# AntoineBlanot/LC2IS

Measured on AMD Instinct MI355X. Metric: training-step images/sec (512x512, ADE20K-150), higher is better.
Workload: dtype bf16; 1 GPU; BaseModelWithText ViT-B/16 + CLIP-text + decoder + fused head/CE train step, 512x512, 151 classes, text len 16, sgd; batch_per_gpu=32, global_batch=32, parallelism=dp1

## Files before the change

### include/lc2is_hip.h

```cpp
#ifndef LC2IS_HIP_H
#define LC2IS_HIP_H
#include <stddef.h>
#include <stdint.h>

#ifdef __cplusplus
extern "C" {
#endif

#define LC2IS_ACT_NONE 0
#define LC2IS_ACT_QUICK_GELU 1
#define LC2IS_ACT_RELU 2
#define LC2IS_ACT_DQUICK_GELU 3
#define LC2IS_ACT_DRELU 4
#define LC2IS_ACT_QUICK_GELU_GRAD 5
#define LC2IS_ACT_MUL_AUX 6
#define LC2IS_ACT_GELU_ERF 7
#define LC2IS_ACT_DGELU_ERF 8
#define LC2IS_ACT_ADD_AUX 9

#define LC2IS_INTERP_BICUBIC 0
#define LC2IS_INTERP_BILINEAR 1

typedef void* lc2is_stream_t;

typedef struct {
  const void* src;
  void* dst;
  void* dstT;
  int N, K, ld_dst, ld_dstT;
  int tile_start;
  int flags;
} lc2is_shadow_desc;

const char* lc2is_version(void);

int lc2is_set_cu_budget(int ncu);
int lc2is_get_cu_budget(void);

int lc2is_gemm_nt_bf16(const void* A, int lda, const void* W, int ldw, const float* bias,
                       const float* resid, int ldr, const void* aux_in, int ldx, void* out_bf16, int ldo,
                       float* out_f32, int ldf, void* aux_out, int ldy, int M, int N, int K, int act,
                       int tile_cfg, lc2is_stream_t stream);

size_t lc2is_gemm_nt_ln_xchg_bytes(int M, int N);
int lc2is_gemm_nt_ln_bf16(const void* A, int lda, const void* W, int ldw, const float* bias, const float* resid, int ldr,
                          float* out_f32, int ldf, const float* gamma, const float* beta, float eps, void* ln_out, int ldl,
                          float* mean, float* rstd, void* xchg, size_t xchg_bytes, int M, int N, int K, lc2is_stream_t stream);

int lc2is_gemm_nt_bf16_batched(const void* A, int lda, long stride_a, const void* W, int ldw, long stride_w,
                               void* out_bf16, int ldo, long stride_ob, float* out_f32, int ldf, long stride_of,
                               int M, int N, int K, int batch, lc2is_stream_t stream);

size_t lc2is_gemm_tn_workspace_bytes(int M, int N, int K);
int lc2is_gemm_tn_bf16(const void* dY, int ldy, const void* X, int ldx, float* dW, int ldw, float* db, int M,
                       int N, int K, int accumulate, void* workspace, size_t workspace_bytes,
                       lc2is_stream_t stream);

#define LC2IS_TN_GROUP_MAX 128
typedef struct lc2is_tn_problem {
  const void* dY; const void* X; float* dW; float* db;
  int ldy, ldx, ldw, M, N, K, accumulate;
} lc2is_tn_problem;
size_t lc2is_gemm_tn_grouped_workspace_bytes(const lc2is_tn_problem* problems, int n);
int lc2is_gemm_tn_grouped(const lc2is_tn_problem* problems, int n, void* workspace, size_t workspace_bytes,
                          lc2is_stream_t stream);
int lc2is_release_captured_tables(void);
int lc2is_captured_tables_mark(void);
int lc2is_release_captured_tables_range(int first, int last);

size_t lc2is_colsum_workspace_bytes(int M, int N);
int lc2is_colsum_bf16(const void* dY, int ldy, float* db, int M, int N, int accumulate, void* workspace,
                      size_t workspace_bytes, lc2is_stream_t stream);

int lc2is_layernorm_fwd(const void* x, int ldx, int x_is_bf16, const float* gamma, const float* beta, void* y_bf16,
                        int ldy, float* y_f32, int ldyf, float* mean, float* rstd, int M, int C, float eps,
                        lc2is_stream_t stream);

size_t lc2is_layernorm_bwd_workspace_bytes(int M, int C);
int lc2is_layernorm_bwd(const void* dy_bf16, int lddy, const float* dy_f32, int lddyf, const void* x,
                        int ldx, int x_is_bf16, const float* gamma, const float* mean, const float* rstd,
                        const void* dres, int lddres, int dres_is_bf16, float* dx_f32, int lddx, void* dx_bf16,
                        int lddxb, float* dgamma, float* dbeta, int accumulate, int M, int C, void* workspace,
                        size_t workspace_bytes, lc2is_stream_t stream);

#define LC2IS_LN_PARTIALS_MAX 64
typedef struct {
  const float* partials;
  float* dgamma;
  float* dbeta;
  int nparts;
  int C;
  int accumulate;
} lc2is_ln_partials;
int lc2is_layernorm_bwd_partials(int M, int C);
int lc2is_ln_partials_reduce(const lc2is_ln_partials* items, int n, lc2is_stream_t stream);

int lc2is_attention_fwd(const void* Q, int ldq, const void* K, int ldk, const void* V, int ldv, void* O,
                        int ldo, float* lse2, const float* kbias, int B, int H, int Sq, int Sk, int D,
                        float scale, int causal, lc2is_stream_t stream);

int lc2is_attention_bwd(const void* Q, int ldq, const void* K, int ldk, const void* V, int ldv,
                        const void* O, int ldo, const void* dO, int lddo, void* dQ, int lddq, void* dK,
                        int lddk, void* dV, int lddv, const float* lse2, float* delta, const float* kbias,
                        int B, int H, int Sq, int Sk, int D, float scale, int causal, lc2is_stream_t stream);

int lc2is_attention_fwd_dropout(const void* Q, int ldq, const void* K, int ldk, const void* V, int ldv, void* O,
                                int ldo, float* lse2, const float* kbias, int B, int H, int Sq, int Sk, int D,
                                float scale, int causal, float p_drop, unsigned long long seed, lc2is_stream_t stream);
int lc2is_attention_bwd_dropout(const void* Q, int ldq, const void* K, int ldk, const void* V, int ldv,
                                const void* O, int ldo, const void* dO, int lddo, void* dQ, int lddq, void* dK,
                                int lddk, void* dV, int lddv, const float* lse2, float* delta, const float* kbias,
                                int B, int H, int Sq, int Sk, int D, float scale, int causal, float p_drop,
                                unsigned long long seed, lc2is_stream_t stream);

int lc2is_dropout_rows_f32(const float* x, int ldx, const float* resid, int ldr, float* y32, int ldy, void* y16,
                           int ldy16, int M, int C, int rows_per_sample, float p, unsigned long long seed,
                           lc2is_stream_t stream);
int lc2is_dropout_rows_bf16(const void* x, int ldx, void* y, int ldy, int M, int C, float p, unsigned long long seed,
                            lc2is_stream_t stream);
int lc2is_dropout_mask(unsigned char* out, long rows, int cols, float p, unsigned long long seed, lc2is_stream_t stream);


int lc2is_shadow_refresh(const lc2is_shadow_desc* descs, int ndesc, int total_tiles, lc2is_stream_t stream);
int lc2is_cast_f32_bf16(const float* src, int ld_src, void* dst_bf16, int ld_dst, int M, int C,
                        lc2is_stream_t stream);
int lc2is_transpose_bf16(const void* src, int ld_src, void* dst, int ld_dst, int R, int C,
                         lc2is_stream_t stream);
int lc2is_transpose_bf16_batched(const void* src, int ld_src, long stride_src, void* dst, int ld_dst, long stride_dst,
                                 int R, int C, int batch, lc2is_stream_t stream);

int lc2is_patchify(const float* pixels, void* out_bf16, int ld_out, int B, int H, int W, int patch,
                   lc2is_stream_t stream);
int lc2is_vit_embed_fwd(const float* patch, int ld_patch, const float* cls, const float* pos, float* x,
                        int ldx, int B, int P, int C, lc2is_stream_t stream);
int lc2is_vit_embed_bwd(const float* dx, int ldx, float* dpos, float* dcls, void* dpatch_bf16, int ld_dpatch,
                        int B, int P, int C, int accumulate, lc2is_stream_t stream);
int lc2is_text_embed_fwd(const int64_t* ids, const float* tok, const float* pos, float* x, int ldx, int B,
                         int L, int C, int vocab, lc2is_stream_t stream);
int lc2is_text_embed_bwd(const int64_t* ids, const float* dx, int ldx, float* dtok, float* dpos, int B, int L,
                         int C, int vocab, int accumulate, lc2is_stream_t stream);
int lc2is_rows_copy_f32(const float* src, int S_src, int src_off, float* dst_f32, void* dst_bf16, int S_dst,
                        int dst_off, int B, int n, int C, lc2is_stream_t stream);
int lc2is_rows_copy_bf16(const void* src, int S_src, int src_off, float* dst_f32, void* dst_bf16, int S_dst,
                         int dst_off, int B, int n, int C, lc2is_stream_t stream);

int lc2is_sgd_step(float* params, const float* grads, float* momentum_buf, size_t n, float lr, float momentum,
                   float weight_decay, float grad_scale, lc2is_stream_t stream);
int lc2is_adamw_step(float* params, const float* grads, float* exp_avg, float* exp_avg_sq, size_t n, float lr,
                     float beta1, float beta2, float eps, float weight_decay, int step, float grad_scale,
                     lc2is_stream_t stream);

size_t lc2is_head_upsample_ce_workspace_bytes(int B, int h, int w, int C, int S, int mode, int want_grad);
int lc2is_head_upsample_ce(const float* scores_lo, int ld, const int64_t* labels, float* dscores_lo,
                           float* scores_hi, float* loss_sum, int B, int h, int w, int C, int S, int mode,
                           long ignore_index, float grad_scale, void* workspace, size_t workspace_bytes,
                           lc2is_stream_t stream);
int lc2is_head_upsample_ce_opts(const float* scores_lo, int ld, const int64_t* labels, float* dscores_lo,
                                float* scores_hi, float* loss_sum, int B, int h, int w, int C, int S, int mode,
                                long ignore_index, float grad_scale, const float* class_weight, float label_smoothing,
                                void* workspace, size_t workspace_bytes, lc2is_stream_t stream);
int lc2is_upsample_bwd_nchw(const float* dhi, float* dlo, int ld, int B, int h, int w, int C, int S, int mode,
                            lc2is_stream_t stream);
int lc2is_ce_nchw_fwd(const float* logits, const int64_t* labels, float* lse, float* loss_sum, int B, int C,
                      long HW, long ignore_index, lc2is_stream_t stream);
int lc2is_ce_nchw_bwd(const float* logits, const int64_t* labels, const float* lse, const float* grad_scale_dev,
                      float grad_scale, float* dlogits, int B, int C, long HW, long ignore_index,
                      lc2is_stream_t stream);
int lc2is_ce_nchw_fwd_opts(const float* logits, const int64_t* labels, float* lse, float* loss_sum, float* loss_px,
                           int B, int C, long HW, long ignore_index, const float* class_weight, float label_smoothing,
                           lc2is_stream_t stream);
int lc2is_ce_nchw_bwd_opts(const float* logits, const int64_t* labels, const float* lse, const float* grad_scale_dev,
                           float grad_scale, const float* grad_px, float* dlogits, int B, int C, long HW,
                           long ignore_index, const float* class_weight, float label_smoothing,
                           lc2is_stream_t stream);
size_t lc2is_ce_nchw_fwd_workspace_bytes(int B, long HW);
int lc2is_ce_nchw_fwd_ordered(const float* logits, const int64_t* labels, float* lse, float* loss_sum, float* loss_px,
                              int B, int C, long HW, long ignore_index, const float* class_weight, float label_smoothing,
                              void* workspace, size_t workspace_bytes, lc2is_stream_t stream);

int lc2is_bilinear_up_fwd(const float* in, float* out_f32, void* out_bf16, int B, int h, int w, int C, int S,
                          lc2is_stream_t stream);
int lc2is_bilinear_up_bwd(const float* dout, float* din_f32, void* din_bf16, int B, int h, int w, int C, int S,
                          int accumulate, lc2is_stream_t stream);
int lc2is_sr_gather(const void* src_bf16, void* dst_bf16, int B, int h, int w, int C, int scatter,
                    lc2is_stream_t stream);
int lc2is_sr_scatter_add_f32(const void* src_bf16, float* dst_f32, int B, int h, int w, int C, lc2is_stream_t stream);
int lc2is_l2norm_fwd(const float* x, float* y_f32, void* y_bf16, float* inv_norm, int M, int C, float eps,
                     lc2is_stream_t stream);
int lc2is_l2norm_bwd(const float* dy, const float* x, const float* inv_norm, float* dx, int M, int C, float eps,
                     lc2is_stream_t stream);
int lc2is_add_n(const float* a, const float* b, const float* c, const float* d, float* out_f32, void* out_bf16,
                size_t n, lc2is_stream_t stream);

int lc2is_rows_gather(const void* src, int ld_src, int src_bf16, void* dst, int ld_dst, int dst_bf16, const int* map,
                      const float* add, int ld_add, int rows, int cols, lc2is_stream_t stream);
int lc2is_swin_attn_fwd(const void* qkv, int ld, void* out, int ldo, float* lse, const float* bias, int nwin,
                        int win_per_img, int nwx, int Hp, int Wp, int ws, int shift, int nH, int C, float scale,
                        lc2is_stream_t stream);
size_t lc2is_swin_attn_bwd_workspace_bytes(int nwin, int ws, int nH);
int lc2is_swin_attn_bwd(const void* qkv, int ld, const void* o, int ld_o, const void* dout, int lddo, const float* lse,
                        const float* bias, void* dqkv, int lddq, float* dbias, int accumulate_dbias, int nwin,
                        int win_per_img, int nwx, int Hp, int Wp, int ws, int shift, int nH, int C, float scale,
                        void* workspace, size_t workspace_bytes, lc2is_stream_t stream);

int lc2is_swin_bias_table_grad(const float* dbias, const int* offsets, const int* positions, float* dtable, int nH, int SS,
                               int T, int accumulate, lc2is_stream_t stream);

int lc2is_resample_u8(const void* src_u8, int H, int W, int C, void* dst_u8, int out_size, int axis, const int* bounds,
                      const int* kk, int ksize, lc2is_stream_t stream);
int lc2is_gather2d_u8(const void* src_u8, int H, int W, int C, void* dst_u8, int out_h, int out_w, const int* yi,
                      const int* xi, lc2is_stream_t stream);
int lc2is_crop_lut(const void* src_u8, int H, int W, int C, int top, int left, int S, const float* lut_f32,
                   float* dst_f32, const int64_t* lut_i64, int64_t* dst_i64, lc2is_stream_t stream);

int lc2is_rows_ce(const float* x, const int64_t* labels, float* lse, float* loss_sum, float* dx, float grad_scale,
                  int M, int K, int accumulate_dx, lc2is_stream_t stream);
int lc2is_cols_ce(const float* x, const int64_t* labels, float* loss_sum, float* dx, float grad_scale, int B, int H,
                  int W, int K, lc2is_stream_t stream);
int lc2is_npair(const float* x, const float* x_pos, const float* x_neg, float* res, int n, int n_pos, int n_neg, int d,
                lc2is_stream_t stream);
int lc2is_npair_bwd(const float* x, const float* x_pos, const float* x_neg, const float* dres, float* dx, float* dx_pos,
                    float* dx_neg, float* workspace, int n, int n_pos, int n_neg, int d, lc2is_stream_t stream);
int lc2is_miou_counts(const float* scores_hi, const int64_t* labels_lo, int* counts, int B, int K, int H, int W, int S,
                      lc2is_stream_t stream);

#define LC2IS_RESIZE_TILE 16
size_t lc2is_resize_argmax_workspace_bytes(long n_tiles, int K);
int lc2is_resize_argmax(const float* scores, int ld, int N, int h, int w, int K, const int64_t* desc, long n_tiles,
                        long total_px, const void* gt, int gt_bytes, uint8_t* pred, int* counts, void* workspace,
                        size_t workspace_bytes, lc2is_stream_t stream);

typedef struct {
  int32_t calls;
// ... 45 lines not shown
```

### lc2is_amd/csrc/gemm_tn.hip

```cpp
#include "common.h"
#include "lc2is_hip.h"
#include <cstdlib>
#include <mutex>
#include <vector>
#include <type_traits>

namespace {

constexpr int TN_BN = 128, TN_BK = 128, TN_BM = 64;
constexpr int TN_TILE_BYTES = TN_BM * 256;
constexpr int TN_STAGE = 2 * TN_TILE_BYTES;

struct TnPlan {
  int ntn, ntk, splits, chunk;
  int big;
};

inline int tn_forced_cfg() {
  static int cfg = -1;
  if (cfg < 0) {
    const char* e = getenv("LC2IS_GEMM_TN_CFG");
    cfg = e ? atoi(e) : 0;
  }
  return cfg;
}

inline TnPlan tn_plan(int M, int N, int K, int ncu) {
  TnPlan p;
  p.big = 0;
  if (N % 256 == 0 && K % 256 == 0 && tn_forced_cfg() != 1) {
    const int ntn = N / 256, ntk = K / 256, tiles = ntn * ntk;
    int splits = (ncu + tiles / 2) / tiles;
    const int max_splits = (M + 511) / 512;
    if (splits > max_splits) splits = max_splits;
    if (splits < 1) splits = 1;
    if (tiles * splits >= 128 || tn_forced_cfg() == 2) {
      int chunk = (M + splits - 1) / splits;
      chunk = (chunk + TN_BM - 1) / TN_BM * TN_BM;
      p.ntn = ntn; p.ntk = ntk; p.chunk = chunk;
      p.splits = (M + chunk - 1) / chunk;
      p.big = 1;
      return p;
    }
  }
  p.ntn = (N + TN_BN - 1) / TN_BN;
  p.ntk = (K + TN_BK - 1) / TN_BK;
  const int tiles = p.ntn * p.ntk;
  int splits = 1024 / tiles;
  int max_splits = (M + 511) / 512;
  const int long_splits = (M + 2047) / 2048;
  if ((long)tiles * long_splits >= 512) max_splits = long_splits;
  if (splits > max_splits) splits = max_splits;
  if (splits < 1) splits = 1;
  int chunk = (M + splits - 1) / splits;
  chunk = (chunk + TN_BM - 1) / TN_BM * TN_BM;
  p.splits = (M + chunk - 1) / chunk;
  p.chunk = chunk;
  return p;
}

__device__ __forceinline__ int tn_swz(int row, int ch) {
  return row * 256 + ((ch ^ (((row & 3) << 2) | ((row >> 2) & 3))) << 4);
}

__device__ __forceinline__ bf16x8_t tr_frag(const char* tile, int addr_lo, int addr_hi) {
  const s16x4_t lo = __builtin_amdgcn_ds_read_tr16_b64_v4i16(
      (__attribute__((address_space(3))) s16x4_t*)LDS_PTR(tile + addr_lo));
  const s16x4_t hi = __builtin_amdgcn_ds_read_tr16_b64_v4i16(
      (__attribute__((address_space(3))) s16x4_t*)LDS_PTR(tile + addr_hi));
  s16x8_t v = {lo[0], lo[1], lo[2], lo[3], hi[0], hi[1], hi[2], hi[3]};
  return __builtin_bit_cast(bf16x8_t, v);
}

__device__ __forceinline__ void tn_small_body(const bf16_t* __restrict__ dY, int ldy,
                                                       const bf16_t* __restrict__ X, int ldx, float* out,
                                                       int ldo, size_t split_stride, float* bias_out,
                                                       size_t bias_split_stride, int M, int N, int K,
                                                       int ntn, int ntk, int chunk, int accumulate, int blk_x, char* smem) {
  const int tid = threadIdx.x, lane = tid & 63, wid = tid >> 6;
  const int wk = wid >> 1, wn = wid & 1;
  const int tiles = ntn * ntk;
  const int split = blk_x / tiles;
  const int tile = blk_x % tiles;
  const int n0 = (tile / ntk) * TN_BN, k0 = (tile % ntk) * TN_BK;
// ... 77 lines not shown
      if (more) gload(st + 1);
#pragma unroll
      for (int s = 0; s < 2; ++s) {
        bf16x8_t xf[4], yf[4];
#pragma unroll
        for (int t = 0; t < 4; ++t) {
          yf[t] = tr_frag(cur, ya_lo[s][t], ya_hi[s][t]);
          xf[t] = tr_frag(cur + TN_TILE_BYTES, xa_lo[s][t], xa_hi[s][t]);
        }
#pragma unroll
        for (int a = 0; a < 4; ++a)
#pragma unroll
          for (int b = 0; b < 4; ++b)
            acc[a][b] = __builtin_amdgcn_mfma_f32_16x16x32_bf16(xf[a], yf[b], acc[a][b], 0, 0, 0);
        if constexpr (CS) {
#pragma unroll
          for (int b = 0; b < 4; ++b) cs[b] = __builtin_amdgcn_mfma_f32_16x16x32_bf16(ones, yf[b], cs[b], 0, 0, 0);
        }
      }
      if (more) lstore(nxt);
      __syncthreads();
    }
  };
  if (do_cs) mainloop(std::true_type{}); else mainloop(std::false_type{});

  float* o = out + (size_t)split * split_stride;
  if (do_cs && lane < 16) {
#pragma unroll
    for (int b = 0; b < 4; ++b) {
      const int n = n0 + wn * 64 + b * 16 + lane;
      if (n < N) {
        float* dst = bias_out + (size_t)split * bias_split_stride + n;
        *dst = (accumulate ? *dst : 0.f) + cs[b][0];
      }
    }
  }
#pragma unroll
  for (int b = 0; b < 4; ++b) {
    const int n = n0 + wn * 64 + b * 16 + (lane & 15);
    if (n >= N) continue;
#pragma unroll
    for (int a = 0; a < 4; ++a) {
      const int k = k0 + wk * 64 + a * 16 + g * 4;
      if (k >= K) continue;
      float* dst = o + (size_t)n * ldo + k;
      f32x4_t v = acc[a][b];
      if (accumulate) v += *(const f32x4_t*)dst;
      *(f32x4_t*)dst = v;
    }
  }
}

__global__ __launch_bounds__(256) void gemm_tn_kernel(const bf16_t* __restrict__ dY, int ldy,
                                                       const bf16_t* __restrict__ X, int ldx, float* out,
                                                       int ldo, size_t split_stride, float* bias_out,
                                                       size_t bias_split_stride, int M, int N, int K,
                                                       int ntn, int ntk, int chunk, int accumulate) {
  extern __shared__ __attribute__((aligned(16))) char smem[];
  tn_small_body(dY, ldy, X, ldx, out, ldo, split_stride, bias_out, bias_split_stride, M, N, K, ntn, ntk, chunk, accumulate,
                (int)blockIdx.x, smem);
}

constexpr int TD_BN = 256, TD_BK = 256;
constexpr int TD_TILE = TN_BM * 512;
constexpr int TD_STAGE = 2 * TD_TILE;

__device__ __forceinline__ int td_swz(int row) { return ((row & 3) << 2) | ((row >> 2) & 3); }

__device__ __forceinline__ void td_dma(const bf16_t* dY, unsigned y_bytes, const bf16_t* X, unsigned x_bytes, char* stage,
                                       int wid, const int* y_goff, const int* x_goff, int ystep, int xstep) {
#if defined(__HIP_DEVICE_COMPILE__)
  const __amdgpu_buffer_rsrc_t rsY = make_rsrc(dY, y_bytes);
  const __amdgpu_buffer_rsrc_t rsX = make_rsrc(X, x_bytes);
#pragma unroll
  for (int j = 0; j < 4; ++j)
    __builtin_amdgcn_raw_ptr_buffer_load_lds(rsY, LDS_PTR(stage + (wid * 4 + j) * 1024), 16, y_goff[j], ystep, 0, 0);
#pragma unroll
  for (int j = 0; j < 4; ++j)
    __builtin_amdgcn_raw_ptr_buffer_load_lds(rsX, LDS_PTR(stage + TD_TILE + (wid * 4 + j) * 1024), 16, x_goff[j], xstep,
                                             0, 0);
#endif
}

__device__ __forceinline__ void tn_dma_body(const bf16_t* __restrict__ dY, int ldy, const bf16_t* __restrict__ X, int ldx,
                                            float* out, int ldo, size_t split_stride, float* bias_out,
                                            size_t bias_split_stride, int M, int N, int K, int ntn, int ntk, int chunk,
                                            int accumulate, int block, char* smem) {
  const int tid = threadIdx.x, lane = tid & 63;
  const int wid = __builtin_amdgcn_readfirstlane(tid >> 6);
  const int wk = wid >> 2, wn = wid & 3;
  const int tiles = ntn * ntk;
  const int split = block / tiles;
  const int tile = block % tiles;
  const int n0 = (tile / ntk) * TD_BN, k0 = (tile % ntk) * TD_BK;
  const int m_begin = split * chunk;
  int m_end = m_begin + chunk;
  if (m_end > M) m_end = M;
  const int nsteps = (m_end - m_begin + TN_BM - 1) / TN_BM;
  const unsigned y_bytes = (unsigned)m_end * (unsigned)ldy * 2u, x_bytes = (unsigned)m_end * (unsigned)ldx * 2u;

  int y_goff[4], x_goff[4];
#pragma unroll
  for (int j = 0; j < 4; ++j) {
    const int row = 2 * (wid * 4 + j) + (lane >> 5);
    const int ch = (lane & 31) ^ td_swz(row);
    y_goff[j] = ((m_begin + row) * ldy + n0 + ch * 8) * 2;
    x_goff[j] = ((m_begin + row) * ldx + k0 + ch * 8) * 2;
  }

  const int g = lane >> 4, q = (lane >> 2) & 3, pp = lane & 3;
  const int r_lo = 8 * g + q, r_hi = r_lo + 4;
  const int x_lo = TD_TILE + r_lo * 512 + (((wk * 16 + (pp >> 1)) ^ td_swz(r_lo)) << 4) + 8 * (pp & 1);
  const int x_hi = TD_TILE + r_hi * 512 + (((wk * 16 + (pp >> 1)) ^ td_swz(r_hi)) << 4) + 8 * (pp & 1);
  const int y_lo = r_lo * 512 + (((wn * 8 + (pp >> 1)) ^ td_swz(r_lo)) << 4) + 8 * (pp & 1);
  const int y_hi = r_hi * 512 + (((wn * 8 + (pp >> 1)) ^ td_swz(r_hi)) << 4) + 8 * (pp & 1);

  f32x4_t acc[8][4];
#pragma unroll
  for (int a = 0; a < 8; ++a)
#pragma unroll
    for (int b = 0; b < 4; ++b) acc[a][b] = f32x4_t{0.f, 0.f, 0.f, 0.f};
  const bool do_cs = (bias_out != nullptr) && (tile % ntk == 0) && (wk == 0);
  f32x4_t cs[4];
#pragma unroll
  for (int b = 0; b < 4; ++b) cs[b] = f32x4_t{0.f, 0.f, 0.f, 0.f};
  const s16x8_t ones_s = {0x3F80, 0x3F80, 0x3F80, 0x3F80, 0x3F80, 0x3F80, 0x3F80, 0x3F80};
  const bf16x8_t ones = __builtin_bit_cast(bf16x8_t, ones_s);

  if (nsteps > 0) td_dma(dY, y_bytes, X, x_bytes, smem, wid, y_goff, x_goff, 0, 0);
  __syncthreads();

  auto mainloop = [&](auto cs_tag) {
    constexpr bool CS = decltype(cs_tag)::value;
    for (int st = 0; st < nsteps; ++st) {
      const char* cur = smem + (st & 1) * TD_STAGE;
      if (st + 1 < nsteps)
        td_dma(dY, y_bytes, X, x_bytes, smem + ((st + 1) & 1) * TD_STAGE, wid, y_goff, x_goff,
               (st + 1) * TN_BM * ldy * 2, (st + 1) * TN_BM * ldx * 2);
#pragma unroll
      for (int s = 0; s < 2; ++s) {
        bf16x8_t xf[8], yf[4];
#pragma unroll
        for (int t = 0; t < 4; ++t) yf[t] = tr_frag(cur + s * 16384, y_lo ^ (t << 5), y_hi ^ (t << 5));
#pragma unroll
        for (int t = 0; t < 8; ++t) xf[t] = tr_frag(cur + s * 16384, x_lo ^ (t << 5), x_hi ^ (t << 5));
#pragma unroll
        for (int b = 0; b < 4; ++b)
#pragma unroll
          for (int a = 0; a < 8; ++a)
            acc[a][b] = __builtin_amdgcn_mfma_f32_16x16x32_bf16(xf[a], yf[b], acc[a][b], 0, 0, 0);
        if constexpr (CS) {
#pragma unroll
          for (int b = 0; b < 4; ++b) cs[b] = __builtin_amdgcn_mfma_f32_16x16x32_bf16(ones, yf[b], cs[b], 0, 0, 0);
        }
      }
      __syncthreads();
    }
  };
  if (do_cs) mainloop(std::true_type{}); else mainloop(std::false_type{});

  float* o = out + (size_t)split * split_stride;
  if (do_cs && lane < 16) {
#pragma unroll
    for (int b = 0; b < 4; ++b) {
      const int n = n0 + wn * 64 + b * 16 + lane;
      float* dst = bias_out + (size_t)split * bias_split_stride + n;
      *dst = (accumulate ? *dst : 0.f) + cs[b][0];
    }
  }
#pragma unroll
  for (int b = 0; b < 4; ++b) {
    const int n = n0 + wn * 64 + b * 16 + (lane & 15);
#pragma unroll
    for (int a = 0; a < 8; ++a) {
      const int k = k0 + wk * 128 + a * 16 + g * 4;
      float* dst = o + (size_t)n * ldo + k;
      f32x4_t v = acc[a][b];
      if (accumulate) v += *(const f32x4_t*)dst;
      *(f32x4_t*)dst = v;
    }
  }
}

__global__ __launch_bounds__(512, 2) void gemm_tn_dma_kernel(const bf16_t* __restrict__ dY, int ldy,
                                                              const bf16_t* __restrict__ X, int ldx, float* out, int ldo,
                                                              size_t split_stride, float* bias_out,
                                                              size_t bias_split_stride, int M, int N, int K, int ntn,
                                                              int ntk, int chunk, int accumulate) {
  extern __shared__ __attribute__((aligned(16))) char smem[];
  tn_dma_body(dY, ldy, X, ldx, out, ldo, split_stride, bias_out, bias_split_stride, M, N, K, ntn, ntk, chunk, accumulate,
              blockIdx.x, smem);
}

constexpr int TG_MAX = 16;
struct TnGroupProb {
  const bf16_t* dY; const bf16_t* X; float* out; float* bias_out; float* dW; float* db;
  size_t split_stride, bias_split_stride;
  int ldy, ldx, ldo, ldw, M, N, K, ntn, ntk, chunk, splits, accumulate;
  int blk_end;
  int red_end;
  int red_blocks;
};
struct TnGroup {
  int n, remap;
  TnGroupProb p[TG_MAX];
};

constexpr int TG_TBL_MAX = LC2IS_TN_GROUP_MAX;
struct TnGroupTbl {
  int n, pad_[3];
  int blk_end[TG_TBL_MAX];
  int red_end[TG_TBL_MAX];
  TnGroupProb p[TG_TBL_MAX];
};
constexpr size_t TG_TBL_BYTES = (sizeof(TnGroupTbl) + 255) / 256 * 256;

__global__ __launch_bounds__(512, 2) void gemm_tn_grouped_tbl_kernel(const TnGroupTbl* __restrict__ t) {
  extern __shared__ __attribute__((aligned(16))) char smem[];
  int i = 0, begin = 0;
  const int n = t->n;
  const int bid = t->pad_[0] ? xcd_round_remap((int)blockIdx.x, (int)gridDim.x) : (int)blockIdx.x;
#pragma unroll 1
  while (i < n - 1 && bid >= t->blk_end[i]) { begin = t->blk_end[i]; ++i; }
  const TnGroupProb* q = &t->p[i];
  tn_dma_body(q->dY, q->ldy, q->X, q->ldx, q->out, q->ldo, q->split_stride, q->bias_out, q->bias_split_stride, q->M, q->N,
              q->K, q->ntn, q->ntk, q->chunk, q->splits == 1 ? q->accumulate : 0, bid - begin, smem);
}

__global__ __launch_bounds__(256) void gemm_tn_grouped_small_kernel(TnGroup g) {
  extern __shared__ __attribute__((aligned(16))) char smem[];
  int i = 0, begin = 0;
#pragma unroll 1
  while (i < g.n - 1 && (int)blockIdx.x >= g.p[i].blk_end) { begin = g.p[i].blk_end; ++i; }
  const TnGroupProb& q = g.p[i];
  tn_small_body(q.dY, q.ldy, q.X, q.ldx, q.out, q.ldo, q.split_stride, q.bias_out, q.bias_split_stride, q.M, q.N, q.K, q.ntn,
                q.ntk, q.chunk, q.splits == 1 ? q.accumulate : 0, (int)blockIdx.x - begin, smem);
}

__global__ __launch_bounds__(256) void gemm_tn_grouped_small_tbl_kernel(const TnGroupTbl* __restrict__ t) {
  extern __shared__ __attribute__((aligned(16))) char smem[];
  int i = 0, begin = 0;
  const int n = t->n;
#pragma unroll 1
  while (i < n - 1 && (int)blockIdx.x >= t->blk_end[i]) { begin = t->blk_end[i]; ++i; }
  const TnGroupProb* q = &t->p[i];
  tn_small_body(q->dY, q->ldy, q->X, q->ldx, q->out, q->ldo, q->split_stride, q->bias_out, q->bias_split_stride, q->M, q->N,
                q->K, q->ntn, q->ntk, q->chunk, q->splits == 1 ? q->accumulate : 0, (int)blockIdx.x - begin, smem);
}

__global__ __launch_bounds__(512, 2) void gemm_tn_grouped_kernel(TnGroup g) {
  extern __shared__ __attribute__((aligned(16))) char smem[];
  int i = 0, begin = 0;
  const int bid = g.remap ? xcd_round_remap((int)blockIdx.x, (int)gridDim.x) : (int)blockIdx.x;
#pragma unroll 1
  while (i < g.n - 1 && bid >= g.p[i].blk_end) { begin = g.p[i].blk_end; ++i; }
  const TnGroupProb& q = g.p[i];
  tn_dma_body(q.dY, q.ldy, q.X, q.ldx, q.out, q.ldo, q.split_stride, q.bias_out, q.bias_split_stride, q.M, q.N, q.K, q.ntn,
              q.ntk, q.chunk, q.splits == 1 ? q.accumulate : 0, bid - begin, smem);
}

__device__ __forceinline__ void slab_reduce_grouped_body(const TnGroupProb& q, int b);

__global__ __launch_bounds__(256) void slab_reduce_grouped_kernel(TnGroup g) {
  int i = 0, begin = 0;
#pragma unroll 1
  while (i < g.n - 1 && (int)blockIdx.x >= g.p[i].red_end) { begin = g.p[i].red_end; ++i; }
  slab_reduce_grouped_body(g.p[i], (int)blockIdx.x - begin);
}

__global__ __launch_bounds__(256) void slab_reduce_grouped_tbl_kernel(const TnGroupTbl* __restrict__ t) {
  int i = 0, begin = 0;
  const int n = t->n;
#pragma unroll 1
  while (i < n - 1 && (int)blockIdx.x >= t->red_end[i]) { begin = t->red_end[i]; ++i; }
  slab_reduce_grouped_body(t->p[i], (int)blockIdx.x - begin);
}

__device__ __forceinline__ void slab_reduce_grouped_body(const TnGroupProb& q, int b) {
  if (q.splits <= 1) return;
  if (b >= q.red_blocks) {
    const int n = (b - q.red_blocks) * 256 + threadIdx.x;
    if (q.db && n < q.N) {
      float t = 0.f;
      for (int sp = 0; sp < q.splits; ++sp) t += q.bias_out[(size_t)sp * q.bias_split_stride + n];
      q.db[n] = q.accumulate ? q.db[n] + t : t;
    }
    return;
  }
  const int K4 = q.K >> 2;
  const size_t total = (size_t)q.N * K4;
  for (size_t idx = (size_t)b * 256 + threadIdx.x; idx < total; idx += (size_t)q.red_blocks * 256) {
    const int n = (int)(idx / K4), k4 = (int)(idx % K4);
    float4 s4 = *(reinterpret_cast<const float4*>(q.out + (size_t)n * q.K) + k4);
    for (int sp = 1; sp < q.splits; ++sp) {
      const float4 v = *reinterpret_cast<const float4*>(q.out + sp * q.split_stride + (size_t)n * q.K + 4 * k4);
      s4.x += v.x; s4.y += v.y; s4.z += v.z; s4.w += v.w;
    }
    float4* dst = reinterpret_cast<float4*>(q.dW + (size_t)n * q.ldw) + k4;
    if (q.accumulate) {
      const float4 d = *dst;
      s4.x += d.x; s4.y += d.y; s4.z += d.z; s4.w += d.w;
    }
    *dst = s4;
  }
}

__global__ __launch_bounds__(256) void slab_reduce_kernel(const float* __restrict__ ws, int splits,
                                                           size_t split_stride, float* out, int ldo, int N,
                                                           int K, int accumulate, const float* __restrict__ bias_ws,
                                                           float* db, int bias_blocks) {
  const int slab_blocks = gridDim.x - bias_blocks;
  if ((int)blockIdx.x >= slab_blocks) {
    const int n = (blockIdx.x - slab_blocks) * 256 + threadIdx.x;
    if (n < N) {
      float t = 0.f;
      for (int sp = 0; sp < splits; ++sp) t += bias_ws[(size_t)sp * N + n];
      db[n] = accumulate ? db[n] + t : t;
    }
    return;
  }
  const int K4 = K >> 2;
  const size_t total = (size_t)N * K4;
  for (size_t i = (size_t)blockIdx.x * 256 + threadIdx.x; i < total; i += (size_t)slab_blocks * 256) {
    const int n = (int)(i / K4), k4 = (int)(i % K4);
    const float4* src = reinterpret_cast<const float4*>(ws + (size_t)n * K) + k4;
    float4 s = *src;
    for (int sp = 1; sp < splits; ++sp) {
      const float4 v = *reinterpret_cast<const float4*>(ws + sp * split_stride + (size_t)n * K + 4 * k4);
      s.x += v.x; s.y += v.y; s.z += v.z; s.w += v.w;
    }
    float4* dst = reinterpret_cast<float4*>(out + (size_t)n * ldo) + k4;
    if (accumulate) {
      const float4 d = *dst;
      s.x += d.x; s.y += d.y; s.z += d.z; s.w += d.w;
    }
    *dst = s;
  }
}

constexpr int CS_ROWBLOCKS = 128;

__global__ __launch_bounds__(256) void colsum_kernel(const bf16_t* __restrict__ dY, int ldy, float* ws, int M,
                                                      int N) {
  __shared__ float red[4][64][8];
  const int lane = threadIdx.x & 63, wave = threadIdx.x >> 6;
  const int cg = blockIdx.x * 64 + lane;
  float s[8] = {0.f, 0.f, 0.f, 0.f, 0.f, 0.f, 0.f, 0.f};
  if (cg * 8 < N) {
    for (int row = blockIdx.y * 4 + wave; row < M; row += gridDim.y * 4) {
      const uint4 v = *reinterpret_cast<const uint4*>(dY + (size_t)row * ldy + cg * 8);
      s[0] += bf16_to_f32((bf16_t)(v.x & 0xffff)); s[1] += bf16_to_f32((bf16_t)(v.x >> 16));
      s[2] += bf16_to_f32((bf16_t)(v.y & 0xffff)); s[3] += bf16_to_f32((bf16_t)(v.y >> 16));
      s[4] += bf16_to_f32((bf16_t)(v.z & 0xffff)); s[5] += bf16_to_f32((bf16_t)(v.z >> 16));
      s[6] += bf16_to_f32((bf16_t)(v.w & 0xffff)); s[7] += bf16_to_f32((bf16_t)(v.w >> 16));
    }
  }
#pragma unroll
  for (int j = 0; j < 8; ++j) red[wave][lane][j] = s[j];
  __syncthreads();
  if (wave == 0 && cg * 8 < N) {
#pragma unroll
    for (int j = 0; j < 8; ++j)
      ws[(size_t)blockIdx.y * N + cg * 8 + j] =
          (red[0][lane][j] + red[1][lane][j]) + (red[2][lane][j] + red[3][lane][j]);
  }
}

__global__ __launch_bounds__(256) void colsum_reduce_kernel(const float* __restrict__ ws, int nparts, int N,
                                                             float* db, int accumulate) {
  const int c = blockIdx.x * 256 + threadIdx.x;
  if (c >= N) return;
  float s = 0.f;
  for (int p = 0; p < nparts; ++p) s += ws[(size_t)p * N + c];
  db[c] = accumulate ? db[c] + s : s;
}

inline int colsum_parts(int M) {
  int p = (M + 3) / 4;
  return p > CS_ROWBLOCKS ? CS_ROWBLOCKS : p;
}

}

static size_t tn_plan_bytes(const TnPlan& p, int N, int K) {
  return p.splits > 1 ? (size_t)p.splits * N * ((size_t)K + 1) * sizeof(float) : 0;
}
// ... 108 lines not shown
    wbytes += 4.0 * pr[i].N * pr[i].K;
    const int steps = (pr[i].M + TN_BM - 1) / TN_BM;
    if (steps > max_steps) max_steps = steps;
    const int ms = (pr[i].M + 511) / 512;
    if (ms < max_splits) max_splits = ms;
  }
  if (max_splits > 32) max_splits = 32;
  if (max_splits < 1) max_splits = 1;
  const double slab_unit = 2.0 / 4.0e12 / 1.65e-6;
  int best = 1;
  double best_t = 1e300;
  for (int sp = 1; sp <= max_splits; ++sp) {
    const long blocks = tiles * sp;
    const double rounds = (double)((blocks + ncu - 1) / ncu);
    const double t = rounds * ((max_steps + sp - 1) / sp + 13.0) + (sp > 1 ? sp * wbytes * slab_unit : 0.0);
    if (t < best_t) { best_t = t; best = sp; }
  }
  for (int i = 0; i < n; ++i) { pl.splits[i] = best; pl.order[i] = i; }
  const int rem = (int)(tiles % ncu);
  if (n > 1 && tiles > ncu && rem != 0 && max_splits >= 2) {
    bool in_tail[TG_TBL_MAX] = {};
    int ts = 0;
    double tail_bytes = 0;
    while (ts < rem) {
      int pick = -1;
      for (int i = 0; i < n; ++i)
        if (!in_tail[i] && (pick < 0 || ptiles[i] <= ptiles[pick])) pick = i;
      if (pick < 0) break;
      in_tail[pick] = true;
      ts += ptiles[pick];
      tail_bytes += 4.0 * pr[pick].N * pr[pick].K;
    }
    int sp = ts > 0 ? ncu / ts : 0;
    if (sp > max_splits) sp = max_splits;
    if (ts >= rem && sp >= 2) {
      const double rounds = (double)((tiles - ts + ncu - 1) / ncu);
      const double t = rounds * (max_steps + 13.0) + ((max_steps + sp - 1) / sp + 13.0) + sp * tail_bytes * slab_unit;
      if (t < best_t) {
        int k = 0;
        for (int i = 0; i < n; ++i) if (!in_tail[i]) { pl.order[k++] = i; pl.splits[i] = 1; }
        for (int i = 0; i < n; ++i) if (in_tail[i]) { pl.order[k++] = i; pl.splits[i] = sp; }
      }
    }
  }
  pl.ws_floats = 0;
  for (int i = 0; i < n; ++i)
    if (pl.splits[i] > 1) pl.ws_floats += (size_t)pl.splits[i] * pr[i].N * ((size_t)pr[i].K + 1);
}
}

static std::mutex g_captured_mu;
static std::vector<void*> g_captured_tables;

extern "C" int lc2is_release_captured_tables(void) {
  std::lock_guard<std::mutex> lock(g_captured_mu);
  int n = 0;
  for (void*& p : g_captured_tables)
    if (p) { (void)hipHostFree(p); p = nullptr; ++n; }
  return n;
}

extern "C" int lc2is_captured_tables_mark(void) {
  std::lock_guard<std::mutex> lock(g_captured_mu);
  return (int)g_captured_tables.size();
}

extern "C" int lc2is_release_captured_tables_range(int first, int last) {
  std::lock_guard<std::mutex> lock(g_captured_mu);
  if (first < 0) first = 0;
  if (last > (int)g_captured_tables.size()) last = (int)g_captured_tables.size();
  int n = 0;
  for (int i = first; i < last; ++i)
    if (g_captured_tables[i]) { (void)hipHostFree(g_captured_tables[i]); g_captured_tables[i] = nullptr; ++n; }
  return n;
}

extern "C" size_t lc2is_gemm_tn_grouped_workspace_bytes(const lc2is_tn_problem* problems, int n) {
  if (tg_valid(problems, n) != LC2IS_OK) return 0;
  TgPlan pl;
  tg_plan(problems, n, pl, lc2is_ncu());
  return pl.ws_floats * sizeof(float) + (n > TG_MAX ? TG_TBL_BYTES : 0);
}

extern "C" int lc2is_gemm_tn_grouped(const lc2is_tn_problem* problems, int n, void* workspace, size_t workspace_bytes,
                                     lc2is_stream_t stream_) {
  hipStream_t stream = (hipStream_t)stream_;
  int rc = tg_valid(problems, n);
  if (rc) return rc;
  TgPlan pl;
  tg_plan(problems, n, pl, lc2is_ncu());
  const bool tbl = n > TG_MAX;
  const size_t need = pl.ws_floats * sizeof(float) + (tbl ? TG_TBL_BYTES : 0);
  if (need && (!workspace || workspace_bytes < need)) return LC2IS_ERR_WORKSPACE;
  struct TblSlot { TnGroupTbl* host; hipEvent_t done; bool in_flight; };
  static thread_local TblSlot ring[4] = {};
  static thread_local unsigned ring_pos = 0;
  static thread_local TnGroupTbl small_tbl;
  TblSlot* slot = nullptr;
  TnGroupTbl* captured_tbl = nullptr;
  if (tbl) {
    hipStreamCaptureStatus cap = hipStreamCaptureStatusNone;
    if (hipStreamIsCapturing(stream, &cap) != hipSuccess) return LC2IS_ERR_LAUNCH;
    if (cap != hipStreamCaptureStatusNone) {
      hipStreamCaptureMode mode = hipStreamCaptureModeRelaxed;
      if (hipThreadExchangeStreamCaptureMode(&mode) != hipSuccess) return LC2IS_ERR_LAUNCH;
      const hipError_t e = hipHostMalloc((void**)&captured_tbl, sizeof(TnGroupTbl), hipHostMallocDefault);
      if (hipThreadExchangeStreamCaptureMode(&mode) != hipSuccess || e != hipSuccess) return LC2IS_ERR_LAUNCH;
      {
        std::lock_guard<std::mutex> lock(g_captured_mu);
        g_captured_tables.push_back(captured_tbl);
      }
    } else {
      slot = &ring[ring_pos++ & 3];
      if (!slot->host) {
        if (hipHostMalloc((void**)&slot->host, sizeof(TnGroupTbl), hipHostMallocDefault) != hipSuccess ||
            hipEventCreateWithFlags(&slot->done, hipEventDisableTiming) != hipSuccess)
          return LC2IS_ERR_LAUNCH;
      }
      if (slot->in_flight && hipEventSynchronize(slot->done) != hipSuccess) return LC2IS_ERR_LAUNCH;
      slot->in_flight = false;
    }
  }
  TnGroupTbl& t = captured_tbl ? *captured_tbl : (tbl ? *slot->host : small_tbl);
  static const int xcd_order = !(getenv("LC2IS_TN_XCD") && atoi(getenv("LC2IS_TN_XCD")) == 0);
  t.n = n;
  t.pad_[0] = xcd_order;
  float* ws = (float*)((char*)workspace + (tbl ? TG_TBL_BYTES : 0));
  int blk = 0, red = 0;
  for (int k = 0; k < n; ++k) {
    const int i = pl.order[k];
    const lc2is_tn_problem& q = problems[i];
    TnGroupProb& d = t.p[k];
    d.dY = (const bf16_t*)q.dY; d.X = (const bf16_t*)q.X; d.dW = q.dW; d.db = q.db;
    d.ldy = q.ldy; d.ldx = q.ldx; d.ldw = q.ldw; d.M = q.M; d.N = q.N; d.K = q.K; d.accumulate = q.accumulate;
    d.ntn = pl.small ? (q.N + TN_BN - 1) / TN_BN : q.N / 256;
    d.ntk = pl.small ? (q.K + TN_BK - 1) / TN_BK : q.K / 256;
    int chunk = (q.M + pl.splits[i] - 1) / pl.splits[i];
    chunk = (chunk + TN_BM - 1) / TN_BM * TN_BM;
    d.chunk = chunk;
    d.splits = (q.M + chunk - 1) / chunk;
    if (pl.splits[i] > 1) {
      float* base = ws;
      ws += (size_t)pl.splits[i] * q.N * ((size_t)q.K + 1);
      if (d.splits > 1) {
        d.out = base; d.ldo = q.K; d.split_stride = (size_t)q.N * q.K;
        d.bias_out = q.db ? base + (size_t)d.splits * q.N * q.K : nullptr; d.bias_split_stride = (size_t)q.N;
      }
    }
    if (d.splits <= 1) {
      d.out = q.dW; d.ldo = q.ldw; d.split_stride = 0; d.bias_out = q.db; d.bias_split_stride = 0;
    }
    blk += d.ntn * d.ntk * d.splits;
    d.blk_end = blk;
    const size_t total4 = (size_t)q.N * q.K / 4;
    int rb = (int)((total4 + 255) / 256);
    if (rb > 1024) rb = 1024;
    d.red_blocks = d.splits > 1 ? rb : 0;
    red += d.splits > 1 ? rb + (q.db ? (q.N + 255) / 256 : 0) : 0;
    d.red_end = red;
    t.blk_end[k] = blk;
    t.red_end[k] = red;
  }
  static DevOnce attr_set;
  if (attr_set.need()) {
    if (hipFuncSetAttribute((const void*)gemm_tn_grouped_kernel, hipFuncAttributeMaxDynamicSharedMemorySize,
                            2 * TD_STAGE) != hipSuccess ||
        hipFuncSetAttribute((const void*)gemm_tn_grouped_tbl_kernel, hipFuncAttributeMaxDynamicSharedMemorySize,
                            2 * TD_STAGE) != hipSuccess ||
        hipFuncSetAttribute((const void*)gemm_tn_grouped_small_kernel, hipFuncAttributeMaxDynamicSharedMemorySize,
                            2 * TN_STAGE) != hipSuccess ||
        hipFuncSetAttribute((const void*)gemm_tn_grouped_small_tbl_kernel, hipFuncAttributeMaxDynamicSharedMemorySize,
                            2 * TN_STAGE) != hipSuccess)
      return LC2IS_ERR_LAUNCH;
    attr_set.done();
  }
  if (tbl) {
    if (hipMemcpyAsync(workspace, &t, sizeof(TnGroupTbl), hipMemcpyHostToDevice, stream) != hipSuccess) return LC2IS_ERR_LAUNCH;
    if (slot) {
      if (hipEventRecord(slot->done, stream) != hipSuccess) return LC2IS_ERR_LAUNCH;
      slot->in_flight = true;
    }
    const TnGroupTbl* dt = (const TnGroupTbl*)workspace;
    if (pl.small)
      hipLaunchKernelGGL(gemm_tn_grouped_small_tbl_kernel, dim3(blk), dim3(256), 2 * TN_STAGE, stream, dt);
    else
      hipLaunchKernelGGL(gemm_tn_grouped_tbl_kernel, dim3(blk), dim3(512), 2 * TD_STAGE, stream, dt);
    rc = lc2is_check_launch();
    if (rc || red == 0) return rc;
    hipLaunchKernelGGL(slab_reduce_grouped_tbl_kernel, dim3(red), dim3(256), 0, stream, dt);
    return lc2is_check_launch();
  }
  TnGroup g{};
  g.n = n;
  g.remap = xcd_order;
  for (int k = 0; k < n; ++k) g.p[k] = t.p[k];
  if (pl.small)
    hipLaunchKernelGGL(gemm_tn_grouped_small_kernel, dim3(blk), dim3(256), 2 * TN_STAGE, stream, g);
  else
    hipLaunchKernelGGL(gemm_tn_grouped_kernel, dim3(blk), dim3(512), 2 * TD_STAGE, stream, g);
  rc = lc2is_check_launch();
  if (rc || red == 0) return rc;
  hipLaunchKernelGGL(slab_reduce_grouped_kernel, dim3(red), dim3(256), 0, stream, g);
  return lc2is_check_launch();
}

extern "C" size_t lc2is_colsum_workspace_bytes(int M, int N) {
  if (M <= 0 || N <= 0) return 0;
  return (size_t)colsum_parts(M) * N * sizeof(float);
}

extern "C" int lc2is_colsum_bf16(const void* dY, int ldy, float* db, int M, int N, int accumulate,
                                 void* workspace, size_t workspace_bytes, lc2is_stream_t stream_) {
  hipStream_t stream = (hipStream_t)stream_;
  if (!dY || !db) return LC2IS_ERR_NULL;
  if (M <= 0 || N <= 0 || N % 8 || ldy < N || ldy % 8) return LC2IS_ERR_SHAPE;
  if (!workspace || workspace_bytes < lc2is_colsum_workspace_bytes(M, N)) return LC2IS_ERR_WORKSPACE;
  const int parts = colsum_parts(M);
  hipLaunchKernelGGL(colsum_kernel, dim3((N / 8 + 63) / 64, parts), dim3(256), 0, stream, (const bf16_t*)dY,
                     ldy, (float*)workspace, M, N);
  int rc = lc2is_check_launch();
  if (rc) return rc;
  hipLaunchKernelGGL(partials_reduce_kernel, dim3((N + 31) / 32, 1), dim3(1024), 0, stream,
                     (const float*)workspace, parts, (size_t)N, (size_t)0, N, db, (float*)nullptr, accumulate);
  return lc2is_check_launch();
}
```

### lc2is_amd/csrc/misc.hip

```cpp
#include "common.h"
#include "lc2is_hip.h"

namespace {

__global__ __launch_bounds__(256) void shadow_refresh_kernel(const lc2is_shadow_desc* __restrict__ descs,
                                                              int ndesc) {
  __shared__ bf16_t tile[64][66];
  int lo = 0, hi = ndesc - 1;
  const int bid = blockIdx.x;
  while (lo < hi) {
    const int mid = (lo + hi + 1) >> 1;
    if (descs[mid].tile_start <= bid) lo = mid; else hi = mid - 1;
  }
  const lc2is_shadow_desc d = descs[lo];
  const int t = bid - d.tile_start;
  const int tk = (d.K + 63) / 64;
  const int n0 = (t / tk) * 64, k0 = (t % tk) * 64;
  const float* src = (const float*)d.src;
  bf16_t* dst = (bf16_t*)d.dst;
  bf16_t* dstT = (bf16_t*)d.dstT;
  const int tx = threadIdx.x & 15, ty = threadIdx.x >> 4;
#pragma unroll
  for (int r = 0; r < 4; ++r) {
    const int n = n0 + ty + 16 * r, k = k0 + 4 * tx;
    float4 v = make_float4(0.f, 0.f, 0.f, 0.f);
    if (n < d.N && k < d.K) v = *reinterpret_cast<const float4*>(src + (size_t)n * d.K + k);
    const bf16_t b0 = f32_to_bf16(v.x), b1 = f32_to_bf16(v.y), b2 = f32_to_bf16(v.z), b3 = f32_to_bf16(v.w);
    if (d.flags & 1) {
      if (dst && n < d.N && k < d.K) *reinterpret_cast<float4*>((float*)d.dst + (size_t)n * d.ld_dst + k) = v;
    } else if (dst && n < d.N && k < d.K) {
      uint2 pk = make_uint2((unsigned)b0 | ((unsigned)b1 << 16), (unsigned)b2 | ((unsigned)b3 << 16));
      *reinterpret_cast<uint2*>(dst + (size_t)n * d.ld_dst + k) = pk;
    }
    tile[ty + 16 * r][4 * tx + 0] = b0;
    tile[ty + 16 * r][4 * tx + 1] = b1;
    tile[ty + 16 * r][4 * tx + 2] = b2;
    tile[ty + 16 * r][4 * tx + 3] = b3;
  }
  if (!dstT) return;
  __syncthreads();
#pragma unroll
  for (int r = 0; r < 4; ++r) {
    const int k = k0 + ty + 16 * r, n = n0 + 4 * tx;
    if (k < d.K && n < d.N) {
      const int kk = ty + 16 * r;
      uint2 pk = make_uint2((unsigned)tile[4 * tx][kk] | ((unsigned)tile[4 * tx + 1][kk] << 16),
                            (unsigned)tile[4 * tx + 2][kk] | ((unsigned)tile[4 * tx + 3][kk] << 16));
      *reinterpret_cast<uint2*>(dstT + (size_t)k * d.ld_dstT + n) = pk;
    }
  }
}

__global__ __launch_bounds__(256) void cast_f32_bf16_kernel(const float* __restrict__ src, int lds_,
                                                             bf16_t* dst, int ldd, int M, int C) {
  const int C4 = C >> 2;
  const size_t total = (size_t)M * C4;
  for (size_t i = (size_t)blockIdx.x * 256 + threadIdx.x; i < total; i += (size_t)gridDim.x * 256) {
    const int m = (int)(i / C4), c4 = (int)(i % C4);
    const float4 v = *reinterpret_cast<const float4*>(src + (size_t)m * lds_ + 4 * c4);
    *reinterpret_cast<uint2*>(dst + (size_t)m * ldd + 4 * c4) =
        make_uint2(pack_bf16x2(v.x, v.y), pack_bf16x2(v.z, v.w));
  }
}

__global__ __launch_bounds__(256) void transpose_bf16_kernel(const bf16_t* __restrict__ src, int lds_,
                                                              bf16_t* dst, int ldd, int R, int C, long bs_src,
                                                              long bs_dst) {
  __shared__ bf16_t tile[64][66];
  src += (size_t)blockIdx.z * bs_src;
  dst += (size_t)blockIdx.z * bs_dst;
  const int r0 = blockIdx.y * 64, c0 = blockIdx.x * 64;
  const int tx = threadIdx.x & 63, ty = threadIdx.x >> 6;
  for (int r = ty; r < 64; r += 4) {
    const int rr = r0 + r, cc = c0 + tx;
    tile[r][tx] = (rr < R && cc < C) ? src[(size_t)rr * lds_ + cc] : (bf16_t)0;
  }
  __syncthreads();
  for (int c = ty; c < 64; c += 4) {
    const int cc = c0 + c, rr = r0 + tx;
    if (cc < C && rr < R) dst[(size_t)cc * ldd + rr] = tile[tx][c];
  }
}

__global__ __launch_bounds__(256) void patchify_kernel(const float* __restrict__ pix, bf16_t* out, int ldo,
// ... 82 lines not shown
    }
  }
}

__global__ __launch_bounds__(256) void text_embed_fwd_kernel(const int64_t* __restrict__ ids,
                                                              const float* __restrict__ tok,
                                                              const float* __restrict__ pos, float* x, int ldx,
                                                              int BL, int L, int C, int vocab) {
  const int C4 = C >> 2;
  const size_t total = (size_t)BL * C4;
  for (size_t i = (size_t)blockIdx.x * 256 + threadIdx.x; i < total; i += (size_t)gridDim.x * 256) {
    const int c4 = (int)(i % C4), r = (int)(i / C4);
    int64_t id = ids[r];
    if (id < 0) id = 0;
    if (id >= vocab) id = vocab - 1;
    const float4 t = *reinterpret_cast<const float4*>(tok + (size_t)id * C + 4 * c4);
    const float4 pe = *reinterpret_cast<const float4*>(pos + (size_t)(r % L) * C + 4 * c4);
    *reinterpret_cast<float4*>(x + (size_t)r * ldx + 4 * c4) =
        make_float4(t.x + pe.x, t.y + pe.y, t.z + pe.z, t.w + pe.w);
  }
}

__global__ __launch_bounds__(256) void text_embed_dtok_kernel(const int64_t* __restrict__ ids, const float* __restrict__ dx,
                                                               int ldx, float* dtok, int R, int C, int vocab) {
  const int r = blockIdx.x;
  auto clampid = [&](int64_t v) { return v < 0 ? (int64_t)0 : (v >= vocab ? (int64_t)(vocab - 1) : v); };
  const int64_t id = clampid(ids[r]);
  int seen = 0;
  for (int q = threadIdx.x; q < r; q += 256) seen |= (clampid(ids[q]) == id);
  if (__syncthreads_or(seen)) return;
  for (int c = threadIdx.x; c < C; c += 256) {
    float acc = 0.f;
    for (int q = r; q < R; ++q)
      if (clampid(ids[q]) == id) acc += dx[(size_t)q * ldx + c];
    dtok[(size_t)id * C + c] += acc;
  }
}

__global__ __launch_bounds__(256) void text_embed_bwd_kernel(const float* __restrict__ dx, int ldx, float* dpos, int B, int L,
                                                              int C, int accumulate) {
  const int total = L * C;
  for (int i = blockIdx.x * 256 + threadIdx.x; i < total; i += gridDim.x * 256) {
    const int c = i % C, l = i / C;
    float acc = 0.f;
    for (int b = 0; b < B; ++b) acc += dx[((size_t)b * L + l) * ldx + c];
    dpos[(size_t)l * C + c] = accumulate ? dpos[(size_t)l * C + c] + acc : acc;
  }
}

__global__ __launch_bounds__(256) void rows_copy_bf16_kernel(const bf16_t* __restrict__ src, int S_src, int src_off,
                                                              float* dst, bf16_t* dst_b, int S_dst, int dst_off,
                                                              int B, int n, int C) {
  const int C4 = C >> 2;
  const size_t total = (size_t)B * n * C4;
  for (size_t i = (size_t)blockIdx.x * 256 + threadIdx.x; i < total; i += (size_t)gridDim.x * 256) {
    const int c4 = (int)(i % C4);
    const int r = (int)(i / C4);
    const int s = r % n, b = r / n;
    const uint2 pk = *reinterpret_cast<const uint2*>(src + ((size_t)b * S_src + src_off + s) * C + 4 * c4);
    const size_t o = ((size_t)b * S_dst + dst_off + s) * C + 4 * c4;
    if (dst) *reinterpret_cast<float4*>(dst + o) = make_float4(bf16_to_f32((bf16_t)(pk.x & 0xffff)), bf16_to_f32((bf16_t)(pk.x >> 16)),
                                                               bf16_to_f32((bf16_t)(pk.y & 0xffff)), bf16_to_f32((bf16_t)(pk.y >> 16)));
    if (dst_b) *reinterpret_cast<uint2*>(dst_b + o) = pk;
  }
}

__global__ __launch_bounds__(256) void rows_copy_kernel(const float* __restrict__ src, int S_src, int src_off,
                                                         float* dst, bf16_t* dst_b, int S_dst, int dst_off,
                                                         int B, int n, int C) {
  const int C4 = C >> 2;
  const size_t total = (size_t)B * n * C4;
  for (size_t i = (size_t)blockIdx.x * 256 + threadIdx.x; i < total; i += (size_t)gridDim.x * 256) {
    const int c4 = (int)(i % C4);
    const int r = (int)(i / C4);
    const int s = r % n, b = r / n;
    const float4 v = *reinterpret_cast<const float4*>(src + ((size_t)b * S_src + src_off + s) * C + 4 * c4);
    const size_t o = ((size_t)b * S_dst + dst_off + s) * C + 4 * c4;
    if (dst) *reinterpret_cast<float4*>(dst + o) = v;
    if (dst_b) *reinterpret_cast<uint2*>(dst_b + o) = make_uint2(pack_bf16x2(v.x, v.y), pack_bf16x2(v.z, v.w));
  }
}

__global__ __launch_bounds__(256) void sgd_kernel(float* p, const float* __restrict__ g, float* mom, size_t n4,
                                                   float lr, float momentum, float wd, float gscale) {
  for (size_t i = (size_t)blockIdx.x * 256 + threadIdx.x; i < n4; i += (size_t)gridDim.x * 256) {
    float4 pv = reinterpret_cast<float4*>(p)[i];
    const float4 gv = reinterpret_cast<const float4*>(g)[i];
    float d[4] = {gv.x * gscale + wd * pv.x, gv.y * gscale + wd * pv.y, gv.z * gscale + wd * pv.z,
                  gv.w * gscale + wd * pv.w};
    if (mom) {
      float4 mv = reinterpret_cast<float4*>(mom)[i];
      mv.x = momentum * mv.x + d[0]; mv.y = momentum * mv.y + d[1];
      mv.z = momentum * mv.z + d[2]; mv.w = momentum * mv.w + d[3];
      reinterpret_cast<float4*>(mom)[i] = mv;
      d[0] = mv.x; d[1] = mv.y; d[2] = mv.z; d[3] = mv.w;
    }
    pv.x -= lr * d[0]; pv.y -= lr * d[1]; pv.z -= lr * d[2]; pv.w -= lr * d[3];
    reinterpret_cast<float4*>(p)[i] = pv;
  }
}

__global__ __launch_bounds__(256) void adamw_kernel(float* p, const float* __restrict__ g, float* m, float* v,
                                                     size_t n4, float lr, float b1, float b2, float eps,
                                                     float wd, float bc1, float bc2, float gscale) {
  for (size_t i = (size_t)blockIdx.x * 256 + threadIdx.x; i < n4; i += (size_t)gridDim.x * 256) {
    float4 pv = reinterpret_cast<float4*>(p)[i];
    const float4 gv = reinterpret_cast<const float4*>(g)[i];
    float4 mv = reinterpret_cast<float4*>(m)[i], vv = reinterpret_cast<float4*>(v)[i];
    float* pp = &pv.x; const float* gp = &gv.x; float* mp = &mv.x; float* vp = &vv.x;
#pragma unroll
    for (int k = 0; k < 4; ++k) {
      const float gg = gp[k] * gscale;
      pp[k] *= (1.f - lr * wd);
      mp[k] = b1 * mp[k] + (1.f - b1) * gg;
      vp[k] = b2 * vp[k] + (1.f - b2) * gg * gg;
      const float denom = sqrtf(vp[k]) / sqrtf(bc2) + eps;
      pp[k] -= (lr / bc1) * (mp[k] / denom);
    }
    reinterpret_cast<float4*>(p)[i] = pv;
    reinterpret_cast<float4*>(m)[i] = mv;
    reinterpret_cast<float4*>(v)[i] = vv;
  }
}

inline int ew_grid(size_t work_items) {
  size_t g = (work_items + 255) / 256;
  if (g > 4096) g = 4096;
  if (g < 1) g = 1;
  return (int)g;
}

}

extern "C" int lc2is_shadow_refresh(const lc2is_shadow_desc* descs_dev, int ndesc, int total_tiles,
                                    lc2is_stream_t stream_) {
  hipStream_t stream = (hipStream_t)stream_;
  if (!descs_dev) return LC2IS_ERR_NULL;
  if (ndesc <= 0 || total_tiles <= 0) return LC2IS_ERR_SHAPE;
  hipLaunchKernelGGL(shadow_refresh_kernel, dim3(total_tiles), dim3(256), 0, stream, descs_dev, ndesc);
  return lc2is_check_launch();
}

extern "C" int lc2is_cast_f32_bf16(const float* src, int ld_src, void* dst, int ld_dst, int M, int C,
                                   lc2is_stream_t stream_) {
  hipStream_t stream = (hipStream_t)stream_;
  if (!src || !dst) return LC2IS_ERR_NULL;
  if (M <= 0 || C <= 0 || C % 4 || ld_src < C || ld_dst < C || ld_src % 4 || ld_dst % 4) return LC2IS_ERR_SHAPE;
  hipLaunchKernelGGL(cast_f32_bf16_kernel, dim3(ew_grid((size_t)M * C / 4)), dim3(256), 0, stream, src, ld_src,
                     (bf16_t*)dst, ld_dst, M, C);
  return lc2is_check_launch();
}

extern "C" int lc2is_transpose_bf16(const void* src, int ld_src, void* dst, int ld_dst, int R, int C,
                                    lc2is_stream_t stream_) {
  hipStream_t stream = (hipStream_t)stream_;
  if (!src || !dst) return LC2IS_ERR_NULL;
  if (R <= 0 || C <= 0 || ld_src < C || ld_dst < R) return LC2IS_ERR_SHAPE;
  hipLaunchKernelGGL(transpose_bf16_kernel, dim3((C + 63) / 64, (R + 63) / 64), dim3(256), 0, stream,
                     (const bf16_t*)src, ld_src, (bf16_t*)dst, ld_dst, R, C, 0L, 0L);
  return lc2is_check_launch();
}

extern "C" int lc2is_transpose_bf16_batched(const void* src, int ld_src, long stride_src, void* dst, int ld_dst,
                                            long stride_dst, int R, int C, int batch, lc2is_stream_t stream_) {
  hipStream_t stream = (hipStream_t)stream_;
  if (!src || !dst) return LC2IS_ERR_NULL;
  if (R <= 0 || C <= 0 || ld_src < C || ld_dst < R || batch <= 0 || batch > 65535) return LC2IS_ERR_SHAPE;
  hipLaunchKernelGGL(transpose_bf16_kernel, dim3((C + 63) / 64, (R + 63) / 64, batch), dim3(256), 0, stream,
                     (const bf16_t*)src, ld_src, (bf16_t*)dst, ld_dst, R, C, stride_src, stride_dst);
  return lc2is_check_launch();
}

extern "C" int lc2is_patchify(const float* pixels, void* out_bf16, int ld_out, int B, int H, int W,
                              int patch, lc2is_stream_t stream_) {
  hipStream_t stream = (hipStream_t)stream_;
  if (!pixels || !out_bf16) return LC2IS_ERR_NULL;
  if (B <= 0 || H <= 0 || W != H || patch <= 0 || H / patch <= 0) return LC2IS_ERR_SHAPE;
  const int G = H / patch, kdim = 3 * patch * patch;
  if (ld_out < kdim) return LC2IS_ERR_SHAPE;
  if (patch % 8 == 0 && W % 8 == 0 && ld_out % 8 == 0 && ((uintptr_t)pixels & 15) == 0 && ((uintptr_t)out_bf16 & 15) == 0)
    hipLaunchKernelGGL(patchify8_kernel, dim3(ew_grid((size_t)B * 3 * H * W / 8)), dim3(256), 0, stream, pixels, (bf16_t*)out_bf16,
                       ld_out, B, H, W, patch, G);
  else
    hipLaunchKernelGGL(patchify_kernel, dim3(B * G * 3 * patch), dim3(256), 0, stream, pixels, (bf16_t*)out_bf16,
                       ld_out, B, H, W, patch, G);
  int rc = lc2is_check_launch();
  if (rc || ld_out == kdim) return rc;
  hipLaunchKernelGGL(zero_pad_cols_kernel, dim3(ew_grid((size_t)B * G * G * (ld_out - kdim))), dim3(256), 0,
                     stream, (bf16_t*)out_bf16, ld_out, B * G * G, kdim);
  return lc2is_check_launch();
}

extern "C" int lc2is_vit_embed_fwd(const float* patch, int ld_patch, const float* cls, const float* pos,
                                   float* x, int ldx, int B, int P, int C, lc2is_stream_t stream_) {
  hipStream_t stream = (hipStream_t)stream_;
  if (!patch || !cls || !pos || !x) return LC2IS_ERR_NULL;
  if (B <= 0 || P <= 0 || C <= 0 || C % 4 || ld_patch < C || ld_patch % 4 || ldx < C || ldx % 4)
    return LC2IS_ERR_SHAPE;
  hipLaunchKernelGGL(vit_embed_fwd_kernel, dim3(ew_grid((size_t)B * (P + 1) * C / 4)), dim3(256), 0, stream,
                     patch, ld_patch, cls, pos, x, ldx, B, P, C);
  return lc2is_check_launch();
}

extern "C" int lc2is_vit_embed_bwd(const float* dx, int ldx, float* dpos, float* dcls, void* dpatch_bf16,
                                   int ld_dpatch, int B, int P, int C, int accumulate, lc2is_stream_t stream_) {
  hipStream_t stream = (hipStream_t)stream_;
  if (!dx || !dpos || !dcls) return LC2IS_ERR_NULL;
  if (B <= 0 || P <= 0 || C <= 0 || C % 4 || ldx < C || ldx % 4 || (dpatch_bf16 && (ld_dpatch < C || ld_dpatch % 4)))
    return LC2IS_ERR_SHAPE;
  hipLaunchKernelGGL(vit_embed_bwd_kernel, dim3(ew_grid((size_t)(P + 1) * C / 4)), dim3(256), 0, stream, dx, ldx,
                     dpos, dcls, (bf16_t*)dpatch_bf16, ld_dpatch, B, P, C, accumulate);
  return lc2is_check_launch();
}

extern "C" int lc2is_text_embed_fwd(const int64_t* ids, const float* tok, const float* pos, float* x, int ldx,
                                    int B, int L, int C, int vocab, lc2is_stream_t stream_) {
  hipStream_t stream = (hipStream_t)stream_;
  if (!ids || !tok || !pos || !x) return LC2IS_ERR_NULL;
  if (B <= 0 || L <= 0 || C <= 0 || C % 4 || vocab <= 0 || ldx < C || ldx % 4) return LC2IS_ERR_SHAPE;
  hipLaunchKernelGGL(text_embed_fwd_kernel, dim3(ew_grid((size_t)B * L * C / 4)), dim3(256), 0, stream, ids, tok,
                     pos, x, ldx, B * L, L, C, vocab);
  return lc2is_check_launch();
}

extern "C" int lc2is_text_embed_bwd(const int64_t* ids, const float* dx, int ldx, float* dtok, float* dpos,
                                    int B, int L, int C, int vocab, int accumulate, lc2is_stream_t stream_) {
  hipStream_t stream = (hipStream_t)stream_;
  if (!ids || !dx || !dtok || !dpos) return LC2IS_ERR_NULL;
  if (B <= 0 || L <= 0 || C <= 0 || vocab <= 0 || ldx < C) return LC2IS_ERR_SHAPE;
  hipLaunchKernelGGL(text_embed_dtok_kernel, dim3(B * L), dim3(256), 0, stream, ids, dx, ldx, dtok, B * L, C, vocab);
  int rc = lc2is_check_launch();
  if (rc) return rc;
  hipLaunchKernelGGL(text_embed_bwd_kernel, dim3(ew_grid((size_t)L * C)), dim3(256), 0, stream, dx, ldx, dpos, B, L, C,
                     accumulate);
  return lc2is_check_launch();
}

extern "C" int lc2is_rows_copy_f32(const float* src, int S_src, int src_off, float* dst_f32, void* dst_bf16,
                                   int S_dst, int dst_off, int B, int n, int C, lc2is_stream_t stream_) {
  hipStream_t stream = (hipStream_t)stream_;
  if (!src || (!dst_f32 && !dst_bf16)) return LC2IS_ERR_NULL;
  if (B <= 0 || n <= 0 || C <= 0 || C % 4 || src_off < 0 || dst_off < 0 || src_off + n > S_src ||
      dst_off + n > S_dst)
    return LC2IS_ERR_SHAPE;
  hipLaunchKernelGGL(rows_copy_kernel, dim3(ew_grid((size_t)B * n * C / 4)), dim3(256), 0, stream, src, S_src,
                     src_off, dst_f32, (bf16_t*)dst_bf16, S_dst, dst_off, B, n, C);
  return lc2is_check_launch();
}

extern "C" int lc2is_rows_copy_bf16(const void* src, int S_src, int src_off, float* dst_f32, void* dst_bf16,
                                    int S_dst, int dst_off, int B, int n, int C, lc2is_stream_t stream_) {
  hipStream_t stream = (hipStream_t)stream_;
  if (!src || (!dst_f32 && !dst_bf16)) return LC2IS_ERR_NULL;
  if (B <= 0 || n <= 0 || C <= 0 || C % 4 || src_off < 0 || dst_off < 0 || src_off + n > S_src ||
      dst_off + n > S_dst)
    return LC2IS_ERR_SHAPE;
  hipLaunchKernelGGL(rows_copy_bf16_kernel, dim3(ew_grid((size_t)B * n * C / 4)), dim3(256), 0, stream, (const bf16_t*)src,
                     S_src, src_off, dst_f32, (bf16_t*)dst_bf16, S_dst, dst_off, B, n, C);
  return lc2is_check_launch();
}

extern "C" int lc2is_sgd_step(float* params, const float* grads, float* momentum_buf, size_t n, float lr,
                              float momentum, float weight_decay, float grad_scale, lc2is_stream_t stream_) {
  hipStream_t stream = (hipStream_t)stream_;
  if (!params || !grads) return LC2IS_ERR_NULL;
  if (n == 0 || n % 4) return LC2IS_ERR_SHAPE;
  hipLaunchKernelGGL(sgd_kernel, dim3(ew_grid(n / 4)), dim3(256), 0, stream, params, grads, momentum_buf, n / 4,
                     lr, momentum, weight_decay, grad_scale);
  return lc2is_check_launch();
}

extern "C" int lc2is_adamw_step(float* params, const float* grads, float* exp_avg, float* exp_avg_sq, size_t n,
                                float lr, float beta1, float beta2, float eps, float weight_decay, int step,
                                float grad_scale, lc2is_stream_t stream_) {
  hipStream_t stream = (hipStream_t)stream_;
  if (!params || !grads || !exp_avg || !exp_avg_sq) return LC2IS_ERR_NULL;
  if (n == 0 || n % 4 || step < 1) return LC2IS_ERR_SHAPE;
  const float bc1 = 1.f - powf(beta1, (float)step), bc2 = 1.f - powf(beta2, (float)step);
  hipLaunchKernelGGL(adamw_kernel, dim3(ew_grid(n / 4)), dim3(256), 0, stream, params, grads, exp_avg,
                     exp_avg_sq, n / 4, lr, beta1, beta2, eps, weight_decay, bc1, bc2, grad_scale);
  return lc2is_check_launch();
}
```

### lc2is_amd/nn/base.py

```python
from __future__ import annotations

import torch
from torch import nn

from .. import ops


import os as _os

_WGRAD_SIDE = _os.environ.get("LC2IS_WGRAD_STREAM", "0") == "1"
_wgrad_streams: dict = {}


def wgrad_stream(device) -> torch.cuda.Stream:
    s = _wgrad_streams.get(device)
    if s is None:
        s = _wgrad_streams[device] = torch.cuda.Stream(device)
    return s


class _on_wgrad_stream:

    def __init__(self, *tensors):
        self.tensors = [t for t in tensors if t is not None]
# ... 26 lines not shown

    _state = None
    _torch_seed = None
    last = {}

    @classmethod
    def manual_seed(cls, seed: int) -> None:
        cls._state = seed & 0xFFFFFFFFFFFFFFFF
        cls._torch_seed = torch.initial_seed()

    @classmethod
    def get_state(cls) -> int | None:
        return cls._state

    @classmethod
    def set_state(cls, state: int | None) -> None:
        cls._state = None if state is None else int(state) & 0xFFFFFFFFFFFFFFFF
        cls._torch_seed = torch.initial_seed()

    @classmethod
    def next_seed(cls, site: str | None = None, p: float = 0.0) -> int:
        ts = torch.initial_seed()
        if cls._state is None or ts != cls._torch_seed:
            rank = torch.distributed.get_rank() if (torch.distributed.is_available() and torch.distributed.is_initialized()) else 0
            cls._state = (ts * 0x9E3779B97F4A7C15 + rank * 0xD1B54A32D192ED03 + 0x2545F4914F6CDD1D) & 0xFFFFFFFFFFFFFFFF
            cls._torch_seed = ts
        cls._state = (cls._state + 0x9E3779B97F4A7C15) & 0xFFFFFFFFFFFFFFFF
        z = cls._state
        z = ((z ^ (z >> 30)) * 0xBF58476D1CE4E5B9) & 0xFFFFFFFFFFFFFFFF
        z = ((z ^ (z >> 27)) * 0x94D049BB133111EB) & 0xFFFFFFFFFFFFFFFF
        z ^= z >> 31
        if site is not None:
            cls.last[site] = (z, p)
        return z


def assign_rng_names(root) -> None:
    for name, mod in root.named_modules():
        mod.rng_name = (name + ".") if name else ""


class DropSites:

    def __init__(self, p: float, prefix: str = "") -> None:
        self.p, self.prefix, self.seeds = float(p), prefix, {}

    def seed(self, site: str) -> int:
        s = self.seeds.get(site)
        if s is None:
            s = self.seeds[site] = DropoutRng.next_seed(self.prefix + site, self.p)
        return s

    @staticmethod
    def make(module_training: bool, p: float, prefix: str = ""):
        return DropSites(p, prefix) if (module_training and p > 0.0) else None


def drop_branch_add(ds: DropSites | None, site: str, branch32: torch.Tensor, resid32: torch.Tensor) -> torch.Tensor:
    return ops.dropout_rows_f32(branch32, ds.p, ds.seed(site), resid=resid32)[0]


def drop_branch_grad16(ds: DropSites | None, site: str, g32: torch.Tensor, g16: torch.Tensor | None) -> torch.Tensor:
    if ds is None:
        return g16 if g16 is not None else ops.cast_bf16(g32)
    return ops.dropout_rows_f32(g32, ds.p, ds.seeds[site], out_f32=None, out_bf16=True)[1]


def require_cuda(t: torch.Tensor, what: str) -> None:
    if not t.is_cuda:
        raise RuntimeError(
            f"lc2is_amd: {what} is on {t.device}; the MI355X path has no CPU fallback — move the module and its "
            "inputs to a HIP device (the CPU oracle lives in oracle/ and is test-only)")


class HipModule(nn.Module):

    def __init__(self) -> None:
        super().__init__()
        self._sh = None
        self._sh_table = None
        self._sh_versions = None
        self._sh_device = None
        self._sh_ptrs = []
        self._grad_ready_cb = None
        self._part_ready_cb = None

    def _build_shadows(self, device):
        raise NotImplementedError

    def _params_for_version(self):
        return list(self.parameters(recurse=True))

    def _ensure_ready(self):
        ps = self._params_for_version()
        dev = ps[0].device
        require_cuda(ps[0], f"{type(self).__name__} parameters")
        if self._sh is None or self._sh_device != dev or any(p.data_ptr() != q for p, q in zip(ps, self._sh_ptrs)):
            ns, entries = self._build_shadows(dev)
            self._sh = ns
            self._sh_table = ops.ShadowTable(entries, dev) if entries else None
            self._sh_device = dev
            self._sh_ptrs = [p.data_ptr() for p in ps]
            self._sh_versions = None
        vers = [p._version for p in ps]
        if vers != self._sh_versions:
            if self._sh_table is not None:
                self._sh_table.refresh()
            self._post_refresh()
            self._sh_versions = vers
        return self._sh

    def _post_refresh(self):
        pass

    def _grads_ready(self):
        if self._sh_device is not None:
            join_wgrad_stream(self._sh_device)
        if self._grad_ready_cb is not None:
            self._grad_ready_cb(self)

    def _part_grads_ready(self, part: nn.Module):
        if self._part_ready_cb is not None:
            if self._sh_device is not None:
                join_wgrad_stream(self._sh_device)
            self._part_ready_cb(self, part)

    def invalidate_shadows(self):
        self._sh_versions = None

    def _apply(self, fn, *args, **kwargs):
        self._sh = None
        return super()._apply(fn, *args, **kwargs)


def grad_buf(p: torch.Tensor):
    if p.grad is None:
        g = getattr(p, "_lc2is_grad", None)
        if g is None or g.shape != p.shape or g.device != p.device:
            g = torch.empty_like(p)
        p.grad = g
        return g, False
    return p.grad, True


class WgradBatch:

    _active = None

    def __init__(self, enabled: bool = True):
        self.enabled = enabled and _os.environ.get("LC2IS_WGRAD_GROUPED", "1") != "0"
        self.items = []

    def __enter__(self):
        if self.enabled:
            self._prev, WgradBatch._active = WgradBatch._active, self
            self._prev_ln = ops.ln_defer_begin()
        return self

    def __exit__(self, exc_type, *exc):
        if self.enabled:
            WgradBatch._active = self._prev
            if exc_type is None:
                self.flush()
                ops.ln_defer_end(self._prev_ln)
            else:
                ops._ln_defer = self._prev_ln
        return False

    def flush(self):
        ops.ln_defer_flush()
        items, self.items = self.items, []
        gmax = ops.GROUP_MAX
        for i in range(0, len(items), gmax):
            chunk = items[i:i + gmax]
            if len(chunk) == 1:
                dy, x, g, gb, acc = chunk[0]
                ops.gemm_tn(dy, x, g, accumulate=acc, db=gb)
            else:
                ops.gemm_tn_grouped(chunk)


def linear_bwd_params(dy_bf16: torch.Tensor, x_bf16: torch.Tensor, weight: nn.Parameter, bias: nn.Parameter | None):
    want_b = bias is not None and bias.requires_grad
    if weight.requires_grad:
        g, acc = grad_buf(weight)
        gb, accb = grad_buf(bias) if want_b else (None, False)
        batch = WgradBatch._active
        if batch is not None and (gb is None or accb == acc) and ops.gemm_tn_groupable(dy_bf16, x_bf16):
            batch.items.append((dy_bf16, x_bf16, g.reshape(g.shape[0], -1), gb, acc))
            return
        with _on_wgrad_stream(dy_bf16, x_bf16):
            if gb is not None and accb != acc:
                ops.colsum(dy_bf16, gb, accumulate=accb)
                gb = None
            ops.gemm_tn(dy_bf16, x_bf16, g.reshape(g.shape[0], -1), accumulate=acc, db=gb)
    elif want_b:
        g, acc = grad_buf(bias)
        with _on_wgrad_stream(dy_bf16):
            ops.colsum(dy_bf16, g, accumulate=acc)


def vec_grad(p: nn.Parameter | None):
    if p is None or not p.requires_grad:
        return None, False
    return grad_buf(p)


GROUP_SKIP = 255


def granule_group_map(offsets, sizes, group_ids, dead=(), align: int = 64, ngroups: int | None = None) -> torch.Tensor:
    if not (len(offsets) == len(sizes) == len(group_ids)) or not len(offsets):
        raise ValueError("granule_group_map: offsets, sizes and group_ids must be non-empty and of one length")
    top = GROUP_SKIP if ngroups is None else int(ngroups)
    if not 1 <= top <= GROUP_SKIP:
        raise ValueError(f"granule_group_map: ngroups must be 1..{GROUP_SKIP}, got {ngroups}")
    dead = set(dead)
    ids, counts, at = [], [], 0
    for k, (o, n, g) in enumerate(zip(offsets, sizes, group_ids)):
        if o != at or o % align or n < 1:
            raise ValueError(f"granule_group_map: parameter {k} at offset {o} (size {n}) does not continue an aligned layout at {at}")
        if not 0 <= int(g) < top:
            raise ValueError(f"granule_group_map: parameter {k} has group id {g}; ids are 0..{top - 1}")
        ids.append(GROUP_SKIP if k in dead else int(g))
        counts.append((n + align - 1) // align)
        at = o + counts[-1] * align
    return torch.repeat_interleave(torch.tensor(ids, dtype=torch.uint8), torch.tensor(counts, dtype=torch.int64))


class ParamArena:

    ALIGN = 64

    def __init__(self, module: nn.Module):
        params = []
        seen = set()
        for p in module.parameters():
            if id(p) not in seen:
                seen.add(id(p))
                params.append(p)
        if not params:
            raise RuntimeError("ParamArena: module has no parameters")
        dev = params[0].device
        require_cuda(params[0], "ParamArena parameters")
        offs, total = [], 0
        for p in params:
            offs.append(total)
            total += (p.numel() + self.ALIGN - 1) // self.ALIGN * self.ALIGN
        self.flat = torch.zeros(total, dtype=torch.float32, device=dev)
        self.grad = torch.zeros(total, dtype=torch.float32, device=dev)
        self.params, self.offsets = params, offs
        self.ranges = {}
        with torch.no_grad():
            for p, o in zip(params, offs):
                n = p.numel()
                view = self.flat[o:o + n].view(p.shape)
                view.copy_(p.data)
                p.data = view
                p._lc2is_grad = self.grad[o:o + n].view(p.shape)
                p.grad = None
                self.ranges[id(p)] = (o, o + n)
        self.numel = total
        self.dead = ()
        self._group_ids = None
        self._group_maps = {}

    def set_groups(self, group_ids, ngroups: int):
        granule_group_map(self.offsets, [p.numel() for p in self.params], group_ids, ngroups=ngroups)
        self._group_ids, self._ngroups, self._group_maps = [int(g) for g in group_ids], int(ngroups), {}

    def group_map(self) -> torch.Tensor:
        m = self._group_maps.get(self.dead)
# ... 49 lines not shown
```

### lc2is_amd/nn/clip.py

```python
from __future__ import annotations

import math
from dataclasses import dataclass

import torch
from torch import nn

from .. import ops
from .base import HipModule, WgradBatch, grad_buf, linear_bwd_params, require_cuda, vec_grad


@dataclass
class ClipArch:
    hidden: int = 768
    heads: int = 12
    layers: int = 12
    intermediate: int = 3072
    eps: float = 1e-5
    vocab: int = 49408
    max_pos: int = 77
    eos_token_id: int = 49407


VIT_B16 = ClipArch(768, 12, 12, 3072)
# ... 77 lines not shown
            layer.mlp.fc1.bias.zero_()
            layer.mlp.fc2.bias.zero_()
        emb = enc.embeddings
        if hasattr(emb, "class_embedding"):
            emb.class_embedding.normal_(0, a.hidden ** -0.5)
            emb.patch_embedding.weight.normal_(0, 0.02)
            emb.position_embedding.weight.normal_(0, 0.02)
        else:
            emb.token_embedding.weight.normal_(0, 0.02)
            emb.position_embedding.weight.normal_(0, 0.02)


def _stack_shadows(stack: _Stack, a: ClipArch, device):
    C, I = a.hidden, a.intermediate
    bf = dict(dtype=torch.bfloat16, device=device)
    per, entries = [], []
    for layer in stack.layers:
        at, mlp = layer.self_attn, layer.mlp
        s = dict(wqkv=torch.empty(3 * C, C, **bf), wqkvT=torch.empty(C, 3 * C, **bf),
                 bqkv=torch.empty(3 * C, dtype=torch.float32, device=device),
                 wo=torch.empty(C, C, **bf), woT=torch.empty(C, C, **bf),
                 w1=torch.empty(I, C, **bf), w1T=torch.empty(C, I, **bf),
                 w2=torch.empty(C, I, **bf), w2T=torch.empty(I, C, **bf))
        for j, proj in enumerate((at.q_proj, at.k_proj, at.v_proj)):
            entries.append((proj.weight, s["wqkv"][j * C:(j + 1) * C], s["wqkvT"][:, j * C:(j + 1) * C]))
            entries.append((proj.bias, s["bqkv"][j * C:(j + 1) * C], None))
        entries.append((at.out_proj.weight, s["wo"], s["woT"]))
        entries.append((mlp.fc1.weight, s["w1"], s["w1T"]))
        entries.append((mlp.fc2.weight, s["w2"], s["w2T"]))
        per.append(s)
    return per, entries


_RESID_BF16 = __import__('os').environ.get("LC2IS_RESID_STREAM", "f32") == "bf16"


def _stack_fwd(x, stack: _Stack, sh, a: ClipArch, B: int, S: int, kbias, causal: bool, save: bool):
    C, H = a.hidden, a.heads
    D = C // H
    scale = D ** -0.5
    saved = []
    lean = x.dtype == torch.bfloat16
    fuse = (not lean) and ops.gemm_nt_ln_ok(x.shape[0], C, C) and ops.gemm_nt_ln_ok(x.shape[0], C, a.intermediate)
    nxt_ln = None
    layers = list(stack.layers)
    for li, (layer, s) in enumerate(zip(layers, sh)):
        if nxt_ln is not None:
            h, m1, r1 = nxt_ln
        else:
            h, _, m1, r1 = ops.layernorm_fwd(x, layer.layer_norm1.weight, layer.layer_norm1.bias, a.eps, save_stats=save)
        qkv, _, _ = ops.gemm_nt(h, s["wqkv"], s["bqkv"])
        o, lse = ops.attention_fwd(qkv[:, :C], qkv[:, C:2 * C], qkv[:, 2 * C:], B, H, S, S, D, scale, causal=causal,
                                   kbias=kbias, save_lse=save)
        if fuse:
            x_mid, h2, m2, r2 = ops.gemm_nt_ln(o, s["wo"], layer.self_attn.out_proj.bias, x, layer.layer_norm2.weight,
                                               layer.layer_norm2.bias, a.eps, save_stats=save)
        else:
            if lean:
                x_mid, _, _ = ops.gemm_nt(o, s["wo"], layer.self_attn.out_proj.bias, resid=x)
            else:
                _, x_mid, _ = ops.gemm_nt(o, s["wo"], layer.self_attn.out_proj.bias, resid=x, out_bf16=None, out_f32=True)
            h2, _, m2, r2 = ops.layernorm_fwd(x_mid, layer.layer_norm2.weight, layer.layer_norm2.bias, a.eps,
                                              save_stats=save)
        act, _, z = ops.gemm_nt(h2, s["w1"], layer.mlp.fc1.bias, act=ops.ACT_QUICK_GELU, aux_out=True if save else None)
        nxt_ln = None
        if fuse and li + 1 < len(layers):
            nl = layers[li + 1].layer_norm1
            x_out, hn, mn, rn = ops.gemm_nt_ln(act, s["w2"], layer.mlp.fc2.bias, x_mid, nl.weight, nl.bias, a.eps, save_stats=save)
            nxt_ln = (hn, mn, rn)
        elif lean:
            x_out, _, _ = ops.gemm_nt(act, s["w2"], layer.mlp.fc2.bias, resid=x_mid)
        else:
            _, x_out, _ = ops.gemm_nt(act, s["w2"], layer.mlp.fc2.bias, resid=x_mid, out_bf16=None, out_f32=True)
        if save:
            saved.append((x, m1, r1, h, qkv, o, lse, x_mid, m2, r2, h2, z, act))
        x = x_out
    return x, saved


_GRAD_STREAM_BF16 = __import__('os').environ.get("LC2IS_GRAD_STREAM", "bf16") != "f32"


def _stack_bwd(g32, g16, stack: _Stack, sh, saved, a: ClipArch, B: int, S: int, kbias, causal: bool, on_layer_done=None,
               final_f32: bool = True):
    C, H = a.hidden, a.heads
    D = C // H
    scale = D ** -0.5
    if on_layer_done is not None:
        default_pair = min(3, len(stack.layers))
    else:
        default_pair = len(stack.layers)
    pair = int(__import__('os').environ.get('LC2IS_WGRAD_PAIR', str(default_pair)))
    batch, waiting = WgradBatch(), []
    batch.__enter__()
    lean = _GRAD_STREAM_BF16
    if lean:
        g32 = None
    first = stack.layers[0]
    try:
        for layer, s, sv in zip(reversed(stack.layers), reversed(sh), reversed(saved)):
            x, m1, r1, h, qkv, o, lse, x_mid, m2, r2, h2, z, act = sv
            at, mlp = layer.self_attn, layer.mlp
            linear_bwd_params(g16, act, mlp.fc2.weight, mlp.fc2.bias)
            dz, _, _ = ops.gemm_nt(g16, s["w2T"], None, act=ops.ACT_DQUICK_GELU, aux_in=z)
            linear_bwd_params(dz, h2, mlp.fc1.weight, mlp.fc1.bias)
            dh2, _, _ = ops.gemm_nt(dz, s["w1T"], None)
            dg, accg = vec_grad(layer.layer_norm2.weight)
            db, _ = vec_grad(layer.layer_norm2.bias)
            gm32, gm16, _, _ = ops.layernorm_bwd(dh2, x_mid, layer.layer_norm2.weight, m2, r2, dres=g16 if lean else g32,
                                                 dgamma=dg, dbeta=db, accumulate=accg, want_f32=not lean,
                                                 need_param_grads=dg is not None)
            linear_bwd_params(gm16, o, at.out_proj.weight, at.out_proj.bias)
            do, _, _ = ops.gemm_nt(gm16, s["woT"], None)
            dqkv = torch.empty_like(qkv)
            ops.attention_bwd(qkv[:, :C], qkv[:, C:2 * C], qkv[:, 2 * C:], o, do, lse, B, H, S, S, D, scale, causal=causal,
                              kbias=kbias, dq=dqkv[:, :C], dk=dqkv[:, C:2 * C], dv=dqkv[:, 2 * C:])
            for j, proj in enumerate((at.q_proj, at.k_proj, at.v_proj)):
                linear_bwd_params(dqkv[:, j * C:(j + 1) * C], h, proj.weight, proj.bias)
            dh, _, _ = ops.gemm_nt(dqkv, s["wqkvT"], None)
            dg, accg = vec_grad(layer.layer_norm1.weight)
            db, _ = vec_grad(layer.layer_norm1.bias)
            g32, g16, _, _ = ops.layernorm_bwd(dh, x, layer.layer_norm1.weight, m1, r1, dres=gm16 if lean else gm32,
                                               dgamma=dg, dbeta=db, accumulate=accg,
                                               want_f32=(not lean) or (final_f32 and layer is first),
                                               need_param_grads=dg is not None)
            waiting.append(layer)
            if len(waiting) >= pair:
                batch.flush()
                if on_layer_done is not None:
                    for done in waiting:
                        on_layer_done(done)
                waiting = []
    finally:
        batch.__exit__(None, None, None)
    if on_layer_done is not None:
        for done in waiting:
            on_layer_done(done)
    return g32, g16


def _remap_legacy_keys(state_dict, prefix, inner: str):
    legacy = prefix + "enc." + inner + "."
    for k in [k for k in state_dict if k.startswith(legacy)]:
        state_dict[prefix + "enc." + k[len(legacy):]] = state_dict.pop(k)
    state_dict.pop(prefix + "enc.embeddings.position_ids", None)


def _interp_matrix_bicubic(n_in: int, n_out: int) -> torch.Tensor:
    A = -0.75
    c1 = lambda x: ((A + 2) * x - (A + 3)) * x * x + 1
    c2 = lambda x: ((A * x - 5 * A) * x + 8 * A) * x - 4 * A
    U = torch.zeros(n_out, n_in, dtype=torch.float64)
    scale = n_in / n_out
    for o in range(n_out):
        src = scale * (o + 0.5) - 0.5
        i0 = math.floor(src)
        t = src - i0
        for k, wgt in enumerate((c2(t + 1), c1(t), c1(1 - t), c2(2 - t))):
            U[o, min(max(i0 - 1 + k, 0), n_in - 1)] += wgt
    return U


VIT_PRETRAINED_SIZE = 224


class _VisionFn(torch.autograd.Function):
    @staticmethod
    def forward(ctx, pixel_values, anchor, mod, keep_cls, save):
        out, saved = mod._fwd(pixel_values, keep_cls, save)
        ctx.mod, ctx.saved, ctx.keep_cls = mod, saved, keep_cls
        return out

    @staticmethod
    def backward(ctx, gout):
        ctx.mod._bwd(gout.contiguous(), ctx.saved, ctx.keep_cls)
        ctx.saved = None
        return None, None, None, None, None


class ImageEncoderCLIP(HipModule):

    keep_cls = False

    def __init__(self, in_size: int, patch_size: int = 16, arch: ClipArch | None = None) -> None:
        super().__init__()
        self.in_size, self.patch_size = in_size, patch_size
        if arch is None:
            if patch_size == 16:
                arch = VIT_B16
            elif patch_size == 14:
                arch = VIT_L14
            else:
                raise ValueError("ImageEncoderCLIP: only patch_size 16 (ViT-B/16) and 14 (ViT-L/14) have defaults")
        self.arch = arch
        self.enc = _VisionParams(arch, in_size, patch_size)
        _clip_init(self.enc, arch)

    def hidden_size(self) -> int:
        return self.arch.hidden

    def pos_emebedding_interpolate(self, tgt_size: int, ignore_index: int = 1, weight: torch.Tensor | None = None) -> torch.Tensor:
        w = (self.enc.embeddings.position_embedding.weight if weight is None else weight).detach().double().cpu()
        old = VIT_PRETRAINED_SIZE // self.patch_size
        keep, grid = w[:ignore_index], w[ignore_index:].reshape(old, old, -1)
        U = _interp_matrix_bicubic(old, tgt_size)
        new = torch.einsum("yi,ijc,xj->yxc", U, grid, U).reshape(tgt_size * tgt_size, -1)
        return torch.cat([keep, new], dim=0).float()

    def _load_from_state_dict(self, state_dict, prefix, *args, **kwargs):
        _remap_legacy_keys(state_dict, prefix, "vision_model")
        key = prefix + "enc.embeddings.position_embedding.weight"
        old_rows = (VIT_PRETRAINED_SIZE // self.patch_size) ** 2 + 1
        mine = self.enc.embeddings.position_embedding.weight.shape[0]
        if key in state_dict and state_dict[key].shape[0] == old_rows and mine != old_rows:
            state_dict[key] = self.pos_emebedding_interpolate(self.in_size // self.patch_size, weight=state_dict[key])
        super()._load_from_state_dict(state_dict, prefix, *args, **kwargs)

    def _build_shadows(self, device):
        a = self.arch
        per, entries = _stack_shadows(self.enc.encoder, a, device)
        k = 3 * self.patch_size ** 2
        kpad = (k + 63) // 64 * 64
        wp = torch.zeros(a.hidden, kpad, dtype=torch.bfloat16, device=device)
        entries.append((self.enc.embeddings.patch_embedding.weight.view(a.hidden, k), wp[:, :k], None))
        return dict(layers=per, wpatch=wp, kpad=kpad), entries

    def _fwd(self, pixel_values, keep_cls, save):
        require_cuda(pixel_values, "pixel_values")
        a, sh = self.arch, self._ensure_ready()
        B = pixel_values.shape[0]
        G = self.in_size // self.patch_size
        P = G * G
        if pixel_values.shape[-1] != self.in_size or pixel_values.shape[-2] != self.in_size:
            raise ValueError(f"Input image size ({pixel_values.shape[-2]}*{pixel_values.shape[-1]}) doesn't match "
                             f"model ({self.in_size}*{self.in_size}).")
        emb = self.enc.embeddings
        cols = ops.patchify(pixel_values.float().contiguous(), self.patch_size, sh["kpad"])
        _, pe, _ = ops.gemm_nt(cols, sh["wpatch"], None, out_bf16=None, out_f32=True)
        x0 = ops.vit_embed_fwd(pe, emb.class_embedding, emb.position_embedding.weight, B, P)
        xb, xf, m0, r0 = ops.layernorm_fwd(x0, self.enc.pre_layrnorm.weight, self.enc.pre_layrnorm.bias, a.eps,
                                           save_stats=save, out_bf16=True if _RESID_BF16 else None,
                                           out_f32=None if _RESID_BF16 else True)
        x, saved = _stack_fwd(xb if _RESID_BF16 else xf, self.enc.encoder, sh["layers"], a, B, P + 1, None, False, save)
        if keep_cls and x.dtype == torch.float32:
            out = x.view(B, P + 1, a.hidden)
        else:
            n, off = (P + 1, 0) if keep_cls else (P, 1)
            out = torch.empty(B * n, a.hidden, dtype=torch.float32, device=x.device)
            ops.rows_copy(x, P + 1, off, n, 0, B, n, dst_f32=out)
            out = out.view(B, n, a.hidden)
        return out, (dict(cols=cols, x0=x0, m0=m0, r0=r0, layers=saved, B=B, P=P) if save else None)

    def _bwd(self, gout, saved, keep_cls):
        a, sh = self.arch, self._sh
        B, P = saved["B"], saved["P"]
        C = a.hidden
        if keep_cls:
            g32 = gout.reshape(B * (P + 1), C).float()
            g16 = ops.cast_bf16(g32)
        elif _GRAD_STREAM_BF16:
            g32 = None
            g16 = torch.zeros(B * (P + 1), C, dtype=torch.bfloat16, device=gout.device)
            ops.rows_copy(gout.reshape(B * P, C).float().contiguous(), P, 0, P + 1, 1, B, P, dst_bf16=g16)
        else:
            g32 = torch.zeros(B * (P + 1), C, dtype=torch.float32, device=gout.device)
            ops.rows_copy(gout.reshape(B * P, C).float().contiguous(), P, 0, P + 1, 1, B, P, dst_f32=g32)
            g16 = ops.cast_bf16(g32)
        g32, g16 = _stack_bwd(g32, g16, self.enc.encoder, sh["layers"], saved["layers"], a, B, P + 1, None, False,
                              on_layer_done=self._part_grads_ready if self._part_ready_cb is not None else None,
                              final_f32=False)
        dg, accg = vec_grad(self.enc.pre_layrnorm.weight)
        db, _ = vec_grad(self.enc.pre_layrnorm.bias)
        dx0, _, _, _ = ops.layernorm_bwd(g32 if g32 is not None else g16, saved["x0"], self.enc.pre_layrnorm.weight, saved["m0"], saved["r0"],
                                         dgamma=dg, dbeta=db, accumulate=accg, want_bf16=False,
                                         need_param_grads=dg is not None)
        emb = self.enc.embeddings
        gpos, accp = grad_buf(emb.position_embedding.weight)
        gcls, accc = grad_buf(emb.class_embedding)
        if accp != accc:
            raise RuntimeError("lc2is_amd: inconsistent gradient state of the ViT embeddings")
        dpatch = ops.vit_embed_bwd(dx0, gpos, gcls, B, P, accumulate=accp)
        gw, accw = grad_buf(emb.patch_embedding.weight)
        k = 3 * self.patch_size ** 2
        if sh["kpad"] == k:
            ops.gemm_tn(dpatch, saved["cols"], gw.view(C, k), accumulate=accw)
        else:
            tmp = ops.gemm_tn(dpatch, saved["cols"])
            gw.view(C, k).copy_(tmp[:, :k]) if not accw else gw.view(C, k).add_(tmp[:, :k])
        self._grads_ready()

    def forward(self, pixel_values: torch.Tensor) -> torch.Tensor:
        anchor = self.enc.pre_layrnorm.weight
        return _VisionFn.apply(pixel_values, anchor, self, self.keep_cls, torch.is_grad_enabled() and anchor.requires_grad)


class ImageEncoderCLIPFull(ImageEncoderCLIP):

    keep_cls = True


class _TextFn(torch.autograd.Function):
    @staticmethod
    def forward(ctx, input_ids, attention_mask, anchor, mod, save):
        out, saved = mod._fwd(input_ids, attention_mask, save)
        ctx.mod, ctx.saved = mod, saved
        return out

    @staticmethod
    def backward(ctx, gout):
        here = torch.cuda.current_stream(gout.device)
        gout.record_stream(here)
        torch.autograd.Variable._execution_engine.queue_callback(
            lambda: torch.cuda.current_stream(gout.device).wait_stream(here))
        ctx.mod._bwd(gout.contiguous(), ctx.saved)
        ctx.saved = None
        return None, None, None, None, None


class TextEncoderCLIP(HipModule):

    def __init__(self, patch_size: int = 16, arch: ClipArch | None = None) -> None:
        super().__init__()
        self.patch_size = patch_size
        if arch is None:
            arch = TEXT_B if patch_size == 16 else TEXT_L
        self.arch = arch
        self.enc = _TextParams(arch)
        _clip_init(self.enc, arch)

    def hidden_size(self) -> int:
        return self.arch.hidden

    def _load_from_state_dict(self, state_dict, prefix, *args, **kwargs):
        _remap_legacy_keys(state_dict, prefix, "text_model")
        super()._load_from_state_dict(state_dict, prefix, *args, **kwargs)

    def _build_shadows(self, device):
        per, entries = _stack_shadows(self.enc.encoder, self.arch, device)
        return dict(layers=per), entries

    def _fwd(self, input_ids, attention_mask, save):
        require_cuda(input_ids, "input_ids")
        a, sh = self.arch, self._ensure_ready()
        B, L = input_ids.shape
        if L > a.max_pos:
            raise ValueError(f"Sequence length must be less than max_position_embeddings (got `sequence length`: "
                             f"{L} and max_position_embeddings: {a.max_pos}")
        emb = self.enc.embeddings
        ids = input_ids.contiguous()
        x = ops.text_embed_fwd(ids, emb.token_embedding.weight, emb.position_embedding.weight)
        if _RESID_BF16:
            x = ops.cast_bf16(x)
        kbias = None
# ... 44 lines not shown
```

### lc2is_amd/ops.py

```python
from __future__ import annotations

import ctypes as C
import os

import torch

from . import _lib

ACT_NONE, ACT_QUICK_GELU, ACT_RELU, ACT_DQUICK_GELU, ACT_DRELU, ACT_QUICK_GELU_GRAD, ACT_MUL_AUX = 0, 1, 2, 3, 4, 5, 6
ACT_GELU_ERF, ACT_DGELU_ERF, ACT_ADD_AUX = 7, 8, 9

_P, _I, _F, _Z, _L, _U64 = C.c_void_p, C.c_int, C.c_float, C.c_size_t, C.c_long, C.c_ulonglong
_ARGTYPES = {
    "lc2is_gemm_nt_bf16": [_P, _I, _P, _I, _P, _P, _I, _P, _I, _P, _I, _P, _I, _P, _I, _I, _I, _I, _I, _I, _P],
    "lc2is_gemm_nt_ln_xchg_bytes": [_I, _I],
    "lc2is_gemm_nt_ln_bf16": [_P, _I, _P, _I, _P, _P, _I, _P, _I, _P, _P, _F, _P, _I, _P, _P, _P, _Z, _I, _I, _I, _P],
    "lc2is_gemm_nt_bf16_batched": [_P, _I, _L, _P, _I, _L, _P, _I, _L, _P, _I, _L, _I, _I, _I, _I, _P],
    "lc2is_transpose_bf16_batched": [_P, _I, _L, _P, _I, _L, _I, _I, _I, _P],
    "lc2is_gemm_tn_workspace_bytes": [_I, _I, _I],
    "lc2is_gemm_tn_bf16": [_P, _I, _P, _I, _P, _I, _P, _I, _I, _I, _I, _P, _Z, _P],
    "lc2is_colsum_workspace_bytes": [_I, _I],
    "lc2is_colsum_bf16": [_P, _I, _P, _I, _I, _I, _P, _Z, _P],
    "lc2is_layernorm_fwd": [_P, _I, _I, _P, _P, _P, _I, _P, _I, _P, _P, _I, _I, _F, _P],
    "lc2is_layernorm_bwd_partials": [_I, _I],
    "lc2is_ln_partials_reduce": [_P, _I, _P],
    "lc2is_layernorm_bwd_workspace_bytes": [_I, _I],
    "lc2is_layernorm_bwd": [_P, _I, _P, _I, _P, _I, _I, _P, _P, _P, _P, _I, _I, _P, _I, _P, _I, _P, _P, _I, _I, _I,
                            _P, _Z, _P],
    "lc2is_attention_fwd": [_P, _I, _P, _I, _P, _I, _P, _I, _P, _P, _I, _I, _I, _I, _I, _F, _I, _P],
    "lc2is_attention_bwd": [_P, _I, _P, _I, _P, _I, _P, _I, _P, _I, _P, _I, _P, _I, _P, _I, _P, _P, _P,
                            _I, _I, _I, _I, _I, _F, _I, _P],
    "lc2is_attention_fwd_dropout": [_P, _I, _P, _I, _P, _I, _P, _I, _P, _P, _I, _I, _I, _I, _I, _F, _I, _F, _U64, _P],
    "lc2is_attention_bwd_dropout": [_P, _I, _P, _I, _P, _I, _P, _I, _P, _I, _P, _I, _P, _I, _P, _I, _P, _P, _P,
                                    _I, _I, _I, _I, _I, _F, _I, _F, _U64, _P],
    "lc2is_dropout_rows_f32": [_P, _I, _P, _I, _P, _I, _P, _I, _I, _I, _I, _F, _U64, _P],
    "lc2is_dropout_rows_bf16": [_P, _I, _P, _I, _I, _I, _F, _U64, _P],
    "lc2is_dropout_mask": [_P, _L, _I, _F, _U64, _P],
    "lc2is_shadow_refresh": [_P, _I, _I, _P],
    "lc2is_set_cu_budget": [_I],
    "lc2is_get_cu_budget": [],
    "lc2is_cast_f32_bf16": [_P, _I, _P, _I, _I, _I, _P],
    "lc2is_transpose_bf16": [_P, _I, _P, _I, _I, _I, _P],
    "lc2is_patchify": [_P, _P, _I, _I, _I, _I, _I, _P],
    "lc2is_vit_embed_fwd": [_P, _I, _P, _P, _P, _I, _I, _I, _I, _P],
    "lc2is_vit_embed_bwd": [_P, _I, _P, _P, _P, _I, _I, _I, _I, _I, _P],
    "lc2is_text_embed_fwd": [_P, _P, _P, _P, _I, _I, _I, _I, _I, _P],
    "lc2is_text_embed_bwd": [_P, _P, _I, _P, _P, _I, _I, _I, _I, _I, _P],
    "lc2is_rows_copy_bf16": [_P, _I, _I, _P, _P, _I, _I, _I, _I, _I, _P],
    "lc2is_rows_copy_f32": [_P, _I, _I, _P, _P, _I, _I, _I, _I, _I, _P],
    "lc2is_sgd_step": [_P, _P, _P, _Z, _F, _F, _F, _F, _P],
    "lc2is_adamw_step": [_P, _P, _P, _P, _Z, _F, _F, _F, _F, _F, _I, _F, _P],
    "lc2is_grad_sumsq_blocks": [_Z],
    "lc2is_grad_sumsq_workspace_bytes": [_Z],
    "lc2is_grad_sumsq": [_P, _Z, _P, _Z, _P],
    "lc2is_optim_ctrl_update": [_P, _P, _P, _I, _P, _I, _F, _F, _I, _F, _F, _P],
    "lc2is_sgd_step_ctrl": [_P, _P, _P, _Z, _P, _F, _F, _I, _P],
    "lc2is_adamw_step_ctrl": [_P, _P, _P, _P, _Z, _P, _F, _F, _F, _F, _I, _P],
    "lc2is_sgd_step_groups": [_P, _P, _P, _Z, _P, _P, _P, _I, _F, _I, _P],
    "lc2is_adamw_step_groups": [_P, _P, _P, _P, _Z, _P, _P, _P, _I, _F, _F, _F, _I, _P],
    "lc2is_head_upsample_ce_workspace_bytes": [_I, _I, _I, _I, _I, _I, _I],
    "lc2is_head_upsample_ce": [_P, _I, _P, _P, _P, _P, _I, _I, _I, _I, _I, _I, C.c_long, _F, _P, _Z, _P],
    "lc2is_ce_nchw_fwd": [_P, _P, _P, _P, _I, _I, C.c_long, C.c_long, _P],
    "lc2is_ce_nchw_bwd": [_P, _P, _P, _P, _F, _P, _I, _I, C.c_long, C.c_long, _P],
    "lc2is_head_upsample_ce_opts": [_P, _I, _P, _P, _P, _P, _I, _I, _I, _I, _I, _I, C.c_long, _F, _P, _F, _P, _Z, _P],
    "lc2is_ce_nchw_fwd_opts": [_P, _P, _P, _P, _P, _I, _I, C.c_long, C.c_long, _P, _F, _P],
    "lc2is_ce_nchw_fwd_workspace_bytes": [_I, C.c_long],
    "lc2is_ce_nchw_fwd_ordered": [_P, _P, _P, _P, _P, _I, _I, C.c_long, C.c_long, _P, _F, _P, _Z, _P],
    "lc2is_ce_nchw_bwd_opts": [_P, _P, _P, _P, _F, _P, _P, _I, _I, C.c_long, C.c_long, _P, _F, _P],
    "lc2is_upsample_bwd_nchw": [_P, _P, _I, _I, _I, _I, _I, _I, _I, _P],
    "lc2is_bilinear_up_fwd": [_P, _P, _P, _I, _I, _I, _I, _I, _P],
    "lc2is_bilinear_up_bwd": [_P, _P, _P, _I, _I, _I, _I, _I, _I, _P],
    "lc2is_sr_gather": [_P, _P, _I, _I, _I, _I, _I, _P],
    "lc2is_sr_scatter_add_f32": [_P, _P, _I, _I, _I, _I, _P],
    "lc2is_l2norm_fwd": [_P, _P, _P, _P, _I, _I, _F, _P],
    "lc2is_l2norm_bwd": [_P, _P, _P, _P, _I, _I, _F, _P],
    "lc2is_add_n": [_P, _P, _P, _P, _P, _P, _Z, _P],
    "lc2is_rows_ce": [_P, _P, _P, _P, _P, _F, _I, _I, _I, _P],
    "lc2is_cols_ce": [_P, _P, _P, _P, _F, _I, _I, _I, _I, _P],
    "lc2is_npair": [_P, _P, _P, _P, _I, _I, _I, _I, _P],
    "lc2is_miou_counts": [_P, _P, _P, _I, _I, _I, _I, _I, _P],
    "lc2is_resize_argmax_workspace_bytes": [_L, _I],
    "lc2is_resize_argmax": [_P, _I, _I, _I, _I, _I, _P, _L, _L, _P, _I, _P, _P, _P, _Z, _P],
    "lc2is_npair_bwd": [_P, _P, _P, _P, _P, _P, _P, _P, _I, _I, _I, _I, _P],
    "lc2is_gemm_tn_grouped_workspace_bytes": [_P, _I],
    "lc2is_gemm_tn_grouped": [_P, _I, _P, _Z, _P],
    "lc2is_release_captured_tables": [],
    "lc2is_captured_tables_mark": [],
    "lc2is_release_captured_tables_range": [_I, _I],
    "lc2is_rows_gather": [_P, _I, _I, _P, _I, _I, _P, _P, _I, _I, _I, _P],
    "lc2is_resample_u8": [_P, _I, _I, _I, _P, _I, _I, _P, _P, _I, _P],
    "lc2is_gather2d_u8": [_P, _I, _I, _I, _P, _I, _I, _P, _P, _P],
    "lc2is_crop_lut": [_P, _I, _I, _I, _I, _I, _I, _P, _P, _P, _P, _P],
    "lc2is_swin_attn_fwd": [_P, _I, _P, _I, _P, _P, _I, _I, _I, _I, _I, _I, _I, _I, _I, _F, _P],
    "lc2is_swin_bias_table_grad": [_P, _P, _P, _P, _I, _I, _I, _I, _P],
    "lc2is_swin_attn_bwd_workspace_bytes": [_I, _I, _I],
    "lc2is_swin_attn_bwd": [_P, _I, _P, _I, _P, _I, _P, _P, _P, _I, _P, _I, _I, _I, _I, _I, _I, _I, _I, _I, _I, _F,
                            _P, _Z, _P],
}
_bound = {}


def _fn(name: str):
    f = _bound.get(name)
    if f is None:
        f = getattr(_lib.load(), name)
        if name in _ARGTYPES:
            f.argtypes = _ARGTYPES[name]
        if name.endswith("_workspace_bytes"):
            f.restype = C.c_size_t
        _bound[name] = f
    return f


def _stream() -> int:
    return torch.cuda.current_stream().cuda_stream


def _chk(t: torch.Tensor | None, dtype, name: str, ndim: int | None = 2):
    if t is None:
        return
    if not t.is_cuda:
        raise RuntimeError(f"lc2is_amd: {name} must be a CUDA(HIP) tensor; there is no CPU path")
    if t.dtype != dtype:
        raise RuntimeError(f"lc2is_amd: {name} must be {dtype}, got {t.dtype}")
    if ndim is not None and t.dim() != ndim:
        raise RuntimeError(f"lc2is_amd: {name} must be {ndim}-D, got shape {tuple(t.shape)}")
    if t.dim() >= 1 and t.stride(-1) != 1:
        raise RuntimeError(f"lc2is_amd: {name} must have unit stride in its last dimension")


def _ptr(t: torch.Tensor | None) -> int | None:
    return None if t is None else t.data_ptr()


def _ld(t: torch.Tensor | None) -> int:
    return 0 if t is None else (t.stride(0) if t.dim() == 2 else t.shape[-1])


def _out(spec, shape, dtype, dev):
    if spec is True:
        return torch.empty(shape, dtype=dtype, device=dev)
    if spec is None or spec is False:
        return None
    return spec



_ws_cache: dict = {}


def workspace(nbytes: int, device, tag: str = "default") -> torch.Tensor:
    key = (str(device), _stream(), tag)
    buf = _ws_cache.get(key)
    if buf is None or buf.numel() < nbytes:
        buf = torch.empty(max(int(nbytes), 1 << 20), dtype=torch.uint8, device=device)
        _ws_cache[key] = buf
    return buf


def gemm_nt(a: torch.Tensor, w: torch.Tensor, bias: torch.Tensor | None = None, *, act: int = ACT_NONE,
            resid: torch.Tensor | None = None, aux_in: torch.Tensor | None = None,
            out_bf16: torch.Tensor | bool | None = True, out_f32: torch.Tensor | bool | None = None,
            aux_out: torch.Tensor | bool | None = None, tile_cfg: int = 0):
    _chk(a, torch.bfloat16, "a"); _chk(w, torch.bfloat16, "w")
    if resid is not None and resid.dtype == torch.bfloat16:
        if act != ACT_NONE or aux_in is not None:
            raise RuntimeError("lc2is_amd.gemm_nt: a bf16 residual needs act == ACT_NONE and no aux_in")
        act, aux_in, resid = ACT_ADD_AUX, resid, None
    _chk(bias, torch.float32, "bias", 1); _chk(resid, torch.float32, "resid"); _chk(aux_in, torch.bfloat16, "aux_in")
    M, K = a.shape
    N, K2 = w.shape
    if K2 != K:
        raise RuntimeError(f"lc2is_amd.gemm_nt: K mismatch {K} vs {K2}")
    if bias is not None and bias.numel() != N:
        raise RuntimeError("lc2is_amd.gemm_nt: bias length != N")
    dev = a.device
    ob = _out(out_bf16, (M, N), torch.bfloat16, dev)
    of = _out(out_f32, (M, N), torch.float32, dev)
    ao = _out(aux_out, (M, N), torch.bfloat16, dev)
    _chk(ob, torch.bfloat16, "out_bf16"); _chk(of, torch.float32, "out_f32"); _chk(ao, torch.bfloat16, "aux_out")
    rc = _fn("lc2is_gemm_nt_bf16")(_ptr(a), _ld(a), _ptr(w), _ld(w), _ptr(bias), _ptr(resid), _ld(resid),
                                   _ptr(aux_in), _ld(aux_in), _ptr(ob), _ld(ob), _ptr(of), _ld(of), _ptr(ao),
                                   _ld(ao), M, N, K, act, tile_cfg, _stream())
    _lib.check(rc, f"gemm_nt M={M} N={N} K={K}")
    return ob, of, ao


_xchg_cache = {}
_LN_FUSE = os.environ.get("LC2IS_LN_FUSE", "1") != "0"
_LN_FUSE_MIN_ROWS = int(os.environ.get("LC2IS_LN_FUSE_MIN_ROWS", "0"))

# ... 17 lines not shown
        raise RuntimeError("lc2is_amd.gemm_nt_ln: shape mismatch")
    dev = a.device
    xf = _out(out_f32 if out_f32 is not None else True, (M, N), torch.float32, dev)
    h = _out(ln_out if ln_out is not None else True, (M, N), torch.bfloat16, dev)
    mean = torch.empty((M,), dtype=torch.float32, device=dev) if save_stats else None
    rstd = torch.empty((M,), dtype=torch.float32, device=dev) if save_stats else None
    nb = _fn("lc2is_gemm_nt_ln_xchg_bytes")(M, N)
    xc = None
    if nb:
        key = (str(dev), _stream())
        xc = _xchg_cache.get(key)
        if xc is None or xc.numel() < nb:
            xc = torch.zeros(max(int(nb), 1 << 21), dtype=torch.uint8, device=dev)
            _xchg_cache[key] = xc
    rc = _fn("lc2is_gemm_nt_ln_bf16")(_ptr(a), _ld(a), _ptr(w), _ld(w), _ptr(bias), _ptr(resid), _ld(resid), _ptr(xf), _ld(xf),
                                      _ptr(gamma), _ptr(beta), float(eps), _ptr(h), _ld(h), _ptr(mean), _ptr(rstd), _ptr(xc),
                                      xc.numel() if xc is not None else 0, M, N, K, _stream())
    _lib.check(rc, f"gemm_nt_ln M={M} N={N} K={K}")
    return xf, h, mean, rstd


def gemm_nt_batched(a: torch.Tensor, w: torch.Tensor, *, out_bf16: torch.Tensor | bool | None = None,
                    out_f32: torch.Tensor | bool | None = True):
    _chk(a, torch.bfloat16, "a", 3); _chk(w, torch.bfloat16, "w", 3)
    Bn, M, K = a.shape
    if w.shape[0] != Bn or w.shape[2] != K:
        raise RuntimeError(f"lc2is_amd.gemm_nt_batched: shape mismatch {tuple(a.shape)} vs {tuple(w.shape)}")
    N = w.shape[1]
    ob = _out(out_bf16, (Bn, M, N), torch.bfloat16, a.device)
    of = _out(out_f32, (Bn, M, N), torch.float32, a.device)
    _chk(ob, torch.bfloat16, "out_bf16", 3); _chk(of, torch.float32, "out_f32", 3)
    st = lambda t: (0, 0) if t is None else (t.stride(1), t.stride(0))
    rc = _fn("lc2is_gemm_nt_bf16_batched")(_ptr(a), a.stride(1), a.stride(0), _ptr(w), w.stride(1), w.stride(0),
                                           _ptr(ob), *st(ob), _ptr(of), *st(of), M, N, K, Bn, _stream())
    _lib.check(rc, f"gemm_nt_batched B={Bn} M={M} N={N} K={K}")
    return ob, of


def transpose_bf16_batched(x: torch.Tensor) -> torch.Tensor:
    _chk(x, torch.bfloat16, "x", 3)
    Bn, R, Cc = x.shape
    out = torch.empty((Bn, Cc, R), dtype=torch.bfloat16, device=x.device)
    rc = _fn("lc2is_transpose_bf16_batched")(_ptr(x), x.stride(1), x.stride(0), _ptr(out), R, Cc * R, R, Cc, Bn, _stream())
    _lib.check(rc, f"transpose_bf16_batched B={Bn} R={R} C={Cc}")
    return out


def gemm_tn(dy: torch.Tensor, x: torch.Tensor, dw: torch.Tensor | None = None, accumulate: bool = False,
            db: torch.Tensor | None = None):
    _chk(dy, torch.bfloat16, "dy"); _chk(x, torch.bfloat16, "x")
    M, N = dy.shape
    M2, K = x.shape
    if M2 != M:
        raise RuntimeError("lc2is_amd.gemm_tn: M mismatch")
    if dw is None:
        dw = torch.empty((N, K), dtype=torch.float32, device=dy.device)
        accumulate = False
    _chk(dw, torch.float32, "dw"); _chk(db, torch.float32, "db", 1)
    if db is not None and db.numel() != N:
        raise RuntimeError("lc2is_amd.gemm_tn: db length != N")
    nbytes = _fn("lc2is_gemm_tn_workspace_bytes")(M, N, K)
    ws = workspace(nbytes, dy.device, "gemm_tn")
    rc = _fn("lc2is_gemm_tn_bf16")(_ptr(dy), _ld(dy), _ptr(x), _ld(x), _ptr(dw), _ld(dw), _ptr(db), M, N, K,
                                   int(accumulate), _ptr(ws), ws.numel(), _stream())
    _lib.check(rc, f"gemm_tn M={M} N={N} K={K}")
    return dw


class TnProblem(C.Structure):
    _fields_ = [("dY", C.c_void_p), ("X", C.c_void_p), ("dW", C.c_void_p), ("db", C.c_void_p), ("ldy", C.c_int),
                ("ldx", C.c_int), ("ldw", C.c_int), ("M", C.c_int), ("N", C.c_int), ("K", C.c_int), ("accumulate", C.c_int)]


GROUP_MAX = 128


_GROUP_MIN_ROWS = int(os.environ.get("LC2IS_GROUP_MIN_ROWS", "4096"))


def gemm_tn_groupable(dy: torch.Tensor, x: torch.Tensor) -> bool:
    return dy.shape[1] % 8 == 0 and x.shape[1] % 8 == 0 and dy.shape[0] >= _GROUP_MIN_ROWS


def gemm_tn_grouped(problems):
    if not 1 <= len(problems) <= GROUP_MAX:
        raise RuntimeError(f"lc2is_amd.gemm_tn_grouped: 1..{GROUP_MAX} problems per launch")
    arr = (TnProblem * len(problems))()
    for i, (dy, x, dw, db, acc) in enumerate(problems):
        _chk(dy, torch.bfloat16, "dy"); _chk(x, torch.bfloat16, "x"); _chk(dw, torch.float32, "dw"); _chk(db, torch.float32, "db", 1)
        M, N = dy.shape
        if x.shape[0] != M or tuple(dw.shape) != (N, x.shape[1]) or (db is not None and db.numel() != N):
            raise RuntimeError("lc2is_amd.gemm_tn_grouped: shape mismatch")
        arr[i] = TnProblem(_ptr(dy), _ptr(x), _ptr(dw), _ptr(db), _ld(dy), _ld(x), _ld(dw), M, N, x.shape[1], int(acc))
    nbytes = _fn("lc2is_gemm_tn_grouped_workspace_bytes")(arr, len(problems))
    ws = workspace(nbytes, problems[0][0].device, "gemm_tn_grouped")
    rc = _fn("lc2is_gemm_tn_grouped")(arr, len(problems), _ptr(ws), ws.numel(), _stream())
    _lib.check(rc, f"gemm_tn_grouped n={len(problems)}")


def release_captured_tables() -> int:
    f = _fn("lc2is_release_captured_tables")
    f.restype = C.c_int
    return int(f())


def captured_tables_mark() -> int:
    return int(_fn("lc2is_captured_tables_mark")())


def release_captured_tables_range(first: int, last: int) -> int:
    return int(_fn("lc2is_release_captured_tables_range")(int(first), int(last)))


def colsum(dy: torch.Tensor, db: torch.Tensor | None = None, accumulate: bool = False):
    _chk(dy, torch.bfloat16, "dy")
    M, N = dy.shape
    if db is None:
        db = torch.empty((N,), dtype=torch.float32, device=dy.device)
        accumulate = False
    _chk(db, torch.float32, "db", 1)
    nbytes = _fn("lc2is_colsum_workspace_bytes")(M, N)
    ws = workspace(nbytes, dy.device, "colsum")
    rc = _fn("lc2is_colsum_bf16")(_ptr(dy), _ld(dy), _ptr(db), M, N, int(accumulate), _ptr(ws), ws.numel(),
                                  _stream())
    _lib.check(rc, f"colsum M={M} N={N}")
    return db


def layernorm_fwd(x: torch.Tensor, gamma: torch.Tensor, beta: torch.Tensor | None, eps: float = 1e-5, *,
                  save_stats: bool = True, out_bf16: torch.Tensor | bool | None = True,
                  out_f32: torch.Tensor | bool | None = None):
    xb = x.dtype == torch.bfloat16
    _chk(x, torch.bfloat16 if xb else torch.float32, "x"); _chk(gamma, torch.float32, "gamma", 1); _chk(beta, torch.float32, "beta", 1)
    M, Cc = x.shape
    dev = x.device
    yb = _out(out_bf16, (M, Cc), torch.bfloat16, dev)
    yf = _out(out_f32, (M, Cc), torch.float32, dev)
    mean = torch.empty((M,), dtype=torch.float32, device=dev) if save_stats else None
    rstd = torch.empty((M,), dtype=torch.float32, device=dev) if save_stats else None
    rc = _fn("lc2is_layernorm_fwd")(_ptr(x), _ld(x), int(xb), _ptr(gamma), _ptr(beta), _ptr(yb), _ld(yb), _ptr(yf),
                                    _ld(yf), _ptr(mean), _ptr(rstd), M, Cc, float(eps), _stream())
    _lib.check(rc, f"layernorm_fwd M={M} C={Cc}")
    return yb, yf, mean, rstd


def layernorm_bwd(dy: torch.Tensor, x: torch.Tensor, gamma: torch.Tensor, mean: torch.Tensor,
                  rstd: torch.Tensor, *, dres: torch.Tensor | None = None, dgamma: torch.Tensor | None = None,
                  dbeta: torch.Tensor | None = None, accumulate: bool = False, want_f32: bool = True,
                  want_bf16: bool = True, need_param_grads: bool = True):
    M, Cc = x.shape
    dev = x.device
    dyb = dy if dy.dtype == torch.bfloat16 else None
    dyf = dy if dy.dtype == torch.float32 else None
    if dyb is None and dyf is None:
        raise RuntimeError("lc2is_amd.layernorm_bwd: dy must be bf16 or fp32")
    xb = x.dtype == torch.bfloat16
    rb = dres is not None and dres.dtype == torch.bfloat16
    _chk(dyb, torch.bfloat16, "dy"); _chk(dyf, torch.float32, "dy"); _chk(x, torch.bfloat16 if xb else torch.float32, "x")
    _chk(dres, torch.bfloat16 if rb else torch.float32, "dres")
    dxf = torch.empty((M, Cc), dtype=torch.float32, device=dev) if want_f32 else None
    dxb = torch.empty((M, Cc), dtype=torch.bfloat16, device=dev) if want_bf16 else None
    if need_param_grads:
        if dgamma is None:
            dgamma = torch.empty((Cc,), dtype=torch.float32, device=dev)
            accumulate = False
            if dbeta is None:
                dbeta = torch.empty((Cc,), dtype=torch.float32, device=dev)
    nbytes = _fn("lc2is_layernorm_bwd_workspace_bytes")(M, Cc)
    defer = _ln_defer if (need_param_grads and (dgamma is not None or dbeta is not None)) else None
    if defer is not None:
        ws = torch.empty(max(int(nbytes), 16), dtype=torch.uint8, device=dev)
        defer.append((ws, _fn("lc2is_layernorm_bwd_partials")(M, Cc), Cc, dgamma, dbeta, bool(accumulate)))
        pg, pb = None, None
    else:
        ws = workspace(nbytes, dev, "ln_bwd")
        pg, pb = dgamma, dbeta
    rc = _fn("lc2is_layernorm_bwd")(_ptr(dyb), _ld(dyb), _ptr(dyf), _ld(dyf), _ptr(x), _ld(x), int(xb), _ptr(gamma),
                                    _ptr(mean), _ptr(rstd), _ptr(dres), _ld(dres), int(rb), _ptr(dxf), _ld(dxf),
                                    _ptr(dxb), _ld(dxb), _ptr(pg), _ptr(pb), int(accumulate), M, Cc,
                                    _ptr(ws), ws.numel(), _stream())
# ... 47 lines not shown


def attention_fwd(q: torch.Tensor, k: torch.Tensor, v: torch.Tensor, B: int, H: int, Sq: int, Sk: int, D: int,
                  scale: float, *, causal: bool = False, kbias: torch.Tensor | None = None,
                  save_lse: bool = True, out: torch.Tensor | None = None, dropout_p: float = 0.0, seed: int = 0):
    _chk(q, torch.bfloat16, "q"); _chk(k, torch.bfloat16, "k"); _chk(v, torch.bfloat16, "v")
    _chk(kbias, torch.float32, "kbias")
    if q.shape != (B * Sq, H * D) or k.shape != (B * Sk, H * D) or v.shape != (B * Sk, H * D):
        raise RuntimeError("lc2is_amd.attention_fwd: q/k/v shapes do not match B,H,S,D")
    if kbias is not None and (kbias.shape != (B, Sk) or not kbias.is_contiguous()):
        raise RuntimeError("lc2is_amd.attention_fwd: kbias must be contiguous [B,Sk]")
    o = out if out is not None else torch.empty((B * Sq, H * D), dtype=torch.bfloat16, device=q.device)
    _chk(o, torch.bfloat16, "out")
    lse = torch.empty((B, H, Sq), dtype=torch.float32, device=q.device) if save_lse else None
    if dropout_p > 0.0:
        rc = _fn("lc2is_attention_fwd_dropout")(_ptr(q), _ld(q), _ptr(k), _ld(k), _ptr(v), _ld(v), _ptr(o), _ld(o),
                                                _ptr(lse), _ptr(kbias), B, H, Sq, Sk, D, float(scale), int(causal),
                                                float(dropout_p), int(seed), _stream())
    else:
        rc = _fn("lc2is_attention_fwd")(_ptr(q), _ld(q), _ptr(k), _ld(k), _ptr(v), _ld(v), _ptr(o), _ld(o),
                                        _ptr(lse), _ptr(kbias), B, H, Sq, Sk, D, float(scale), int(causal),
                                        _stream())
    _lib.check(rc, f"attention_fwd B={B} H={H} Sq={Sq} Sk={Sk} D={D}")
    return o, lse


def attention_bwd(q, k, v, o, do, lse2, B: int, H: int, Sq: int, Sk: int, D: int, scale: float, *,
                  causal: bool = False, kbias: torch.Tensor | None = None, dq=None, dk=None, dv=None,
                  dropout_p: float = 0.0, seed: int = 0):
    for t, n in ((q, "q"), (k, "k"), (v, "v"), (o, "o"), (do, "do")):
        _chk(t, torch.bfloat16, n)
    _chk(lse2, torch.float32, "lse2", 3); _chk(kbias, torch.float32, "kbias")
    dev = q.device
    dq = dq if dq is not None else torch.empty((B * Sq, H * D), dtype=torch.bfloat16, device=dev)
    dk = dk if dk is not None else torch.empty((B * Sk, H * D), dtype=torch.bfloat16, device=dev)
    dv = dv if dv is not None else torch.empty((B * Sk, H * D), dtype=torch.bfloat16, device=dev)
    for t, n in ((dq, "dq"), (dk, "dk"), (dv, "dv")):
        _chk(t, torch.bfloat16, n)
    delta = torch.empty((B, H, Sq), dtype=torch.float32, device=dev)
    args = (_ptr(q), _ld(q), _ptr(k), _ld(k), _ptr(v), _ld(v), _ptr(o), _ld(o), _ptr(do), _ld(do), _ptr(dq), _ld(dq),
            _ptr(dk), _ld(dk), _ptr(dv), _ld(dv), _ptr(lse2), _ptr(delta), _ptr(kbias), B, H, Sq, Sk, D, float(scale),
            int(causal))
    if dropout_p > 0.0:
        rc = _fn("lc2is_attention_bwd_dropout")(*args, float(dropout_p), int(seed), _stream())
    else:
        rc = _fn("lc2is_attention_bwd")(*args, _stream())
    _lib.check(rc, f"attention_bwd B={B} H={H} Sq={Sq} Sk={Sk} D={D}")
    return dq, dk, dv


def dropout_rows_f32(x: torch.Tensor, p: float, seed: int, *, resid: torch.Tensor | None = None,
                     out_f32: torch.Tensor | bool | None = True, out_bf16: torch.Tensor | bool | None = None,
                     rows_per_sample: int = 0):
    _chk(x, torch.float32, "x"); _chk(resid, torch.float32, "resid")
    M, Cc = x.shape
    yf = _out(out_f32, (M, Cc), torch.float32, x.device)
    yb = _out(out_bf16, (M, Cc), torch.bfloat16, x.device)
    _chk(yf, torch.float32, "out_f32"); _chk(yb, torch.bfloat16, "out_bf16")
    rc = _fn("lc2is_dropout_rows_f32")(_ptr(x), _ld(x), _ptr(resid), _ld(resid), _ptr(yf), _ld(yf), _ptr(yb), _ld(yb), M, Cc,
                                       int(rows_per_sample), float(p), int(seed), _stream())
    _lib.check(rc, f"dropout_rows_f32 M={M} C={Cc}")
    return yf, yb


def dropout_rows_bf16(x: torch.Tensor, p: float, seed: int, out: torch.Tensor | None = None):
    _chk(x, torch.bfloat16, "x")
    y = x if out is None else out
    _chk(y, torch.bfloat16, "out")
    M, Cc = x.shape
    rc = _fn("lc2is_dropout_rows_bf16")(_ptr(x), _ld(x), _ptr(y), _ld(y), M, Cc, float(p), int(seed), _stream())
    _lib.check(rc, f"dropout_rows_bf16 M={M} C={Cc}")
    return y


def dropout_mask(rows: int, cols: int, p: float, seed: int, device) -> torch.Tensor:
    out = torch.empty((rows, cols), dtype=torch.uint8, device=device)
    _lib.check(_fn("lc2is_dropout_mask")(_ptr(out), rows, cols, float(p), int(seed), _stream()), "dropout_mask")
    return out


INTERP_BICUBIC, INTERP_BILINEAR = 0, 1


class ShadowDesc(C.Structure):
    _fields_ = [("src", C.c_void_p), ("dst", C.c_void_p), ("dstT", C.c_void_p), ("N", C.c_int), ("K", C.c_int),
                ("ld_dst", C.c_int), ("ld_dstT", C.c_int), ("tile_start", C.c_int), ("flags", C.c_int)]


class ShadowTable:

    def __init__(self, entries, device):
        descs = (ShadowDesc * len(entries))()
        start = 0
        self._keep = []
        for i, (src, dst, dstT) in enumerate(entries):
            if src.dim() == 1:
                src = src.unsqueeze(0)
                dst = dst.unsqueeze(0) if dst is not None and dst.dim() == 1 else dst
            f32copy = dst is not None and dst.dtype == torch.float32
            _chk(src, torch.float32, "shadow src")
            _chk(dst, torch.float32 if f32copy else torch.bfloat16, "shadow dst")
            _chk(dstT, torch.bfloat16, "shadow dstT")
            if f32copy and dstT is not None:
                raise RuntimeError("lc2is_amd: fp32 shadow copies have no transposed twin")
            if not src.is_contiguous():
                raise RuntimeError("lc2is_amd: shadow source must be contiguous")
            N, K = src.shape
            if K % 4 or (dstT is not None and N % 4):
                raise RuntimeError(f"lc2is_amd: shadow shape [{N},{K}] not supported")
            if dst is not None and tuple(dst.shape) != (N, K):
                raise RuntimeError("lc2is_amd: shadow dst shape mismatch")
            if dstT is not None and tuple(dstT.shape) != (K, N):
                raise RuntimeError("lc2is_amd: shadow dstT shape mismatch")
            descs[i] = ShadowDesc(src.data_ptr(), _ptr(dst), _ptr(dstT), N, K, _ld(dst), _ld(dstT), start, int(f32copy))
            start += ((N + 63) // 64) * ((K + 63) // 64)
            self._keep.append((src, dst, dstT))
        self.n = len(entries)
        self.total_tiles = start
        raw = bytes(descs)
        self.dev = torch.frombuffer(bytearray(raw), dtype=torch.uint8).to(device)

    def refresh(self):
        rc = _fn("lc2is_shadow_refresh")(self.dev.data_ptr(), self.n, self.total_tiles, _stream())
        _lib.check(rc, "shadow_refresh")


def cast_bf16(src: torch.Tensor, out: torch.Tensor | None = None):
    _chk(src, torch.float32, "src")
    M, Cc = src.shape
    out = out if out is not None else torch.empty((M, Cc), dtype=torch.bfloat16, device=src.device)
    _chk(out, torch.bfloat16, "out")
    _lib.check(_fn("lc2is_cast_f32_bf16")(_ptr(src), _ld(src), _ptr(out), _ld(out), M, Cc, _stream()), "cast")
    return out


def transpose_bf16(src: torch.Tensor, out: torch.Tensor | None = None):
    _chk(src, torch.bfloat16, "src")
    R, Cc = src.shape
    out = out if out is not None else torch.empty((Cc, R), dtype=torch.bfloat16, device=src.device)
    _chk(out, torch.bfloat16, "out")
    _lib.check(_fn("lc2is_transpose_bf16")(_ptr(src), _ld(src), _ptr(out), _ld(out), R, Cc, _stream()),
               "transpose")
    return out


def patchify(pixels: torch.Tensor, patch: int, kpad: int | None = None):
    _chk(pixels, torch.float32, "pixel_values", 4)
    if not pixels.is_contiguous() or pixels.shape[1] != 3:
        raise RuntimeError("lc2is_amd.patchify: pixel_values must be contiguous [B,3,H,W]")
    B, _, H, W = pixels.shape
    G = H // patch
    k = 3 * patch * patch
    kpad = kpad or ((k + 63) // 64) * 64
    out = torch.empty((B * G * G, kpad), dtype=torch.bfloat16, device=pixels.device)
    _lib.check(_fn("lc2is_patchify")(_ptr(pixels), _ptr(out), kpad, B, H, W, patch, _stream()), "patchify")
    return out


def vit_embed_fwd(patch_f32, cls, pos, B: int, P: int):
    _chk(patch_f32, torch.float32, "patch"); _chk(cls, torch.float32, "cls", 1); _chk(pos, torch.float32, "pos")
    Cc = patch_f32.shape[1]
    x = torch.empty((B * (P + 1), Cc), dtype=torch.float32, device=patch_f32.device)
    _lib.check(_fn("lc2is_vit_embed_fwd")(_ptr(patch_f32), _ld(patch_f32), _ptr(cls), _ptr(pos), _ptr(x), Cc, B,
                                          P, Cc, _stream()), "vit_embed_fwd")
    return x


def vit_embed_bwd(dx, dpos, dcls, B: int, P: int, accumulate: bool = False):
    _chk(dx, torch.float32, "dx"); _chk(dpos, torch.float32, "dpos"); _chk(dcls, torch.float32, "dcls", 1)
    Cc = dx.shape[1]
    dpatch = torch.empty((B * P, Cc), dtype=torch.bfloat16, device=dx.device)
    _lib.check(_fn("lc2is_vit_embed_bwd")(_ptr(dx), _ld(dx), _ptr(dpos), _ptr(dcls), _ptr(dpatch), Cc, B, P, Cc,
                                          int(accumulate), _stream()), "vit_embed_bwd")
    return dpatch


def text_embed_fwd(ids, tok, pos):
    _chk(ids, torch.int64, "input_ids"); _chk(tok, torch.float32, "tok"); _chk(pos, torch.float32, "pos")
    if not ids.is_contiguous():
        raise RuntimeError("lc2is_amd.text_embed_fwd: input_ids must be contiguous")
    B, L = ids.shape
    V, Cc = tok.shape
    x = torch.empty((B * L, Cc), dtype=torch.float32, device=tok.device)
    _lib.check(_fn("lc2is_text_embed_fwd")(_ptr(ids), _ptr(tok), _ptr(pos), _ptr(x), Cc, B, L, Cc, V, _stream()),
               "text_embed_fwd")
    return x


def text_embed_bwd(ids, dx, dtok, dpos, accumulate: bool = False):
    _chk(ids, torch.int64, "input_ids"); _chk(dx, torch.float32, "dx")
    B, L = ids.shape
    V, Cc = dtok.shape
    _lib.check(_fn("lc2is_text_embed_bwd")(_ptr(ids), _ptr(dx), _ld(dx), _ptr(dtok), _ptr(dpos), B, L, Cc, V,
                                           int(accumulate), _stream()), "text_embed_bwd")


def rows_copy(src, S_src: int, src_off: int, S_dst: int, dst_off: int, B: int, n: int, *, dst_f32=None,
              dst_bf16=None):
    sb = src.dtype == torch.bfloat16
    _chk(src, torch.bfloat16 if sb else torch.float32, "src")
    Cc = src.shape[1]
    if not src.is_contiguous() or src.shape[0] != B * S_src:
        raise RuntimeError("lc2is_amd.rows_copy: src must be contiguous [B*S_src, C]")
    for t in (dst_f32, dst_bf16):
        if t is not None and (not t.is_contiguous() or tuple(t.shape) != (B * S_dst, Cc)):
            raise RuntimeError("lc2is_amd.rows_copy: dst must be contiguous [B*S_dst, C]")
    _lib.check(_fn("lc2is_rows_copy_bf16" if sb else "lc2is_rows_copy_f32")(_ptr(src), S_src, src_off, _ptr(dst_f32), _ptr(dst_bf16),
                                                                            S_dst, dst_off, B, n, Cc, _stream()), "rows_copy")


def sgd_step(params, grads, momentum_buf, lr, momentum=0.0, weight_decay=0.0, grad_scale=1.0):
    _chk(params, torch.float32, "params", 1); _chk(grads, torch.float32, "grads", 1)
    _lib.check(_fn("lc2is_sgd_step")(_ptr(params), _ptr(grads), _ptr(momentum_buf), params.numel(), lr, momentum,
                                     weight_decay, grad_scale, _stream()), "sgd_step")


def adamw_step(params, grads, m, v, lr, beta1, beta2, eps, weight_decay, step, grad_scale=1.0):
    _chk(params, torch.float32, "params", 1); _chk(grads, torch.float32, "grads", 1)
    _lib.check(_fn("lc2is_adamw_step")(_ptr(params), _ptr(grads), _ptr(m), _ptr(v), params.numel(), lr, beta1,
                                       beta2, eps, weight_decay, int(step), grad_scale, _stream()), "adamw_step")


OPTIM_CTRL_WORDS = 12
(CTRL_CALLS, CTRL_APPLIED, CTRL_SKIPPED, CTRL_FINITE, CTRL_GRAD_NORM, CTRL_CLIP_COEF, CTRL_LR, CTRL_BC1, CTRL_BC2, CTRL_GRAD_MUL,
 CTRL_APPLY) = range(11)


def _chk_ctrl(ctrl):
    _chk(ctrl, torch.int32, "ctrl", 1)
    if ctrl.numel() != OPTIM_CTRL_WORDS:
        raise RuntimeError(f"lc2is_amd: ctrl must be an int32 [{OPTIM_CTRL_WORDS}] control block (lc2is_optim_ctrl)")


def _chk_same_numel(name, params, *others):
    for t in others:
        if t is not None:
            _chk(t, torch.float32, name + " buffer", 1)
            if t.numel() != params.numel():
                raise RuntimeError(f"lc2is_amd.{name}: every buffer must have params' {params.numel()} elements, got {t.numel()}")


def grad_sumsq(grads):
    _chk(grads, torch.float32, "grads", 1)
    n = grads.numel()
    nb = _fn("lc2is_grad_sumsq_blocks")(n)
    if nb <= 0:
        raise RuntimeError(f"lc2is_amd.grad_sumsq: numel must be a positive multiple of 4, got {n}")
    need = _fn("lc2is_grad_sumsq_workspace_bytes")(n)
    ws = workspace(need, grads.device, "grad_sumsq")
    _lib.check(_fn("lc2is_grad_sumsq")(_ptr(grads), n, _ptr(ws), ws.numel(), _stream()), "grad_sumsq")
    return ws[:4 * nb].view(torch.float32), ws[4 * nb:8 * nb].view(torch.int32)


def optim_ctrl_update(ctrl, partials, flags, lr_table, *, grad_scale=1.0, max_norm=float("inf"), skip_nonfinite=False,
                      beta1=0.0, beta2=0.0):
    _chk_ctrl(ctrl); _chk(partials, torch.float32, "partials", 1); _chk(flags, torch.int32, "flags", 1)
    _chk(lr_table, torch.float32, "lr_table", 1)
    if flags.numel() != partials.numel() or not partials.is_contiguous() or not flags.is_contiguous():
        raise RuntimeError("lc2is_amd.optim_ctrl_update: partials and flags must be contiguous and of one length")
    if lr_table.numel() < 1 or not lr_table.is_contiguous():
        raise RuntimeError("lc2is_amd.optim_ctrl_update: lr_table must be a non-empty contiguous fp32 tensor")
    _lib.check(_fn("lc2is_optim_ctrl_update")(_ptr(ctrl), _ptr(partials), _ptr(flags), partials.numel(), _ptr(lr_table),
                                              lr_table.numel(), grad_scale, max_norm, int(bool(skip_nonfinite)), beta1, beta2,
                                              _stream()), "optim_ctrl_update")


def sgd_step_ctrl(params, grads, momentum_buf, ctrl, momentum=0.0, weight_decay=0.0, reverse=False):
    _chk(params, torch.float32, "params", 1); _chk_same_numel("sgd_step_ctrl", params, grads, momentum_buf); _chk_ctrl(ctrl)
    _lib.check(_fn("lc2is_sgd_step_ctrl")(_ptr(params), _ptr(grads), _ptr(momentum_buf), params.numel(), _ptr(ctrl), momentum,
                                          weight_decay, int(bool(reverse)), _stream()), "sgd_step_ctrl")


def adamw_step_ctrl(params, grads, m, v, ctrl, beta1, beta2, eps, weight_decay, reverse=False):
    _chk(params, torch.float32, "params", 1); _chk_same_numel("adamw_step_ctrl", params, grads, m, v); _chk_ctrl(ctrl)
    _lib.check(_fn("lc2is_adamw_step_ctrl")(_ptr(params), _ptr(grads), _ptr(m), _ptr(v), params.numel(), _ptr(ctrl), beta1,
                                            beta2, eps, weight_decay, int(bool(reverse)), _stream()), "adamw_step_ctrl")


GROUP_GRANULE, MAX_PARAM_GROUPS, GROUP_SKIP = 64, 255, 255


def _chk_groups(name, params, granule_group, groups):
    _chk(granule_group, torch.uint8, "granule_group", 1); _chk(groups, torch.float32, "groups", 2)
    if granule_group is None or groups is None:
        raise RuntimeError(f"lc2is_amd.{name}: granule_group and groups are required")
    n = params.numel()
    if n == 0 or n % GROUP_GRANULE:
        raise RuntimeError(f"lc2is_amd.{name}: numel must be a positive multiple of {GROUP_GRANULE}, got {n}")
    if not params.is_contiguous() or not granule_group.is_contiguous() or granule_group.numel() != n // GROUP_GRANULE:
        raise RuntimeError(f"lc2is_amd.{name}: granule_group must be a contiguous uint8 [{n // GROUP_GRANULE}] map (one id per "
                           f"{GROUP_GRANULE} elements), got {tuple(granule_group.shape)}")
    if not groups.is_contiguous() or groups.shape[1] != 2 or not 1 <= groups.shape[0] <= MAX_PARAM_GROUPS:
        raise RuntimeError(f"lc2is_amd.{name}: groups must be a contiguous fp32 [ngroups, 2] table of (lr_scale, weight_decay), "
                           f"1 <= ngroups <= {MAX_PARAM_GROUPS}, got {tuple(groups.shape)}")


def sgd_step_groups(params, grads, momentum_buf, ctrl, granule_group, groups, momentum=0.0, reverse=False):
    _chk(params, torch.float32, "params", 1); _chk_same_numel("sgd_step_groups", params, grads, momentum_buf); _chk_ctrl(ctrl)
    _chk_groups("sgd_step_groups", params, granule_group, groups)
    _lib.check(_fn("lc2is_sgd_step_groups")(_ptr(params), _ptr(grads), _ptr(momentum_buf), params.numel(), _ptr(ctrl),
                                            _ptr(granule_group), _ptr(groups), groups.shape[0], momentum, int(bool(reverse)),
                                            _stream()), "sgd_step_groups")

# ... 442 lines not shown
```

### lc2is_amd/step.py

```python
from __future__ import annotations

import math
import os
import re

import torch
from torch import nn

from . import ops
from .nn.base import HipModule, ParamArena


_DEFAULT_LR = 1e-5


def lr_table_from_torch(make_scheduler, base_lr: float, steps: int) -> torch.Tensor:
    if steps < 1:
        raise ValueError("lr_table_from_torch: steps must be >= 1")
    opt = torch.optim.SGD([torch.nn.Parameter(torch.zeros(1))], lr=base_lr)
    sched = make_scheduler(opt)
    rates = []
    for i in range(steps):
        rates.append(opt.param_groups[0]["lr"])
        if i + 1 < steps:
            opt.step()
            sched.step()
    return torch.tensor(rates, dtype=torch.float64).to(torch.float32)


def _lr_table(lr_schedule, schedule_steps, lr) -> torch.Tensor:
    if lr_schedule is None:
        if schedule_steps is not None:
            raise ValueError("TrainStep: schedule_steps needs a callable lr_schedule")
        return torch.tensor([lr], dtype=torch.float64).to(torch.float32)
    if callable(lr_schedule):
        if schedule_steps is None or int(schedule_steps) < 1:
            raise ValueError("TrainStep: a callable lr_schedule needs schedule_steps=N >= 1 (the table is tabulated on the host)")
        table = torch.tensor([float(lr_schedule(i)) for i in range(int(schedule_steps))], dtype=torch.float64)
    else:
        if schedule_steps is not None:
            raise ValueError("TrainStep: schedule_steps goes with a callable lr_schedule, not with a table")
        table = torch.as_tensor(lr_schedule).detach().to("cpu", torch.float64)
        if table.dim() != 1:
            raise ValueError("TrainStep: lr_schedule must be a 1-D sequence or tensor of rates")
    if table.numel() == 0:
        raise ValueError("TrainStep: lr_schedule is empty")
    if not bool(torch.isfinite(table).all()) or bool((table < 0).any()):
        raise ValueError("TrainStep: lr_schedule must hold finite, non-negative rates")
    table = table.to(torch.float32)
    if lr != _DEFAULT_LR and torch.tensor(lr, dtype=torch.float64).to(torch.float32) != table[0]:
        raise ValueError(f"TrainStep: lr={lr} conflicts with lr_schedule, which starts at {float(table[0])}; give the rates "
                         "through lr_schedule alone")
    return table


_GROUP_KEYS = {"params", "lr_scale", "weight_decay"}
_MAX_GROUPS = ops.MAX_PARAM_GROUPS


def _resolve_param_groups(model: nn.Module, param_groups, weight_decay: float):
    named, seen = [], set()
    for name, prm in model.named_parameters():
        if id(prm) not in seen:
            seen.add(id(prm))
            named.append((name, prm))
    by_name, name_of = dict(named), {id(prm): name for name, prm in named}
    if isinstance(param_groups, dict) or not hasattr(param_groups, "__iter__"):
        raise ValueError("TrainStep: param_groups must be a sequence of dicts")
    param_groups = list(param_groups)
    if not param_groups:
        raise ValueError("TrainStep: param_groups is empty (use None for no groups)")
    if len(param_groups) > _MAX_GROUPS:
        raise ValueError(f"TrainStep: {len(param_groups)} param_groups; more than {_MAX_GROUPS} groups are not supported")
    groups, group_of = [], {}
    for gi, g in enumerate(param_groups):
        if not isinstance(g, dict) or "params" not in g:
            raise ValueError(f"TrainStep: param_groups[{gi}] must be a dict with a 'params' entry")
        unknown = set(g) - _GROUP_KEYS
        if unknown:
            raise ValueError(f"TrainStep: param_groups[{gi}] has unknown keys {sorted(unknown)} (known: {sorted(_GROUP_KEYS)})")
        lr_scale, wd = float(g.get("lr_scale", 1.0)), float(g.get("weight_decay", weight_decay))
        for key, val in (("lr_scale", lr_scale), ("weight_decay", wd)):
            if not math.isfinite(val) or val < 0.0:
                raise ValueError(f"TrainStep: param_groups[{gi}] {key} must be finite and >= 0, got {val}")
        members = g["params"]
        members = [members] if isinstance(members, (str, torch.Tensor)) else list(members)
        if not members:
            raise ValueError(f"TrainStep: param_groups[{gi}] has empty params")
        names = []
        for m in members:
            if isinstance(m, str):
                if m not in by_name:
                    raise ValueError(f"TrainStep: param_groups[{gi}]: '{m}' is not a parameter of the model")
                prm = by_name[m]
            elif isinstance(m, torch.Tensor) and id(m) in name_of:
                prm = m
            else:
                what = f"a tensor of shape {tuple(m.shape)}" if isinstance(m, torch.Tensor) else repr(m)
                raise ValueError(f"TrainStep: param_groups[{gi}]: {what} is not a parameter of the model")
            if id(prm) in group_of:
                raise ValueError(f"TrainStep: parameter '{name_of[id(prm)]}' is in two groups (param_groups[{group_of[id(prm)]}] "
                                 f"and param_groups[{gi}])" if group_of[id(prm)] != gi else
                                 f"TrainStep: parameter '{name_of[id(prm)]}' is listed twice in param_groups[{gi}]")
            group_of[id(prm)] = gi
            names.append(name_of[id(prm)])
        groups.append(dict(names=tuple(names), numel=sum(by_name[n].numel() for n in names), lr_scale=lr_scale, weight_decay=wd))
    rest = [name for name, prm in named if id(prm) not in group_of]
    if rest:
        if len(groups) + 1 > _MAX_GROUPS:
            raise ValueError(f"TrainStep: {len(groups)} param_groups plus the implicit group of the {len(rest)} parameters named in "
                             f"none; more than {_MAX_GROUPS} groups are not supported")
        for n in rest:
            group_of[id(by_name[n])] = len(groups)
        groups.append(dict(names=tuple(rest), numel=sum(by_name[n].numel() for n in rest), lr_scale=1.0,
                           weight_decay=float(weight_decay)))
    return groups, group_of


_TOWER_LAYER = re.compile(r"^(.*)\.encoder\.layers\.(\d+)\.")


def make_param_groups(model: nn.Module, *, weight_decay: float, no_decay=True, lr_scales=None, layer_decay=None) -> list:
    extra = tuple(no_decay) if isinstance(no_decay, (tuple, list)) else ()
    lr_scales = dict(lr_scales or {})
    named, seen = [], set()
    for name, prm in model.named_parameters():
        if id(prm) not in seen:
            seen.add(id(prm))
            named.append((name, prm))
    depth = {}
    for name, _ in named:
        m = _TOWER_LAYER.match(name)
        if m:
            depth[m.group(1)] = max(depth.get(m.group(1), 0), int(m.group(2)) + 1)
    merged = {}
    for name, prm in named:
        wd = float(weight_decay)
        if no_decay and (prm.dim() == 1 or name.endswith(("position_embedding.weight", "token_embedding.weight"))
                         or any(sub in name for sub in extra)):
            wd = 0.0
        scale, best = 1.0, -1
        for prefix, f in lr_scales.items():
            if name.startswith(prefix) and len(prefix) > best:
                scale, best = float(f), len(prefix)
        if layer_decay is not None:
            m = _TOWER_LAYER.match(name)
            if m:
                scale *= float(layer_decay) ** (depth[m.group(1)] - int(m.group(2)))
            else:
                for tower, L in depth.items():
                    if name.startswith((tower + ".embeddings.", tower + ".pre_layrnorm.")):
                        scale *= float(layer_decay) ** (L + 1)
        merged.setdefault((scale, wd), []).append(name)
    return [dict(params=names, lr_scale=scale, weight_decay=wd) for (scale, wd), names in merged.items()]


class TrainStep:

    def __init__(self, model: nn.Module, *, optimizer: str = "sgd", lr: float = _DEFAULT_LR, momentum: float = 0.0,
                 weight_decay: float = 0.0, betas=(0.9, 0.999), eps: float = 1e-8, reducer=None,
                 ignore_index: int | None = None, criterion: nn.Module | None = None, lr_schedule=None,
                 schedule_steps: int | None = None, max_grad_norm: float | None = None, skip_nonfinite: bool = False,
                 device_state: bool = False, param_groups=None) -> None:
        device_path = bool(device_state or skip_nonfinite or lr_schedule is not None or max_grad_norm is not None
                           or param_groups is not None)
        groups = None
        if param_groups is not None:
            groups, group_of = _resolve_param_groups(model, param_groups, weight_decay)
        if max_grad_norm is not None and not float(max_grad_norm) > 0.0:
            raise ValueError(f"TrainStep: max_grad_norm must be > 0 (or None / inf for no clipping), got {max_grad_norm}")
        table = _lr_table(lr_schedule, schedule_steps, lr) if (device_path or schedule_steps is not None) else None
        self._loss_opts = False
        if criterion is not None:
            from .nn.loss import AuxiliaryLoss, CrossEntropyLoss
            if not isinstance(criterion, (CrossEntropyLoss, nn.CrossEntropyLoss)) or isinstance(criterion, AuxiliaryLoss):
                raise TypeError("TrainStep: criterion must be a CrossEntropyLoss (lc2is_amd.nn or torch.nn)")
            if ignore_index is not None and ignore_index != -100:
                raise ValueError("TrainStep: give ignore_index through the criterion, not as a TrainStep argument too")
            if criterion.reduction == "none":
                raise ValueError("TrainStep: a training step needs a scalar loss; criterion reduction='none' cannot train")
            ignore_index = criterion.ignore_index
            self._loss_opts = (criterion.weight is not None or criterion.label_smoothing != 0.0
                               or criterion.reduction != "mean")
        self.criterion = criterion
        self.model = model
        self.arena = ParamArena(model)
        self.kind = optimizer.lower()
        if self.kind not in ("sgd", "adamw"):
            raise ValueError("TrainStep: optimizer must be 'sgd' or 'adamw'")
        self.lr, self.momentum, self.weight_decay, self.betas, self.eps = lr, momentum, weight_decay, betas, eps
        dev = self.arena.flat.device
        self.mom = torch.zeros_like(self.arena.flat) if (self.kind == "sgd" and momentum != 0.0) else None
        if self.kind == "adamw":
            self.m, self.v = torch.zeros_like(self.arena.flat), torch.zeros_like(self.arena.flat)
        self.t = 0
        self.reducer = reducer
        self.ignore_index = -100 if ignore_index is None else ignore_index
        self._hip_modules = [m for m in model.modules() if isinstance(m, HipModule)]
        if reducer is not None:
            reducer.attach(model, self.arena)
        self._dev = dev
        self._ctrl = None
        if device_path:
            self._ctrl = torch.zeros(ops.OPTIM_CTRL_WORDS, dtype=torch.int32, device=dev)
            self._ctrl_f = self._ctrl.view(torch.float32)
            self.lr_table = table.to(dev)
            self.max_grad_norm = float("inf") if max_grad_norm is None else float(max_grad_norm)
            self.skip_nonfinite = bool(skip_nonfinite)
            self.reverse_walk = False
        self._groups = groups
        if groups is not None:
            self.arena.set_groups([group_of[id(p)] for p in self.arena.params], len(groups))
            self._group_table = torch.tensor([[g["lr_scale"], g["weight_decay"]] for g in groups], dtype=torch.float32).to(dev)

    def _ctrl_view(self, word: int, as_float: bool) -> torch.Tensor:
        if self._ctrl is None:
            raise RuntimeError("TrainStep: this accessor needs the device-held path (lr_schedule / max_grad_norm / "
                               "skip_nonfinite / device_state=True)")
        return (self._ctrl_f if as_float else self._ctrl)[word]

    @property
    def last_grad_norm(self) -> torch.Tensor:
        return self._ctrl_view(ops.CTRL_GRAD_NORM, True)

    @property
    def last_clip_coef(self) -> torch.Tensor:
        return self._ctrl_view(ops.CTRL_CLIP_COEF, True)

    @property
    def last_lr(self) -> torch.Tensor:
        return self._ctrl_view(ops.CTRL_LR, True)

    @property
    def skipped_steps(self) -> torch.Tensor:
        return self._ctrl_view(ops.CTRL_SKIPPED, False)

    @property
    def applied_steps(self) -> torch.Tensor:
        return self._ctrl_view(ops.CTRL_APPLIED, False)

    @property
    def param_groups(self):
        return None if self._groups is None else tuple(dict(g) for g in self._groups)

    def step(self, inputs: dict, labels: torch.Tensor) -> torch.Tensor:
        arena = self.arena
        arena.zero_grad(set_to_none=True)
        if self.reducer is not None:
            self.reducer.begin_step()
        if self._loss_opts:
            c = self.criterion
            loss = self.model.forward_loss(inputs, labels, self.ignore_index, weight=c.weight,
                                           label_smoothing=float(c.label_smoothing), reduction=c.reduction)
        else:
            loss = self.model.forward_loss(inputs, labels, self.ignore_index)
        loss.backward()
        live = arena.finalize_grads()
        gscale = 1.0
        if self.reducer is not None:
            self.reducer.finish_step()
            gscale = 1.0 / self.reducer.world_size
        self.t += 1
        segs = [(0, arena.numel)] if (self.weight_decay == 0.0 or live == [(0, arena.numel)]) else live
        if self._ctrl is not None:
            ctrl = self._ctrl
            b1, b2 = self.betas if self.kind == "adamw" else (0.0, 0.0)
            partials, flags = ops.grad_sumsq(arena.grad)
            ops.optim_ctrl_update(ctrl, partials, flags, self.lr_table, grad_scale=gscale, max_norm=self.max_grad_norm,
                                  skip_nonfinite=self.skip_nonfinite, beta1=b1, beta2=b2)
            if self._groups is not None:
                gmap = arena.group_map()
                if self.kind == "sgd":
                    ops.sgd_step_groups(arena.flat, arena.grad, self.mom, ctrl, gmap, self._group_table, self.momentum,
                                        reverse=self.reverse_walk)
                else:
                    ops.adamw_step_groups(arena.flat, arena.grad, self.m, self.v, ctrl, gmap, self._group_table, self.betas[0],
                                          self.betas[1], self.eps, reverse=self.reverse_walk)
                segs = []
            for lo, hi in segs:
                sl = slice(lo, hi)
                if self.kind == "sgd":
                    ops.sgd_step_ctrl(arena.flat[sl], arena.grad[sl], None if self.mom is None else self.mom[sl], ctrl,
                                      self.momentum, self.weight_decay, reverse=self.reverse_walk)
                else:
                    ops.adamw_step_ctrl(arena.flat[sl], arena.grad[sl], self.m[sl], self.v[sl], ctrl, self.betas[0],
                                        self.betas[1], self.eps, self.weight_decay, reverse=self.reverse_walk)
            segs = []
        for lo, hi in segs:
            sl = slice(lo, hi)
            if self.kind == "sgd":
                ops.sgd_step(arena.flat[sl], arena.grad[sl], None if self.mom is None else self.mom[sl], self.lr,
                             self.momentum, self.weight_decay, gscale)
            else:
                ops.adamw_step(arena.flat[sl], arena.grad[sl], self.m[sl], self.v[sl], self.lr, self.betas[0],
                               self.betas[1], self.eps, self.weight_decay, self.t, gscale)
        for m in self._hip_modules:
            m.invalidate_shadows()
        return loss.detach()

    def capture(self, inputs: dict, labels: torch.Tensor, warmup: int = 2):
        if self.reducer is not None:
            raise RuntimeError("TrainStep.capture: graph capture is only wired for single-GPU steps")
        if self.kind == "adamw" and self._ctrl is None:
            raise RuntimeError("TrainStep.capture: AdamW bias correction is step-dependent; capture supports SGD")
        if hasattr(self.model, "overlap_text") and os.environ.get("LC2IS_GRAPH_OVERLAP", "1") == "0":
            self.model.overlap_text = False
        from .nn.base import DropoutRng
        DropoutRng.last.clear()
        static_in = {k: v.clone() for k, v in inputs.items()}
        static_lb = labels.clone()
        side = torch.cuda.Stream()
        side.wait_stream(torch.cuda.current_stream())
        with torch.cuda.stream(side):
            for _ in range(warmup):
                self.step(static_in, static_lb)
        torch.cuda.current_stream().wait_stream(side)
        torch.cuda.synchronize()
        if DropoutRng.last:
            raise RuntimeError("TrainStep.capture: the model has active dropout / drop-path sites "
                               f"({len(DropoutRng.last)}); their per-step seeds cannot be captured — train eagerly or set the rates to 0")
        prev = getattr(self, "_captured", None)
        if prev is not None:
            prev.release()
        graph = torch.cuda.CUDAGraph()
        t_before = self.t
        mark0 = ops.captured_tables_mark()
        with torch.cuda.graph(graph, stream=side):
            static_loss = self.step(static_in, static_lb)
        mark1 = ops.captured_tables_mark()
        self.t = t_before

        def replay(new_inputs: dict, new_labels: torch.Tensor) -> torch.Tensor:
            for k, v in new_inputs.items():
                if v is not static_in[k]:
                    static_in[k].copy_(v, non_blocking=True)
            if new_labels is not static_lb:
                static_lb.copy_(new_labels, non_blocking=True)
            graph.replay()
            self.t += 1
            return static_loss

        state = {"live": True}

        def release() -> None:
            if not state["live"]:
                return
            state["live"] = False
            torch.cuda.synchronize()
            graph.reset()
            ops.release_captured_tables_range(mark0, mark1)
            if getattr(self, "_captured", None) is replay:
                self._captured = None

        replay.static_inputs, replay.static_labels, replay.graph, replay.release = static_in, static_lb, graph, release
        self._captured = replay
        return replay
```

Measured before the change: 1079 images/s.

## Fuse optimizer update and bf16 shadow refresh into grouped weight-gradient GEMM epilogue

Adds an update-capable grouped TN GEMM: after computing each weight-gradient tile (or in the split-K reduction), the kernel applies the SGD/AdamW step in registers and writes bf16 shadow copies (including a transposed copy via LDS). The later flat optimizer pass then skips these weights through a per-granule skip mask, and the separate shadow refresh is avoided for weights already refreshed in-kernel. The aim is to cut re-reading of gradients, parameters and optimizer state plus the shadow-refresh launches. The cost is a heavier GEMM epilogue with extra registers and LDS traffic, and a skip-map lookup in the optimizer kernels.

```diff
diff --git a/include/lc2is_hip.h b/include/lc2is_hip.h
--- a/include/lc2is_hip.h
+++ b/include/lc2is_hip.h
@@ -64,6 +64,21 @@
 size_t lc2is_gemm_tn_grouped_workspace_bytes(const lc2is_tn_problem* problems, int n);
 int lc2is_gemm_tn_grouped(const lc2is_tn_problem* problems, int n, void* workspace, size_t workspace_bytes,
                           lc2is_stream_t stream);
+#define LC2IS_UPDATE_SGD 1
+#define LC2IS_UPDATE_ADAMW 2
+typedef struct lc2is_tn_update {
+  float* p; float* state0; float* state1;
+  void* dst; void* dstT;
+  int ld_dst, ld_dstT;
+} lc2is_tn_update;
+typedef struct lc2is_update_consts {
+  int kind;
+  int step;
+  float lr, momentum, weight_decay, grad_scale, beta1, beta2, eps;
+} lc2is_update_consts;
+int lc2is_gemm_tn_grouped_update(const lc2is_tn_problem* problems, int n, const lc2is_tn_update* updates,
+                                 const lc2is_update_consts* consts, int* applied, void* workspace, size_t workspace_bytes,
+                                 lc2is_stream_t stream);
 int lc2is_release_captured_tables(void);
 int lc2is_captured_tables_mark(void);
 int lc2is_release_captured_tables_range(int first, int last);
@@ -149,6 +164,11 @@
 int lc2is_adamw_step(float* params, const float* grads, float* exp_avg, float* exp_avg_sq, size_t n, float lr,
                      float beta1, float beta2, float eps, float weight_decay, int step, float grad_scale,
                      lc2is_stream_t stream);
+int lc2is_sgd_step_masked(float* params, const float* grads, float* momentum_buf, size_t n, float lr, float momentum,
+                          float weight_decay, float grad_scale, const unsigned char* skip, lc2is_stream_t stream);
+int lc2is_adamw_step_masked(float* params, const float* grads, float* exp_avg, float* exp_avg_sq, size_t n, float lr,
+                            float beta1, float beta2, float eps, float weight_decay, int step, float grad_scale,
+                            const unsigned char* skip, lc2is_stream_t stream);
 
 size_t lc2is_head_upsample_ce_workspace_bytes(int B, int h, int w, int C, int S, int mode, int want_grad);
 int lc2is_head_upsample_ce(const float* scores_lo, int ld, const int64_t* labels, float* dscores_lo,
diff --git a/lc2is_amd/csrc/gemm_tn.hip b/lc2is_amd/csrc/gemm_tn.hip
--- a/lc2is_amd/csrc/gemm_tn.hip
+++ b/lc2is_amd/csrc/gemm_tn.hip
@@ -1,5 +1,7 @@
 #include "common.h"
 #include "lc2is_hip.h"
+#include "optim_update.h"
+#include <cmath>
 #include <cstdlib>
 #include <mutex>
 #include <vector>
@@ -243,10 +245,94 @@
 #endif
 }
 
+__device__ __forceinline__ uint2 tn_update4(const lc2is_tn_update& up, const UpdConsts& uc, const AdamwScalars& sc, size_t off,
+                                            const float4 gv) {
+  float4 pv = *reinterpret_cast<const float4*>(up.p + off);
+  if (uc.kind == LC2IS_UPD_ADAMW)
+    pv = adamw_update4(sc, pv, gv, up.state0 + off, up.state1 + off);
+  else
+    pv = sgd_update4(pv, gv, up.state0 ? up.state0 + off : nullptr, uc.lr, uc.momentum, uc.wd, uc.gscale);
+  *reinterpret_cast<float4*>(up.p + off) = pv;
+  return make_uint2(pack_bf16x2(pv.x, pv.y), pack_bf16x2(pv.z, pv.w));
+}
+
+template <int MODE>
+__device__ __forceinline__ void tn_update_tile_mode(const f32x4_t (&acc)[8][4], const lc2is_tn_update& up, const UpdConsts& uc,
+                                                    int ldw, int n0, int k0, int wn, int wk, int g, int lane, char* smem) {
+  constexpr int BATCH = MODE == 2 ? 4 : 8;
+  const AdamwScalars sc = adamw_scalars(uc.lr, uc.b1, uc.b2, uc.eps, uc.wd, uc.bc1, uc.bc2, uc.gscale);
+  bf16_t* D = (bf16_t*)up.dst;
+  bf16_t* DT = (bf16_t*)up.dstT;
+#pragma unroll
+  for (int b = 0; b < 4; ++b) {
+    const int nl = wn * 64 + b * 16 + (lane & 15);
+    const size_t row = (size_t)(n0 + nl) * ldw + k0 + wk * 128 + g * 4;
+#pragma unroll
+    for (int a0 = 0; a0 < 8; a0 += BATCH) {
+      float4 pv[BATCH], s0[BATCH], s1[BATCH];
+#pragma unroll
+      for (int j = 0; j < BATCH; ++j) {
+        const size_t off = row + (a0 + j) * 16;
+        pv[j] = *reinterpret_cast<const float4*>(up.p + off);
+        if constexpr (MODE >= 1) s0[j] = *reinterpret_cast<const float4*>(up.state0 + off);
+        if constexpr (MODE == 2) s1[j] = *reinterpret_cast<const float4*>(up.state1 + off);
+      }
+#pragma unroll
+      for (int j = 0; j < BATCH; ++j) {
+        const int a = a0 + j;
+        const int kl = wk * 128 + a * 16 + g * 4;
+        const size_t off = row + a * 16;
+        const f32x4_t v = acc[a][b];
+        const float4 gv = make_float4(v[0], v[1], v[2], v[3]);
+        if constexpr (MODE == 2) {
+          adamw_update4_regs(sc, pv[j], gv, s0[j], s1[j]);
+          *reinterpret_cast<float4*>(up.state0 + off) = s0[j];
+          *reinterpret_cast<float4*>(up.state1 + off) = s1[j];
+        } else if constexpr (MODE == 1) {
+          sgd_update4_regs<true>(pv[j], gv, s0[j], uc.lr, uc.momentum, uc.wd, uc.gscale);
+          *reinterpret_cast<float4*>(up.state0 + off) = s0[j];
+        } else {
+          sgd_update4_regs<false>(pv[j], gv, s0[j], uc.lr, uc.momentum, uc.wd, uc.gscale);
+        }
+        *reinterpret_cast<float4*>(up.p + off) = pv[j];
+        const uint2 pk = make_uint2(pack_bf16x2(pv[j].x, pv[j].y), pack_bf16x2(pv[j].z, pv[j].w));
+        if (D) *reinterpret_cast<uint2*>(D + (size_t)(n0 + nl) * up.ld_dst + k0 + kl) = pk;
+        if (DT) {
+          char* t = smem + kl * 512 + ((nl * 2) ^ (((kl >> 2) & 3) << 5));
+          *reinterpret_cast<bf16_t*>(t) = (bf16_t)(pk.x & 0xffffu);
+          *reinterpret_cast<bf16_t*>(t + 512) = (bf16_t)(pk.x >> 16);
+          *reinterpret_cast<bf16_t*>(t + 1024) = (bf16_t)(pk.y & 0xffffu);
+          *reinterpret_cast<bf16_t*>(t + 1536) = (bf16_t)(pk.y >> 16);
+        }
+      }
+    }
+  }
+  if (!DT) return;
+  __syncthreads();
+#pragma unroll 4
+  for (int it = 0; it < 16; ++it) {
+    const int c = it * 512 + (int)threadIdx.x;
+    const int row = c >> 5, c16 = c & 31;
+    const uint4 v = *reinterpret_cast<const uint4*>(smem + row * 512 + ((c16 ^ (((row >> 2) & 3) << 1)) << 4));
+    *reinterpret_cast<uint4*>(DT + (size_t)(k0 + row) * up.ld_dstT + n0 + c16 * 8) = v;
+  }
+}
+
+__device__ __forceinline__ void tn_update_tile(const f32x4_t (&acc)[8][4], const lc2is_tn_update& up, const UpdConsts& uc,
+                                               int ldw, int n0, int k0, int wn, int wk, int g, int lane, char* smem) {
+  if (uc.kind == LC2IS_UPD_ADAMW)
+    tn_update_tile_mode<2>(acc, up, uc, ldw, n0, k0, wn, wk, g, lane, smem);
+  else if (up.state0)
+    tn_update_tile_mode<1>(acc, up, uc, ldw, n0, k0, wn, wk, g, lane, smem);
+  else
+    tn_update_tile_mode<0>(acc, up, uc, ldw, n0, k0, wn, wk, g, lane, smem);
+}
+
 __device__ __forceinline__ void tn_dma_body(const bf16_t* __restrict__ dY, int ldy, const bf16_t* __restrict__ X, int ldx,
                                             float* out, int ldo, size_t split_stride, float* bias_out,
                                             size_t bias_split_stride, int M, int N, int K, int ntn, int ntk, int chunk,
-                                            int accumulate, int block, char* smem) {
+                                            int accumulate, int block, char* smem,
+                                            const lc2is_tn_update up = lc2is_tn_update{}, const UpdConsts uc = UpdConsts{}) {
   const int tid = threadIdx.x, lane = tid & 63;
   const int wid = __builtin_amdgcn_readfirstlane(tid >> 6);
   const int wk = wid >> 2, wn = wid & 3;
@@ -341,6 +427,7 @@
       *(f32x4_t*)dst = v;
     }
   }
+  if (up.p != nullptr) tn_update_tile(acc, up, uc, ldo, n0, k0, wn, wk, g, lane, smem);
 }
 
 __global__ __launch_bounds__(512, 2) void gemm_tn_dma_kernel(const bf16_t* __restrict__ dY, int ldy,
@@ -361,9 +448,12 @@
   int blk_end;
   int red_end;
   int red_blocks;
+  int upd_where;
+  lc2is_tn_update up;
 };
 struct TnGroup {
   int n, remap;
+  UpdConsts uc;
   TnGroupProb p[TG_MAX];
 };
 
@@ -372,6 +462,7 @@
   int n, pad_[3];
   int blk_end[TG_TBL_MAX];
   int red_end[TG_TBL_MAX];
+  UpdConsts uc;
   TnGroupProb p[TG_TBL_MAX];
 };
 constexpr size_t TG_TBL_BYTES = (sizeof(TnGroupTbl) + 255) / 256 * 256;
@@ -385,7 +476,8 @@
   while (i < n - 1 && bid >= t->blk_end[i]) { begin = t->blk_end[i]; ++i; }
   const TnGroupProb* q = &t->p[i];
   tn_dma_body(q->dY, q->ldy, q->X, q->ldx, q->out, q->ldo, q->split_stride, q->bias_out, q->bias_split_stride, q->M, q->N,
-              q->K, q->ntn, q->ntk, q->chunk, q->splits == 1 ? q->accumulate : 0, bid - begin, smem);
+              q->K, q->ntn, q->ntk, q->chunk, q->splits == 1 ? q->accumulate : 0, bid - begin, smem,
+              q->upd_where == 1 ? q->up : lc2is_tn_update{}, t->uc);
 }
 
 __global__ __launch_bounds__(256) void gemm_tn_grouped_small_kernel(TnGroup g) {
@@ -417,16 +509,16 @@
   while (i < g.n - 1 && bid >= g.p[i].blk_end) { begin = g.p[i].blk_end; ++i; }
   const TnGroupProb& q = g.p[i];
   tn_dma_body(q.dY, q.ldy, q.X, q.ldx, q.out, q.ldo, q.split_stride, q.bias_out, q.bias_split_stride, q.M, q.N, q.K, q.ntn,
-              q.ntk, q.chunk, q.splits == 1 ? q.accumulate : 0, bid - begin, smem);
-}
-
-__device__ __forceinline__ void slab_reduce_grouped_body(const TnGroupProb& q, int b);
+              q.ntk, q.chunk, q.splits == 1 ? q.accumulate : 0, bid - begin, smem, q.upd_where == 1 ? q.up : lc2is_tn_update{}, g.uc);
+}
+
+__device__ __forceinline__ void slab_reduce_grouped_body(const TnGroupProb& q, const UpdConsts& uc, int b);
 
 __global__ __launch_bounds__(256) void slab_reduce_grouped_kernel(TnGroup g) {
   int i = 0, begin = 0;
 #pragma unroll 1
   while (i < g.n - 1 && (int)blockIdx.x >= g.p[i].red_end) { begin = g.p[i].red_end; ++i; }
-  slab_reduce_grouped_body(g.p[i], (int)blockIdx.x - begin);
+  slab_reduce_grouped_body(g.p[i], g.uc, (int)blockIdx.x - begin);
 }
 
 __global__ __launch_bounds__(256) void slab_reduce_grouped_tbl_kernel(const TnGroupTbl* __restrict__ t) {
@@ -434,10 +526,10 @@
   const int n = t->n;
 #pragma unroll 1
   while (i < n - 1 && (int)blockIdx.x >= t->red_end[i]) { begin = t->red_end[i]; ++i; }
-  slab_reduce_grouped_body(t->p[i], (int)blockIdx.x - begin);
-}
-
-__device__ __forceinline__ void slab_reduce_grouped_body(const TnGroupProb& q, int b) {
+  slab_reduce_grouped_body(t->p[i], t->uc, (int)blockIdx.x - begin);
+}
+
+__device__ __forceinline__ void slab_reduce_grouped_body(const TnGroupProb& q, const UpdConsts& uc, int b) {
   if (q.splits <= 1) return;
   if (b >= q.red_blocks) {
     const int n = (b - q.red_blocks) * 256 + threadIdx.x;
@@ -450,6 +542,8 @@
   }
   const int K4 = q.K >> 2;
   const size_t total = (size_t)q.N * K4;
+  const bool upd = q.upd_where == 2;
+  const AdamwScalars sc = adamw_scalars(uc.lr, uc.b1, uc.b2, uc.eps, uc.wd, uc.bc1, uc.bc2, uc.gscale);
   for (size_t idx = (size_t)b * 256 + threadIdx.x; idx < total; idx += (size_t)q.red_blocks * 256) {
     const int n = (int)(idx / K4), k4 = (int)(idx % K4);
     float4 s4 = *(reinterpret_cast<const float4*>(q.out + (size_t)n * q.K) + k4);
@@ -463,6 +557,17 @@
       s4.x += d.x; s4.y += d.y; s4.z += d.z; s4.w += d.w;
     }
     *dst = s4;
+    if (upd) {
+      const uint2 pk = tn_update4(q.up, uc, sc, (size_t)n * q.ldw + 4 * k4, s4);
+      if (q.up.dst) *reinterpret_cast<uint2*>((bf16_t*)q.up.dst + (size_t)n * q.up.ld_dst + 4 * k4) = pk;
+      if (q.up.dstT) {
+        bf16_t* t = (bf16_t*)q.up.dstT + (size_t)(4 * k4) * q.up.ld_dstT + n;
+        t[0] = (bf16_t)(pk.x & 0xffffu);
+        t[(size_t)q.up.ld_dstT] = (bf16_t)(pk.x >> 16);
+        t[2 * (size_t)q.up.ld_dstT] = (bf16_t)(pk.y & 0xffffu);
+        t[3 * (size_t)q.up.ld_dstT] = (bf16_t)(pk.y >> 16);
+      }
+    }
   }
 }
 
@@ -737,11 +842,46 @@
   return pl.ws_floats * sizeof(float) + (n > TG_MAX ? TG_TBL_BYTES : 0);
 }
 
+static int tn_grouped_impl(const lc2is_tn_problem* problems, int n, const lc2is_tn_update* updates,
+                           const lc2is_update_consts* consts, int* applied, void* workspace, size_t workspace_bytes,
+                           hipStream_t stream);
+
 extern "C" int lc2is_gemm_tn_grouped(const lc2is_tn_problem* problems, int n, void* workspace, size_t workspace_bytes,
                                      lc2is_stream_t stream_) {
-  hipStream_t stream = (hipStream_t)stream_;
+  return tn_grouped_impl(problems, n, nullptr, nullptr, nullptr, workspace, workspace_bytes, (hipStream_t)stream_);
+}
+
+extern "C" int lc2is_gemm_tn_grouped_update(const lc2is_tn_problem* problems, int n, const lc2is_tn_update* updates,
+                                            const lc2is_update_consts* consts, int* applied, void* workspace,
+                                            size_t workspace_bytes, lc2is_stream_t stream_) {
+  if (updates && !consts) return LC2IS_ERR_NULL;
+  return tn_grouped_impl(problems, n, updates, consts, applied, workspace, workspace_bytes, (hipStream_t)stream_);
+}
+
+static int tg_update_valid(const lc2is_tn_problem* pr, int n, const lc2is_tn_update* up, const lc2is_update_consts* c) {
+  if (c->kind != LC2IS_UPDATE_SGD && c->kind != LC2IS_UPDATE_ADAMW) return LC2IS_ERR_UNSUPPORTED;
+  if (c->kind == LC2IS_UPDATE_ADAMW && c->step < 1) return LC2IS_ERR_SHAPE;
+  for (int i = 0; i < n; ++i) {
+    const lc2is_tn_update& u = up[i];
+    if (!u.p) continue;
+    if (c->kind == LC2IS_UPDATE_ADAMW && (!u.state0 || !u.state1)) return LC2IS_ERR_NULL;
+    if (((uintptr_t)u.p | (uintptr_t)u.state0 | (uintptr_t)u.state1 | (uintptr_t)pr[i].dW | (uintptr_t)u.dstT) & 15u)
+      return LC2IS_ERR_SHAPE;
+    if ((uintptr_t)u.dst & 7u) return LC2IS_ERR_SHAPE;
+    if (u.dst && (u.ld_dst < pr[i].K || u.ld_dst % 4)) return LC2IS_ERR_SHAPE;
+    if (u.dstT && (u.ld_dstT < pr[i].N || u.ld_dstT % 8)) return LC2IS_ERR_SHAPE;
+  }
+  return LC2IS_OK;
+}
+
+static int tn_grouped_impl(const lc2is_tn_problem* problems, int n, const lc2is_tn_update* updates,
+                           const lc2is_update_consts* consts, int* applied, void* workspace, size_t workspace_bytes,
+                           hipStream_t stream) {
   int rc = tg_valid(problems, n);
   if (rc) return rc;
+  if (updates && (rc = tg_update_valid(problems, n, updates, consts)) != LC2IS_OK) return rc;
+  if (applied)
+    for (int i = 0; i < n; ++i) applied[i] = 0;
   TgPlan pl;
   tg_plan(problems, n, pl, lc2is_ncu());
   const bool tbl = n > TG_MAX;
@@ -780,6 +920,16 @@
   static const int xcd_order = !(getenv("LC2IS_TN_XCD") && atoi(getenv("LC2IS_TN_XCD")) == 0);
   t.n = n;
   t.pad_[0] = xcd_order;
+  t.uc = UpdConsts{};
+  if (updates) {
+    t.uc.kind = consts->kind == LC2IS_UPDATE_ADAMW ? LC2IS_UPD_ADAMW : LC2IS_UPD_SGD;
+    t.uc.lr = consts->lr; t.uc.momentum = consts->momentum; t.uc.wd = consts->weight_decay; t.uc.gscale = consts->grad_scale;
+    t.uc.b1 = consts->beta1; t.uc.b2 = consts->beta2; t.uc.eps = consts->eps;
+    if (consts->kind == LC2IS_UPDATE_ADAMW) {
+      t.uc.bc1 = 1.f - powf(consts->beta1, (float)consts->step);
+      t.uc.bc2 = 1.f - powf(consts->beta2, (float)consts->step);
+    }
+  }
   float* ws = (float*)((char*)workspace + (tbl ? TG_TBL_BYTES : 0));
   int blk = 0, red = 0;
   for (int k = 0; k < n; ++k) {
@@ -811,6 +961,13 @@
     int rb = (int)((total4 + 255) / 256);
     if (rb > 1024) rb = 1024;
     d.red_blocks = d.splits > 1 ? rb : 0;
+    d.up = lc2is_tn_update{};
+    d.upd_where = 0;
+    if (updates && updates[i].p && !pl.small && !q.accumulate) {
+      d.up = updates[i];
+      d.upd_where = d.splits > 1 ? 2 : 1;
+      if (applied) applied[i] = 1;
+    }
     red += d.splits > 1 ? rb + (q.db ? (q.N + 255) / 256 : 0) : 0;
     d.red_end = red;
     t.blk_end[k] = blk;
@@ -848,6 +1005,7 @@
   TnGroup g{};
   g.n = n;
   g.remap = xcd_order;
+  g.uc = t.uc;
   for (int k = 0; k < n; ++k) g.p[k] = t.p[k];
   if (pl.small)
     hipLaunchKernelGGL(gemm_tn_grouped_small_kernel, dim3(blk), dim3(256), 2 * TN_STAGE, stream, g);
diff --git a/lc2is_amd/csrc/misc.hip b/lc2is_amd/csrc/misc.hip
--- a/lc2is_amd/csrc/misc.hip
+++ b/lc2is_amd/csrc/misc.hip
@@ -1,5 +1,6 @@
 #include "common.h"
 #include "lc2is_hip.h"
+#include "optim_update.h"
 
 namespace {
 
@@ -248,44 +249,27 @@
 }
 
 __global__ __launch_bounds__(256) void sgd_kernel(float* p, const float* __restrict__ g, float* mom, size_t n4,
-                                                   float lr, float momentum, float wd, float gscale) {
+                                                   float lr, float momentum, float wd, float gscale,
+                                                   const uint8_t* __restrict__ skip) {
   for (size_t i = (size_t)blockIdx.x * 256 + threadIdx.x; i < n4; i += (size_t)gridDim.x * 256) {
-    float4 pv = reinterpret_cast<float4*>(p)[i];
+    if (skip && skip[i >> 4]) continue;
+    const float4 pv = reinterpret_cast<float4*>(p)[i];
     const float4 gv = reinterpret_cast<const float4*>(g)[i];
-    float d[4] = {gv.x * gscale + wd * pv.x, gv.y * gscale + wd * pv.y, gv.z * gscale + wd * pv.z,
-                  gv.w * gscale + wd * pv.w};
-    if (mom) {
-      float4 mv = reinterpret_cast<float4*>(mom)[i];
-      mv.x = momentum * mv.x + d[0]; mv.y = momentum * mv.y + d[1];
-      mv.z = momentum * mv.z + d[2]; mv.w = momentum * mv.w + d[3];
-      reinterpret_cast<float4*>(mom)[i] = mv;
-      d[0] = mv.x; d[1] = mv.y; d[2] = mv.z; d[3] = mv.w;
-    }
-    pv.x -= lr * d[0]; pv.y -= lr * d[1]; pv.z -= lr * d[2]; pv.w -= lr * d[3];
-    reinterpret_cast<float4*>(p)[i] = pv;
+    reinterpret_cast<float4*>(p)[i] =
+        sgd_update4(pv, gv, mom ? mom + 4 * i : nullptr, lr, momentum, wd, gscale);
   }
 }
 
 __global__ __launch_bounds__(256) void adamw_kernel(float* p, const float* __restrict__ g, float* m, float* v,
                                                      size_t n4, float lr, float b1, float b2, float eps,
-                                                     float wd, float bc1, float bc2, float gscale) {
+                                                     float wd, float bc1, float bc2, float gscale,
+                                                     const uint8_t* __restrict__ skip) {
+  const AdamwScalars sc = adamw_scalars(lr, b1, b2, eps, wd, bc1, bc2, gscale);
   for (size_t i = (size_t)blockIdx.x * 256 + threadIdx.x; i < n4; i += (size_t)gridDim.x * 256) {
-    float4 pv = reinterpret_cast<float4*>(p)[i];
+    if (skip && skip[i >> 4]) continue;
+    const float4 pv = reinterpret_cast<float4*>(p)[i];
     const float4 gv = reinterpret_cast<const float4*>(g)[i];
-    float4 mv = reinterpret_cast<float4*>(m)[i], vv = reinterpret_cast<float4*>(v)[i];
-    float* pp = &pv.x; const float* gp = &gv.x; float* mp = &mv.x; float* vp = &vv.x;
-#pragma unroll
-    for (int k = 0; k < 4; ++k) {
-      const float gg = gp[k] * gscale;
-      pp[k] *= (1.f - lr * wd);
-      mp[k] = b1 * mp[k] + (1.f - b1) * gg;
-      vp[k] = b2 * vp[k] + (1.f - b2) * gg * gg;
-      const float denom = sqrtf(vp[k]) / sqrtf(bc2) + eps;
-      pp[k] -= (lr / bc1) * (mp[k] / denom);
-    }
-    reinterpret_cast<float4*>(p)[i] = pv;
-    reinterpret_cast<float4*>(m)[i] = mv;
-    reinterpret_cast<float4*>(v)[i] = vv;
+    reinterpret_cast<float4*>(p)[i] = adamw_update4(sc, pv, gv, m + 4 * i, v + 4 * i);
   }
 }
 
@@ -426,24 +410,49 @@
   return lc2is_check_launch();
 }
 
+static int sgd_step_impl(float* params, const float* grads, float* momentum_buf, size_t n, float lr, float momentum,
+                         float weight_decay, float grad_scale, const uint8_t* skip, hipStream_t stream) {
+  if (!params || !grads) return LC2IS_ERR_NULL;
+  if (n == 0 || n % 4 || (skip && n % 64)) return LC2IS_ERR_SHAPE;
+  hipLaunchKernelGGL(sgd_kernel, dim3(ew_grid(n / 4)), dim3(256), 0, stream, params, grads, momentum_buf, n / 4,
+                     lr, momentum, weight_decay, grad_scale, skip);
+  return lc2is_check_launch();
+}
+
+static int adamw_step_impl(float* params, const float* grads, float* exp_avg, float* exp_avg_sq, size_t n, float lr,
+                           float beta1, float beta2, float eps, float weight_decay, int step, float grad_scale,
+                           const uint8_t* skip, hipStream_t stream) {
+  if (!params || !grads || !exp_avg || !exp_avg_sq) return LC2IS_ERR_NULL;
+  if (n == 0 || n % 4 || step < 1 || (skip && n % 64)) return LC2IS_ERR_SHAPE;
+  const float bc1 = 1.f - powf(beta1, (float)step), bc2 = 1.f - powf(beta2, (float)step);
+  hipLaunchKernelGGL(adamw_kernel, dim3(ew_grid(n / 4)), dim3(256), 0, stream, params, grads, exp_avg,
+                     exp_avg_sq, n / 4, lr, beta1, beta2, eps, weight_decay, bc1, bc2, grad_scale, skip);
+  return lc2is_check_launch();
+}
+
 extern "C" int lc2is_sgd_step(float* params, const float* grads, float* momentum_buf, size_t n, float lr,
                               float momentum, float weight_decay, float grad_scale, lc2is_stream_t stream_) {
-  hipStream_t stream = (hipStream_t)stream_;
-  if (!params || !grads) return LC2IS_ERR_NULL;
-  if (n == 0 || n % 4) return LC2IS_ERR_SHAPE;
-  hipLaunchKernelGGL(sgd_kernel, dim3(ew_grid(n / 4)), dim3(256), 0, stream, params, grads, momentum_buf, n / 4,
-                     lr, momentum, weight_decay, grad_scale);
-  return lc2is_check_launch();
+  return sgd_step_impl(params, grads, momentum_buf, n, lr, momentum, weight_decay, grad_scale, nullptr, (hipStream_t)stream_);
 }
 
 extern "C" int lc2is_adamw_step(float* params, const float* grads, float* exp_avg, float* exp_avg_sq, size_t n,
                                 float lr, float beta1, float beta2, float eps, float weight_decay, int step,
                                 float grad_scale, lc2is_stream_t stream_) {
-  hipStream_t stream = (hipStream_t)stream_;
-  if (!params || !grads || !exp_avg || !exp_avg_sq) return LC2IS_ERR_NULL;
-  if (n == 0 || n % 4 || step < 1) return LC2IS_ERR_SHAPE;
-  const float bc1 = 1.f - powf(beta1, (float)step), bc2 = 1.f - powf(beta2, (float)step);
-  hipLaunchKernelGGL(adamw_kernel, dim3(ew_grid(n / 4)), dim3(256), 0, stream, params, grads, exp_avg,
-                     exp_avg_sq, n / 4, lr, beta1, beta2, eps, weight_decay, bc1, bc2, grad_scale);
-  return lc2is_check_launch();
-}
+  return adamw_step_impl(params, grads, exp_avg, exp_avg_sq, n, lr, beta1, beta2, eps, weight_decay, step, grad_scale, nullptr,
+                         (hipStream_t)stream_);
+}
+
+extern "C" int lc2is_sgd_step_masked(float* params, const float* grads, float* momentum_buf, size_t n, float lr,
+                                     float momentum, float weight_decay, float grad_scale, const uint8_t* skip,
+                                     lc2is_stream_t stream_) {
+  if (!skip) return LC2IS_ERR_NULL;
+  return sgd_step_impl(params, grads, momentum_buf, n, lr, momentum, weight_decay, grad_scale, skip, (hipStream_t)stream_);
+}
+
+extern "C" int lc2is_adamw_step_masked(float* params, const float* grads, float* exp_avg, float* exp_avg_sq, size_t n,
+                                       float lr, float beta1, float beta2, float eps, float weight_decay, int step,
+                                       float grad_scale, const uint8_t* skip, lc2is_stream_t stream_) {
+  if (!skip) return LC2IS_ERR_NULL;
+  return adamw_step_impl(params, grads, exp_avg, exp_avg_sq, n, lr, beta1, beta2, eps, weight_decay, step, grad_scale, skip,
+                         (hipStream_t)stream_);
+}
diff --git a/lc2is_amd/csrc/optim_update.h b/lc2is_amd/csrc/optim_update.h
--- /dev/null
+++ b/lc2is_amd/csrc/optim_update.h
@@ -0,0 +1,81 @@
+#pragma once
+#include <hip/hip_runtime.h>
+
+enum { LC2IS_UPD_NONE = 0, LC2IS_UPD_SGD = 1, LC2IS_UPD_ADAMW = 2 };
+
+struct UpdConsts {
+  int kind;
+  float lr, momentum, wd, gscale;
+  float b1, b2, eps, bc1, bc2;
+};
+
+__device__ __forceinline__ float sgd_dir(float p, float g, float wd, float gscale) {
+  return __fmaf_rn(wd, p, __fmul_rn(g, gscale));
+}
+__device__ __forceinline__ float sgd_mom(float momentum, float mv, float d) { return __fmaf_rn(momentum, mv, d); }
+__device__ __forceinline__ float sgd_apply(float p, float lr, float d) { return __fmaf_rn(-lr, d, p); }
+
+struct AdamwScalars {
+  float decay, omb1, omb2, b1, b2, lr_bc1, sqrt_bc2, eps, gscale;
+};
+__device__ __forceinline__ AdamwScalars adamw_scalars(float lr, float b1, float b2, float eps, float wd, float bc1, float bc2,
+                                                      float gscale) {
+  AdamwScalars s;
+  s.decay = __fmaf_rn(-lr, wd, 1.f);
+  s.omb1 = __fsub_rn(1.f, b1);
+  s.omb2 = __fsub_rn(1.f, b2);
+  s.b1 = b1; s.b2 = b2;
+  s.lr_bc1 = lr / bc1;
+  s.sqrt_bc2 = sqrtf(bc2);
+  s.eps = eps; s.gscale = gscale;
+  return s;
+}
+__device__ __forceinline__ void adamw_update1(const AdamwScalars& s, float& p, float g, float& m, float& v) {
+  const float gg = __fmul_rn(g, s.gscale);
+  m = __fmaf_rn(s.omb1, gg, __fmul_rn(s.b1, m));
+  v = __fmaf_rn(gg, __fmul_rn(s.omb2, gg), __fmul_rn(s.b2, v));
+  const float denom = __fadd_rn(sqrtf(v) / s.sqrt_bc2, s.eps);
+  p = __fmaf_rn(s.decay, p, -__fmul_rn(s.lr_bc1, (m / denom)));
+}
+
+template <bool HAS_MOM>
+__device__ __forceinline__ void sgd_update4_regs(float4& pv, const float4 gv, float4& mv, float lr, float momentum, float wd,
+                                                 float gscale) {
+  float d[4] = {sgd_dir(pv.x, gv.x, wd, gscale), sgd_dir(pv.y, gv.y, wd, gscale), sgd_dir(pv.z, gv.z, wd, gscale),
+                sgd_dir(pv.w, gv.w, wd, gscale)};
+  if constexpr (HAS_MOM) {
+    mv.x = sgd_mom(momentum, mv.x, d[0]); mv.y = sgd_mom(momentum, mv.y, d[1]);
+    mv.z = sgd_mom(momentum, mv.z, d[2]); mv.w = sgd_mom(momentum, mv.w, d[3]);
+    d[0] = mv.x; d[1] = mv.y; d[2] = mv.z; d[3] = mv.w;
+  }
+  pv.x = sgd_apply(pv.x, lr, d[0]); pv.y = sgd_apply(pv.y, lr, d[1]);
+  pv.z = sgd_apply(pv.z, lr, d[2]); pv.w = sgd_apply(pv.w, lr, d[3]);
+}
+
+__device__ __forceinline__ void adamw_update4_regs(const AdamwScalars& s, float4& pv, const float4 gv, float4& mv, float4& vv) {
+  adamw_update1(s, pv.x, gv.x, mv.x, vv.x);
+  adamw_update1(s, pv.y, gv.y, mv.y, vv.y);
+  adamw_update1(s, pv.z, gv.z, mv.z, vv.z);
+  adamw_update1(s, pv.w, gv.w, mv.w, vv.w);
+}
+
+__device__ __forceinline__ float4 sgd_update4(float4 pv, const float4 gv, float* mom, float lr, float momentum, float wd,
+                                              float gscale) {
+  float4 mv = make_float4(0.f, 0.f, 0.f, 0.f);
+  if (mom) {
+    mv = *reinterpret_cast<float4*>(mom);
+    sgd_update4_regs<true>(pv, gv, mv, lr, momentum, wd, gscale);
+    *reinterpret_cast<float4*>(mom) = mv;
+  } else {
+    sgd_update4_regs<false>(pv, gv, mv, lr, momentum, wd, gscale);
+  }
+  return pv;
+}
+
+__device__ __forceinline__ float4 adamw_update4(const AdamwScalars& s, float4 pv, const float4 gv, float* m, float* v) {
+  float4 mv = *reinterpret_cast<float4*>(m), vv = *reinterpret_cast<float4*>(v);
+  adamw_update4_regs(s, pv, gv, mv, vv);
+  *reinterpret_cast<float4*>(m) = mv;
+  *reinterpret_cast<float4*>(v) = vv;
+  return pv;
+}
diff --git a/lc2is_amd/nn/base.py b/lc2is_amd/nn/base.py
--- a/lc2is_amd/nn/base.py
+++ b/lc2is_amd/nn/base.py
@@ -132,6 +132,10 @@
         self._sh_versions = None
         self._sh_device = None
         self._sh_ptrs = []
+        self._sh_entries = []
+        self._sh_pending = None
+        self._sh_residuals = {}
+        self._fwd_saves = 0
         self._grad_ready_cb = None
         self._part_ready_cb = None
 
@@ -149,12 +153,17 @@
             ns, entries = self._build_shadows(dev)
             self._sh = ns
             self._sh_table = ops.ShadowTable(entries, dev) if entries else None
+            self._sh_entries, self._sh_residuals, self._sh_pending = list(entries), {}, None
             self._sh_device = dev
             self._sh_ptrs = [p.data_ptr() for p in ps]
             self._sh_versions = None
         vers = [p._version for p in ps]
         if vers != self._sh_versions:
-            if self._sh_table is not None:
+            pending, self._sh_pending = self._sh_pending, None
+            if pending is not None and pending[0] == vers:
+                if pending[1] is not None:
+                    pending[1].refresh()
+            elif self._sh_table is not None:
                 self._sh_table.refresh()
             self._post_refresh()
             self._sh_versions = vers
@@ -177,6 +186,23 @@
 
     def invalidate_shadows(self):
         self._sh_versions = None
+        self._sh_pending = None
+
+    def shadows_refreshed_in_kernel(self, param_ptrs) -> bool:
+        if self._sh is None or self._sh_table is None:
+            return False
+        done = frozenset(i for i, (src, _, _) in enumerate(self._sh_entries) if src.data_ptr() in param_ptrs)
+        if not done:
+            return False
+        if done not in self._sh_residuals:
+            if torch.cuda.is_current_stream_capturing():
+                raise RuntimeError("HipModule: the set of weights updated in-kernel while capturing differs from every warm-up "
+                                   "step's; the residual shadow table cannot be uploaded inside a captured step")
+            rest = [e for i, e in enumerate(self._sh_entries) if i not in done]
+            self._sh_residuals[done] = ops.ShadowTable(rest, self._sh_device) if rest else None
+        self._sh_versions = None
+        self._sh_pending = ([p._version for p in self._params_for_version()], self._sh_residuals[done])
+        return True
 
     def _apply(self, fn, *args, **kwargs):
         self._sh = None
@@ -221,23 +247,80 @@
         ops.ln_defer_flush()
         items, self.items = self.items, []
         gmax = ops.GROUP_MAX
+        fu = FusedUpdate._active
         for i in range(0, len(items), gmax):
             chunk = items[i:i + gmax]
+            probs = [it[:5] for it in chunk]
             if len(chunk) == 1:
-                dy, x, g, gb, acc = chunk[0]
+                dy, x, g, gb, acc = probs[0]
                 ops.gemm_tn(dy, x, g, accumulate=acc, db=gb)
+            elif fu is None:
+                ops.gemm_tn_grouped(probs)
             else:
-                ops.gemm_tn_grouped(chunk)
-
-
-def linear_bwd_params(dy_bf16: torch.Tensor, x_bf16: torch.Tensor, weight: nn.Parameter, bias: nn.Parameter | None):
+                weights = [it[5] for it in chunk]
+                updates = fu.updates_for(weights, [it[6] for it in chunk])
+                with ops.tn_update(updates, fu.consts):
+                    flags = ops.gemm_tn_grouped(probs)
+                fu.record([w for w, f in zip(weights, flags) if f])
+
+
+class FusedUpdate:
+
+    _active = None
+
+    def __init__(self, arena, consts, state0=None, state1=None):
+        self.arena, self.consts, self.state0, self.state1 = arena, consts, state0, state1
+        self.applied = []
+        self._offered = set()
+        self._twice = set()
+
+    def offer(self, weight, acc: bool, shadow) -> bool:
+        wid = id(weight)
+        if wid in self._offered:
+            self._twice.add(wid)
+        self._offered.add(wid)
+        return (not acc) and shadow is not None and weight.dim() == 2 and wid in self.arena.ranges and wid not in self._twice
+
+    def updates_for(self, weights, shadows):
+        out = []
+        for w, sh in zip(weights, shadows):
+            if w is None or id(w) in self._twice:
+                out.append(None)
+                continue
+            lo, hi = self.arena.ranges[id(w)]
+            st = [None if s is None else s[lo:hi].view(w.shape) for s in (self.state0, self.state1)]
+            out.append((w.data, st[0], st[1], sh[0], sh[1]))
+        return out
+
+    def record(self, weights):
+        self.applied.extend(weights)
+
+    def applied_ranges(self):
+        return sorted(self.arena.ranges[id(w)] for w in self.applied)
+
+
+def skip_granules(ranges, numel: int, align: int = 64) -> torch.Tensor:
+    if numel % align:
+        raise ValueError("skip_granules: the arena must be whole granules")
+    m = torch.zeros(numel // align, dtype=torch.uint8)
+    for lo, hi in ranges:
+        if not 0 <= lo < hi <= numel or lo % align or hi % align:
+            raise ValueError(f"skip_granules: range ({lo}, {hi}) is not whole granules of a {numel}-element arena")
+        m[lo // align:hi // align] = 1
+    return m
+
+
+def linear_bwd_params(dy_bf16: torch.Tensor, x_bf16: torch.Tensor, weight: nn.Parameter, bias: nn.Parameter | None,
+                      shadow=None):
     want_b = bias is not None and bias.requires_grad
     if weight.requires_grad:
         g, acc = grad_buf(weight)
         gb, accb = grad_buf(bias) if want_b else (None, False)
         batch = WgradBatch._active
+        fu = FusedUpdate._active
+        take = fu is not None and fu.offer(weight, acc, shadow)
         if batch is not None and (gb is None or accb == acc) and ops.gemm_tn_groupable(dy_bf16, x_bf16):
-            batch.items.append((dy_bf16, x_bf16, g.reshape(g.shape[0], -1), gb, acc))
+            batch.items.append((dy_bf16, x_bf16, g.reshape(g.shape[0], -1), gb, acc, weight if take else None, shadow))
             return
         with _on_wgrad_stream(dy_bf16, x_bf16):
             if gb is not None and accb != acc:
diff --git a/lc2is_amd/nn/clip.py b/lc2is_amd/nn/clip.py
--- a/lc2is_amd/nn/clip.py
+++ b/lc2is_amd/nn/clip.py
@@ -183,7 +183,7 @@
 
 
 def _stack_bwd(g32, g16, stack: _Stack, sh, saved, a: ClipArch, B: int, S: int, kbias, causal: bool, on_layer_done=None,
-               final_f32: bool = True):
+               final_f32: bool = True, fuse: bool = False):
     C, H = a.hidden, a.heads
     D = C // H
     scale = D ** -0.5
@@ -202,22 +202,23 @@
         for layer, s, sv in zip(reversed(stack.layers), reversed(sh), reversed(saved)):
             x, m1, r1, h, qkv, o, lse, x_mid, m2, r2, h2, z, act = sv
             at, mlp = layer.self_attn, layer.mlp
-            linear_bwd_params(g16, act, mlp.fc2.weight, mlp.fc2.bias)
+            linear_bwd_params(g16, act, mlp.fc2.weight, mlp.fc2.bias, shadow=(s["w2"], s["w2T"]) if fuse else None)
             dz, _, _ = ops.gemm_nt(g16, s["w2T"], None, act=ops.ACT_DQUICK_GELU, aux_in=z)
-            linear_bwd_params(dz, h2, mlp.fc1.weight, mlp.fc1.bias)
+            linear_bwd_params(dz, h2, mlp.fc1.weight, mlp.fc1.bias, shadow=(s["w1"], s["w1T"]) if fuse else None)
             dh2, _, _ = ops.gemm_nt(dz, s["w1T"], None)
             dg, accg = vec_grad(layer.layer_norm2.weight)
             db, _ = vec_grad(layer.layer_norm2.bias)
             gm32, gm16, _, _ = ops.layernorm_bwd(dh2, x_mid, layer.layer_norm2.weight, m2, r2, dres=g16 if lean else g32,
                                                  dgamma=dg, dbeta=db, accumulate=accg, want_f32=not lean,
                                                  need_param_grads=dg is not None)
-            linear_bwd_params(gm16, o, at.out_proj.weight, at.out_proj.bias)
+            linear_bwd_params(gm16, o, at.out_proj.weight, at.out_proj.bias, shadow=(s["wo"], s["woT"]) if fuse else None)
             do, _, _ = ops.gemm_nt(gm16, s["woT"], None)
             dqkv = torch.empty_like(qkv)
             ops.attention_bwd(qkv[:, :C], qkv[:, C:2 * C], qkv[:, 2 * C:], o, do, lse, B, H, S, S, D, scale, causal=causal,
                               kbias=kbias, dq=dqkv[:, :C], dk=dqkv[:, C:2 * C], dv=dqkv[:, 2 * C:])
             for j, proj in enumerate((at.q_proj, at.k_proj, at.v_proj)):
-                linear_bwd_params(dqkv[:, j * C:(j + 1) * C], h, proj.weight, proj.bias)
+                linear_bwd_params(dqkv[:, j * C:(j + 1) * C], h, proj.weight, proj.bias,
+                                  shadow=(s["wqkv"][j * C:(j + 1) * C], s["wqkvT"][:, j * C:(j + 1) * C]) if fuse else None)
             dh, _, _ = ops.gemm_nt(dqkv, s["wqkvT"], None)
             dg, accg = vec_grad(layer.layer_norm1.weight)
             db, _ = vec_grad(layer.layer_norm1.bias)
@@ -329,6 +330,8 @@
     def _fwd(self, pixel_values, keep_cls, save):
         require_cuda(pixel_values, "pixel_values")
         a, sh = self.arch, self._ensure_ready()
+        if save:
+            self._fwd_saves += 1
         B = pixel_values.shape[0]
         G = self.in_size // self.patch_size
         P = G * G
@@ -369,7 +372,7 @@
             g16 = ops.cast_bf16(g32)
         g32, g16 = _stack_bwd(g32, g16, self.enc.encoder, sh["layers"], saved["layers"], a, B, P + 1, None, False,
                               on_layer_done=self._part_grads_ready if self._part_ready_cb is not None else None,
-                              final_f32=False)
+                              final_f32=False, fuse=self._fwd_saves == 1)
         dg, accg = vec_grad(self.enc.pre_layrnorm.weight)
         db, _ = vec_grad(self.enc.pre_layrnorm.bias)
         dx0, _, _, _ = ops.layernorm_bwd(g32 if g32 is not None else g16, saved["x0"], self.enc.pre_layrnorm.weight, saved["m0"], saved["r0"],
diff --git a/lc2is_amd/ops.py b/lc2is_amd/ops.py
--- a/lc2is_amd/ops.py
+++ b/lc2is_amd/ops.py
@@ -50,6 +50,8 @@
     "lc2is_rows_copy_f32": [_P, _I, _I, _P, _P, _I, _I, _I, _I, _I, _P],
     "lc2is_sgd_step": [_P, _P, _P, _Z, _F, _F, _F, _F, _P],
     "lc2is_adamw_step": [_P, _P, _P, _P, _Z, _F, _F, _F, _F, _F, _I, _F, _P],
+    "lc2is_sgd_step_masked": [_P, _P, _P, _Z, _F, _F, _F, _F, _P, _P],
+    "lc2is_adamw_step_masked": [_P, _P, _P, _P, _Z, _F, _F, _F, _F, _F, _I, _F, _P, _P],
     "lc2is_grad_sumsq_blocks": [_Z],
     "lc2is_grad_sumsq_workspace_bytes": [_Z],
     "lc2is_grad_sumsq": [_P, _Z, _P, _Z, _P],
@@ -84,6 +86,7 @@
     "lc2is_npair_bwd": [_P, _P, _P, _P, _P, _P, _P, _P, _I, _I, _I, _I, _P],
     "lc2is_gemm_tn_grouped_workspace_bytes": [_P, _I],
     "lc2is_gemm_tn_grouped": [_P, _I, _P, _Z, _P],
+    "lc2is_gemm_tn_grouped_update": [_P, _I, _P, _P, _P, _P, _Z, _P],
     "lc2is_release_captured_tables": [],
     "lc2is_captured_tables_mark": [],
     "lc2is_release_captured_tables_range": [_I, _I],
@@ -106,7 +109,7 @@
         f = getattr(_lib.load(), name)
         if name in _ARGTYPES:
             f.argtypes = _ARGTYPES[name]
-        if name.endswith("_workspace_bytes"):
+        if name.endswith("_bytes"):
             f.restype = C.c_size_t
         _bound[name] = f
     return f
@@ -290,9 +293,77 @@
     return dy.shape[1] % 8 == 0 and x.shape[1] % 8 == 0 and dy.shape[0] >= _GROUP_MIN_ROWS
 
 
-def gemm_tn_grouped(problems):
+class TnUpdate(C.Structure):
+    _fields_ = [("p", C.c_void_p), ("state0", C.c_void_p), ("state1", C.c_void_p), ("dst", C.c_void_p), ("dstT", C.c_void_p),
+                ("ld_dst", C.c_int), ("ld_dstT", C.c_int)]
+
+
+class UpdateConsts(C.Structure):
+    _fields_ = [("kind", C.c_int), ("step", C.c_int), ("lr", C.c_float), ("momentum", C.c_float), ("weight_decay", C.c_float),
+                ("grad_scale", C.c_float), ("beta1", C.c_float), ("beta2", C.c_float), ("eps", C.c_float)]
+
+
+UPDATE_SGD, UPDATE_ADAMW = 1, 2
+
+
+def update_consts(kind: str, *, lr: float, momentum: float = 0.0, weight_decay: float = 0.0, grad_scale: float = 1.0,
+                  betas=(0.9, 0.999), eps: float = 1e-8, step: int = 1) -> UpdateConsts:
+    if kind not in ("sgd", "adamw"):
+        raise ValueError("update_consts: kind must be 'sgd' or 'adamw'")
+    if kind == "adamw" and int(step) < 1:
+        raise ValueError("update_consts: AdamW needs step >= 1")
+    return UpdateConsts(UPDATE_SGD if kind == "sgd" else UPDATE_ADAMW, int(step), lr, momentum, weight_decay, grad_scale,
+                        betas[0], betas[1], eps)
+
+
+def pack_tn_update(dw: torch.Tensor, upd, kind: str) -> TnUpdate:
+    if upd is None:
+        return TnUpdate()
+    p, s0, s1, dst, dstT = upd
+    N, K = dw.shape
+    for name, t in (("p", p), ("state0", s0), ("state1", s1)):
+        if t is None:
+            continue
+        if t.dtype != torch.float32 or tuple(t.shape) != (N, K) or t.stride() != dw.stride():
+            raise RuntimeError(f"lc2is_amd.gemm_tn_grouped: update {name} must be fp32 and laid out like dW")
+    if p is None or (kind == "adamw" and (s0 is None or s1 is None)):
+        raise RuntimeError("lc2is_amd.gemm_tn_grouped: update without p (or AdamW without both moments)")
+    if kind == "sgd" and s1 is not None:
+        raise RuntimeError("lc2is_amd.gemm_tn_grouped: SGD has one state buffer")
+    if dst is not None and (dst.dtype != torch.bfloat16 or tuple(dst.shape) != (N, K) or dst.stride(1) != 1):
+        raise RuntimeError("lc2is_amd.gemm_tn_grouped: update dst must be a bf16 [N,K] view with unit inner stride")
+    if dstT is not None and (dstT.dtype != torch.bfloat16 or tuple(dstT.shape) != (K, N) or dstT.stride(1) != 1):
+        raise RuntimeError("lc2is_amd.gemm_tn_grouped: update dstT must be a bf16 [K,N] view with unit inner stride")
+    return TnUpdate(_ptr(p), _ptr(s0), _ptr(s1), _ptr(dst), _ptr(dstT), _ld(dst), _ld(dstT))
+
+
+_tn_update_ctx = None
+
+
+class tn_update:
+
+    def __init__(self, updates, consts):
+        self.ctx = (updates, consts)
+
+    def __enter__(self):
+        global _tn_update_ctx
+        _tn_update_ctx = self.ctx
+        return self
+
+    def __exit__(self, *exc):
+        global _tn_update_ctx
+        _tn_update_ctx = None
+        return False
+
+
+def gemm_tn_grouped(problems, updates=None, consts: UpdateConsts | None = None):
+    global _tn_update_ctx
+    if updates is None and _tn_update_ctx is not None:
+        (updates, consts), _tn_update_ctx = _tn_update_ctx, None
     if not 1 <= len(problems) <= GROUP_MAX:
         raise RuntimeError(f"lc2is_amd.gemm_tn_grouped: 1..{GROUP_MAX} problems per launch")
+    if updates is not None and (consts is None or len(updates) != len(problems)):
+        raise RuntimeError("lc2is_amd.gemm_tn_grouped: updates need consts and one entry (or None) per problem")
     arr = (TnProblem * len(problems))()
     for i, (dy, x, dw, db, acc) in enumerate(problems):
         _chk(dy, torch.bfloat16, "dy"); _chk(x, torch.bfloat16, "x"); _chk(dw, torch.float32, "dw"); _chk(db, torch.float32, "db", 1)
@@ -302,8 +373,18 @@
         arr[i] = TnProblem(_ptr(dy), _ptr(x), _ptr(dw), _ptr(db), _ld(dy), _ld(x), _ld(dw), M, N, x.shape[1], int(acc))
     nbytes = _fn("lc2is_gemm_tn_grouped_workspace_bytes")(arr, len(problems))
     ws = workspace(nbytes, problems[0][0].device, "gemm_tn_grouped")
-    rc = _fn("lc2is_gemm_tn_grouped")(arr, len(problems), _ptr(ws), ws.numel(), _stream())
-    _lib.check(rc, f"gemm_tn_grouped n={len(problems)}")
+    if updates is None or all(u is None for u in updates):
+        rc = _fn("lc2is_gemm_tn_grouped")(arr, len(problems), _ptr(ws), ws.numel(), _stream())
+        _lib.check(rc, f"gemm_tn_grouped n={len(problems)}")
+        return [False] * len(problems)
+    kind = "sgd" if consts.kind == UPDATE_SGD else "adamw"
+    uarr = (TnUpdate * len(problems))()
+    for i, u in enumerate(updates):
+        uarr[i] = pack_tn_update(problems[i][2], u, kind)
+    applied = (C.c_int * len(problems))()
+    rc = _fn("lc2is_gemm_tn_grouped_update")(arr, len(problems), uarr, C.byref(consts), applied, _ptr(ws), ws.numel(), _stream())
+    _lib.check(rc, f"gemm_tn_grouped_update n={len(problems)}")
+    return [bool(a) for a in applied]
 
 
 def release_captured_tables() -> int:
@@ -517,6 +598,10 @@
 INTERP_BICUBIC, INTERP_BILINEAR = 0, 1
 
 
+shadow_refresh_launches = 0
+shadow_refresh_tiles = 0
+
+
 class ShadowDesc(C.Structure):
     _fields_ = [("src", C.c_void_p), ("dst", C.c_void_p), ("dstT", C.c_void_p), ("N", C.c_int), ("K", C.c_int),
                 ("ld_dst", C.c_int), ("ld_dstT", C.c_int), ("tile_start", C.c_int), ("flags", C.c_int)]
@@ -556,6 +641,9 @@
         self.dev = torch.frombuffer(bytearray(raw), dtype=torch.uint8).to(device)
 
     def refresh(self):
+        global shadow_refresh_launches, shadow_refresh_tiles
+        shadow_refresh_launches += 1
+        shadow_refresh_tiles += self.total_tiles
         rc = _fn("lc2is_shadow_refresh")(self.dev.data_ptr(), self.n, self.total_tiles, _stream())
         _lib.check(rc, "shadow_refresh")
 
@@ -654,6 +742,24 @@
     _chk(params, torch.float32, "params", 1); _chk(grads, torch.float32, "grads", 1)
     _lib.check(_fn("lc2is_adamw_step")(_ptr(params), _ptr(grads), _ptr(m), _ptr(v), params.numel(), lr, beta1,
                                        beta2, eps, weight_decay, int(step), grad_scale, _stream()), "adamw_step")
+
+
+def _chk_skip(params, skip):
+    _chk(skip, torch.uint8, "skip", 1)
+    if params.numel() % 64 or skip.numel() != params.numel() // 64:
+        raise RuntimeError("lc2is_amd: a masked optimizer step needs whole 64-element granules and one skip byte per granule")
+
+
+def sgd_step_masked(params, grads, momentum_buf, skip, lr, momentum=0.0, weight_decay=0.0, grad_scale=1.0):
+    _chk(params, torch.float32, "params", 1); _chk(grads, torch.float32, "grads", 1); _chk_skip(params, skip)
+    _lib.check(_fn("lc2is_sgd_step_masked")(_ptr(params), _ptr(grads), _ptr(momentum_buf), params.numel(), lr, momentum,
+                                            weight_decay, grad_scale, _ptr(skip), _stream()), "sgd_step_masked")
+
+
+def adamw_step_masked(params, grads, m, v, skip, lr, beta1, beta2, eps, weight_decay, step, grad_scale=1.0):
+    _chk(params, torch.float32, "params", 1); _chk(grads, torch.float32, "grads", 1); _chk_skip(params, skip)
+    _lib.check(_fn("lc2is_adamw_step_masked")(_ptr(params), _ptr(grads), _ptr(m), _ptr(v), params.numel(), lr, beta1, beta2, eps,
+                                              weight_decay, int(step), grad_scale, _ptr(skip), _stream()), "adamw_step_masked")
 
 
 OPTIM_CTRL_WORDS = 12
diff --git a/lc2is_amd/step.py b/lc2is_amd/step.py
--- a/lc2is_amd/step.py
+++ b/lc2is_amd/step.py
@@ -8,7 +8,7 @@
 from torch import nn
 
 from . import ops
-from .nn.base import HipModule, ParamArena
+from .nn.base import FusedUpdate, HipModule, ParamArena, skip_granules
 
 
 _DEFAULT_LR = 1e-5
@@ -155,6 +155,10 @@
     return [dict(params=names, lr_scale=scale, weight_decay=wd) for (scale, wd), names in merged.items()]
 
 
+def fused_update_eligible(*, reducer, device_path: bool, env: str | None) -> bool:
+    return env != "0" and reducer is None and not device_path
+
+
 class TrainStep:
 
     def __init__(self, model: nn.Module, *, optimizer: str = "sgd", lr: float = _DEFAULT_LR, momentum: float = 0.0,
@@ -212,6 +216,34 @@
         if groups is not None:
             self.arena.set_groups([group_of[id(p)] for p in self.arena.params], len(groups))
             self._group_table = torch.tensor([[g["lr_scale"], g["weight_decay"]] for g in groups], dtype=torch.float32).to(dev)
+        self._skip_maps = {}
+        self.fused_applied = 0
+
+    @property
+    def fused_update(self) -> bool:
+        return fused_update_eligible(reducer=self.reducer, device_path=self._ctrl is not None,
+                                     env=os.environ.get("LC2IS_FUSED_UPDATE"))
+
+    def _arm(self):
+        if not self.fused_update:
+            return None
+        for m in self._hip_modules:
+            m._fwd_saves = 0
+        consts = ops.update_consts(self.kind, lr=self.lr, momentum=self.momentum, weight_decay=self.weight_decay, grad_scale=1.0,
+                                   betas=self.betas, eps=self.eps, step=self.t + 1)
+        if self.kind == "sgd":
+            return FusedUpdate(self.arena, consts, self.mom)
+        return FusedUpdate(self.arena, consts, self.m, self.v)
+
+    def _skip_map(self, ranges) -> torch.Tensor:
+        key = tuple(ranges)
+        m = self._skip_maps.get(key)
+        if m is None:
+            if torch.cuda.is_current_stream_capturing():
+                raise RuntimeError("TrainStep: the set of weights updated in-kernel while capturing differs from every warm-up "
+                                   "step's; the skip map cannot be uploaded inside a captured step")
+            m = self._skip_maps[key] = skip_granules(key, self.arena.numel, self.arena.ALIGN).to(self._dev)
+        return m
 
     def _ctrl_view(self, word: int, as_float: bool) -> torch.Tensor:
         if self._ctrl is None:
@@ -248,13 +280,18 @@
         arena.zero_grad(set_to_none=True)
         if self.reducer is not None:
             self.reducer.begin_step()
+        fused = self._arm()
         if self._loss_opts:
             c = self.criterion
             loss = self.model.forward_loss(inputs, labels, self.ignore_index, weight=c.weight,
                                            label_smoothing=float(c.label_smoothing), reduction=c.reduction)
         else:
             loss = self.model.forward_loss(inputs, labels, self.ignore_index)
-        loss.backward()
+        prev, FusedUpdate._active = FusedUpdate._active, fused
+        try:
+            loss.backward()
+        finally:
+            FusedUpdate._active = prev
         live = arena.finalize_grads()
         gscale = 1.0
         if self.reducer is not None:
@@ -286,16 +323,24 @@
                     ops.adamw_step_ctrl(arena.flat[sl], arena.grad[sl], self.m[sl], self.v[sl], ctrl, self.betas[0],
                                         self.betas[1], self.eps, self.weight_decay, reverse=self.reverse_walk)
             segs = []
+        done = fused.applied_ranges() if fused is not None else []
+        self.fused_applied = len(done)
+        skip = self._skip_map(done) if done else None
         for lo, hi in segs:
             sl = slice(lo, hi)
+            sk = () if skip is None else (skip[lo // arena.ALIGN:hi // arena.ALIGN],)
             if self.kind == "sgd":
-                ops.sgd_step(arena.flat[sl], arena.grad[sl], None if self.mom is None else self.mom[sl], self.lr,
-                             self.momentum, self.weight_decay, gscale)
+                (ops.sgd_step_masked if sk else ops.sgd_step)(arena.flat[sl], arena.grad[sl], None if self.mom is None else self.mom[sl],
+                                                              *sk, self.lr, self.momentum, self.weight_decay, gscale)
             else:
-                ops.adamw_step(arena.flat[sl], arena.grad[sl], self.m[sl], self.v[sl], self.lr, self.betas[0],
-                               self.betas[1], self.eps, self.weight_decay, self.t, gscale)
+                (ops.adamw_step_masked if sk else ops.adamw_step)(arena.flat[sl], arena.grad[sl], self.m[sl], self.v[sl], *sk, self.lr,
+                                                                  self.betas[0], self.betas[1], self.eps, self.weight_decay, self.t, gscale)
         for m in self._hip_modules:
             m.invalidate_shadows()
+        if done:
+            ptrs = {w.data_ptr() for w in fused.applied}
+            for m in self._hip_modules:
+                m.shadows_refreshed_in_kernel(ptrs)
         return loss.detach()
 
     def capture(self, inputs: dict, labels: torch.Tensor, warmup: int = 2):
```

Result: no change. 1078 images/s (-0.1%).
